# MinghanLi/STMask

Hardware: AMD Instinct MI355X
Metric: frames/sec at 360x640 R50-DCN-FPN (STMask hot path, fp32) (higher is better)
Workload: dtype f32

## Files before the change

include/stmask_hip.h:

```cpp
#ifndef STMASK_HIP_H_
#define STMASK_HIP_H_

#include <stddef.h>
#include <stdint.h>

#ifdef __cplusplus
extern "C" {
#endif

#define STM_ABI_VERSION 6

enum stm_status {
    STM_OK = 0,
    STM_EINVAL = -1,
    STM_ENULL = -2,
    STM_ELAUNCH = -3,
    STM_EWORKSPACE = -4,
    STM_EUNSUPPORTED = -5
};

typedef void* stm_stream_t;

int stm_version(void);
const char* stm_last_error_string(void);
// ... 177 lines not shown

int stm_gather_detections_f32(const int64_t* idx, const int64_t* cls, const float* score, const float* box, const int* count,
                              const float* mask_coeff, const float* track, const float* centerness, int B, int top_k, int N,
                              int mask_dim, int embed_dim, int D, float* out_box, int64_t* out_cls, float* out_score,
                              float* out_coeff, float* out_track, float* out_centerness, int* out_clip, stm_stream_t stream);
int stm_shift_rois_f32(const float* box, const int* clip, float* rois, int n, int feat_h, int feat_w, stm_stream_t stream);
int stm_shift_apply_f32(const float* loc_shift, const float* coeff_shift, float* box, float* coeff, float* score, int n,
                        int mask_dim, float score_decay, stm_stream_t stream);
int stm_match_scores_f32(const float* cos, const float* mask_iou, const float* det_box, const float* prev_box,
                         const float* det_score, const int64_t* det_cls, const int64_t* prev_cls, const int* det_clip,
                         const int* prev_offsets, int D, int Pn, const float* coeff4, float dummy_iou, int* match,
                         stm_stream_t stream);
int stm_match_scores_embed_f32(const float* det_track, const float* prev_track, int embed_dim, const float* mask_iou,
                               const float* det_box, const float* prev_box, const float* det_score, const int64_t* det_cls,
                               const int64_t* prev_cls, const int* det_clip, const int* prev_offsets, int D, int Pn,
                               const float* coeff4, float dummy_iou, int* match, stm_stream_t stream);
int stm_gather_rows2(const void* const* a_rows, const void* const* b_rows, void* const* out_rows, const int* row_bytes,
                     int n_tensors, const int* plan, int n_rows, int n_a, stm_stream_t stream);
int stm_pack_tracked_f32(const float* mask, const float* score, const int* tracked, const int* offsets, const float* box,
                         const int64_t* cls, const float* mask_coeff, int n_rows, int hw, int B, int top_k, int cols,
                         int mask_dim, int max_age, float score_thr, int* keep_ws, float* out, stm_stream_t stream);
int stm_pack_tracked_bits_f32(const uint64_t* mask_bits, int words, const float* score, const int* tracked, const int* offsets,
                              const float* box, const int64_t* cls, const float* mask_coeff, int n_rows, int B, int top_k,
                              int cols, int mask_dim, int max_age, float score_thr, int* keep_ws, float* out,
                              stm_stream_t stream);

int stm_split_planes_f16(const float* x, void* planes, int64_t n_pixels, int C, stm_stream_t stream);
int stm_conv_pack_weights_f16(const float* weight, void* packed, int Cout, int Cin, int kh, int kw, int tile_n, float wscale,
                              stm_stream_t stream);
int stm_conv2d_planar_f16(const void* x_planes, const void* packed_weight, const float* bias, const float* residual_f32,
                          const void* residual_planes, float* out_f32, void* out_planes, const stm_conv_geom* g, int relu,
                          void* workspace, size_t workspace_bytes, stm_stream_t stream);
int stm_dcn_sample_planar_f16(const float* x, const float* offset_mask, int om_ld, void* planes, int out_np,
                              long long out_plane_stride, const stm_deform_geom* g, stm_stream_t stream);

int stm_preprocess_u8_f32(const uint8_t* img, float* out, int n, int H0, int W0, int h, int w, int Hp, int Wp,
                          const double* mean, const double* stdv, int mode, stm_stream_t stream);

typedef struct stm_frame_desc {
    const uint8_t* ptr;
    int H0, W0;
    int64_t row_stride_bytes;
} stm_frame_desc;
int stm_preprocess_u8_multi_f32(const stm_frame_desc* frames, int n, float* out, int h, int w, int Hp, int Wp, const double* mean,
                                const double* stdv, int mode, stm_stream_t stream);

typedef struct stm_head_layout {
    int B, K, n_levels, n_cls, mask_dim, embed_dim, group_pad, small_ld, trk_ld;
    int lvl_start[8], lvl_hw[8];
} stm_head_layout;
int stm_head_assemble_f32(const float* const* small, const float* const* trk, const stm_head_layout* layout, float* conf,
                          float* loc, float* mask, float* track, float* centerness, stm_stream_t stream);

int stm_dcn_sample_planar_f32(const float* x, const float* offset_mask, int om_ld, void* planes, int out_np,
                              long long out_plane_stride, const stm_deform_geom* g, stm_stream_t stream);
int stm_resize_bilinear_planes_f32(const float* x, void* planes, int B, int H, int W, int C, int Ho, int Wo, int fmt,
                                   stm_stream_t stream);

int stm_bias_relu_maxpool_planes_f32(const float* x, const float* bias, void* planes, int B, int H, int W, int C, int fmt,
                                     stm_stream_t stream);

int stm_roi_align_planes_f32(const float* t2s_prev, const float* t2s, const float* corr, const float* rois, void* planes, int B,
                             int H, int W, int C1, int Cc, int n, int PH, int PW, int fmt, stm_stream_t stream);
int stm_roi_align_planes_nhwc_f32(const float* t2s_prev, const float* t2s, const float* corr, int corr_ld, const float* rois,
                                  void* planes, int B, int H, int W, int C1, int Cc, int n, int PH, int PW, int fmt,
                                  stm_stream_t stream);

int stm_stem_rows_planes_f32(const float* x, void* planes, int B, int H, int W, int Cin, int kw, int sw, int pw, int fmt,
                             stm_stream_t stream);

size_t stm_stem_packed_weight_bytes(int Cout, int fmt);
int stm_stem_pack_weights_f32(const float* weight, void* packed, int Cout, int fmt, float wscale, stm_stream_t stream);
int stm_stem_fused_f32(const float* x, const void* packed_weight, const float* bias, void* out_planes, int B, int H, int W, int Cout,
                       int fmt, int out_fmt, float out_scale, stm_stream_t stream);

int stm_planar_set_range_flag(int* device_flag);

int stm_deform_sample_planar_f32(const float* x, int x_ld, const float* offsets, int om_ld, int has_mask, void* planes, int out_np,
                                 int out_pixel_offset, long long out_plane_stride, const stm_deform_geom* g, int fmt,
                                 stm_stream_t stream);

int stm_dcn_sample_planar_fmt_f32(const float* x, const float* offset_mask, int om_ld, void* planes, int out_np,
                                  long long out_plane_stride, const stm_deform_geom* g, int fmt, stm_stream_t stream);

int stm_deform_conv_fused_planar_supported(const stm_deform_geom* g, int Cout, int has_mask, int fmt);
int stm_deform_conv_fused_planar_f32(const float* x, int x_ld, const float* offsets, int om_ld, int has_mask, const void* packed_weight,
                                     const float* bias, void* out_planes, int out_np, int out_pixel_offset, long long out_plane_stride,
                                     int Cout, int relu, float out_scale, const stm_deform_geom* g, int fmt, int out_fmt,
                                     stm_stream_t stream);

typedef struct stm_render_frame {
    const void* base;
    uint8_t* out;
    int64_t base_row_stride;
    int64_t out_row_stride;
    double mean[3], stdv[3];
    int base_fmt, base_h, base_w, base_crop_h, base_crop_w;
    int out_h, out_w;
    int inst_begin, n_inst, crop_h, crop_w;
    int reserved;
} stm_render_frame;
size_t stm_render_workspace_bytes(int n_masks);
int stm_render_overlay_u8(const stm_render_frame* frames, int n_frames, const float* masks, int n_masks, int mh, int mw,
                          const float* colors, const int* boxes, float alpha, void* workspace, size_t workspace_bytes,
                          stm_stream_t stream);

// ... 15 lines not shown
```

stmask_amd/_lib.py:

```python
import ctypes
import os
import subprocess

_HERE = os.path.dirname(os.path.abspath(__file__))
LIB_PATH = os.environ.get("STM_LIBRARY") or os.path.join(_HERE, "libstmask_hip.so")
_lib = None

c_i, c_l, c_f, c_p, c_sz = ctypes.c_int, ctypes.c_int64, ctypes.c_float, ctypes.c_void_p, ctypes.c_size_t

ABI_VERSION = 6
ABI_SYMBOLS = [
    "stm_version", "stm_last_error_string", "stm_struct_bytes", "stm_debug_reload_tunables", "stm_debug_launch_count", "stm_conv_kxr_packed_bytes", "stm_conv_pack_weights_kxr_f32", "stm_conv2d_planar_kxr_f32", "stm_conv2d_planar_dual_f32", "stm_conv2d_planar_windows_f32", "stm_conv2d_planar_windows_pool_f32", "stm_temporal_pool_fc_f32", "stm_stem_packed_weight_bytes", "stm_stem_pack_weights_f32", "stm_stem_fused_f32", "stm_chain_tail_weight_bytes", "stm_chain_tail_weight_bytes_proj", "stm_chain_pack_tail_f32", "stm_chain_pack_tail_proj_f32", "stm_bottleneck_chain_f32", "stm_bottleneck_chain_proj_f32", "stm_deform_im2col_f32", "stm_deform_conv_workspace_bytes",
    "stm_deform_conv_fwd_f32", "stm_gemm_bias_f32", "stm_gemm_workspace_bytes", "stm_gemm_bias_ws_f32", "stm_fcb_ali_offsets_f32", "stm_corr_patch_f32", "stm_corr_patch_nhwc_f32",
    "stm_roi_align_avg_f32", "stm_decode_boxes_f32", "stm_generate_candidates_f32", "stm_cc_fast_nms_f32",
    "stm_detect_cc_workspace_bytes", "stm_detect_cc_f32", "stm_detect_cc_logits_f32", "stm_fast_nms_workspace_bytes", "stm_fast_nms_f32",
    "stm_jaccard_f32", "stm_lincomb_sigmoid_crop_f32", "stm_mask_iou_workspace_bytes", "stm_mask_iou_f32",
    "stm_bias_act_f32", "stm_mask_rle_workspace_bytes", "stm_mask_resize_rle_f32",
    "stm_conv_packed_weight_bytes", "stm_conv_pack_weights_f32",
    "stm_split_bf16_planes_f32", "stm_conv2d_planar_f32", "stm_conv_packed_weight_bytes_tiled",
    "stm_conv_pack_weights_tiled_f32", "stm_preprocess_u8_f32", "stm_head_assemble_f32", "stm_conv2d_planar_ws_f32", "stm_dcn_sample_planar_f32", "stm_conv_pack_weights_fmt_f32", "stm_split_planes_fmt_f32", "stm_dcn_sample_planar_fmt_f32", "stm_planar_set_range_flag", "stm_resize_bilinear_planes_f32", "stm_bias_relu_maxpool_planes_f32", "stm_roi_align_planes_f32", "stm_roi_align_planes_nhwc_f32", "stm_deform_sample_planar_f32", "stm_stem_rows_planes_f32", "stm_mask_iou_grouped_f32", "stm_cc_fast_nms_workspace_bytes", "stm_cc_fast_nms_ws_f32",
    "stm_gather_detections_f32", "stm_shift_rois_f32", "stm_shift_apply_f32", "stm_match_scores_f32", "stm_match_scores_embed_f32", "stm_gather_rows2", "stm_pack_tracked_f32", "stm_pack_tracked_bits_f32",
    "stm_lincomb_sigmoid_crop_bits_f32", "stm_mask_iou_bits_f32", "stm_split_planes_f16", "stm_conv_pack_weights_f16", "stm_conv2d_planar_f16", "stm_dcn_sample_planar_f16",
    "stm_deform_conv_fused_planar_supported", "stm_deform_conv_fused_planar_f32", "stm_fast_nms_batched_workspace_bytes", "stm_fast_nms_batched_f32", "stm_rle_strings_host",
    "stm_preprocess_u8_multi_f32", "stm_render_workspace_bytes", "stm_render_overlay_u8",
    "stm_deform_col2im_f32", "stm_deform_col2im_coord_f32", "stm_roi_align_backward_f32", "stm_corr_backward_f32",
]


class StmError(RuntimeError):
    pass


class DeformGeom(ctypes.Structure):
    _fields_ = [(n, c_i) for n in ("B", "C", "H", "W", "kh", "kw", "sh", "sw", "ph", "pw", "dh", "dw", "dg", "Ho", "Wo")]


class ConvGeom(ctypes.Structure):
    _fields_ = ([(n, c_i) for n in ("B", "H", "W", "C", "Ho", "Wo", "Cout", "kh", "kw", "sh", "sw", "ph", "pw", "x_ld",
                                    "out_ld", "res_ld", "planes", "groups", "n_levels")] +
                [("lvl_start", c_i * 9), ("lvl_h", c_i * 8), ("lvl_w", c_i * 8),
                 ("x_plane_stride", c_l), ("out_plane_stride", c_l), ("res_plane_stride", c_l), ("x_np", c_i), ("out_np", c_i), ("res_np", c_i), ("group_cout", c_i * 8), ("fmt", c_i), ("out_scale", c_f), ("tile_n", c_i), ("out_fmt_plus1", c_i),
                 ("win_h", c_i), ("win_w", c_i), ("win_y0", c_i), ("win_x0", c_i)])


class ConvWindow(ctypes.Structure):
    _fields_ = [(n, c_i) for n in ("kh", "kw", "ph", "pw", "Ho", "Wo", "y0", "x0")]


class FrameDesc(ctypes.Structure):
    _fields_ = [("ptr", c_p), ("H0", c_i), ("W0", c_i), ("row_stride_bytes", c_l)]


class RenderFrame(ctypes.Structure):
    _fields_ = ([("base", c_p), ("out", c_p), ("base_row_stride", c_l), ("out_row_stride", c_l), ("mean", ctypes.c_double * 3),
                 ("stdv", ctypes.c_double * 3)] +
                [(n, c_i) for n in ("base_fmt", "base_h", "base_w", "base_crop_h", "base_crop_w", "out_h", "out_w", "inst_begin", "n_inst",
                                    "crop_h", "crop_w", "reserved")])


class HeadLayout(ctypes.Structure):
    _fields_ = ([(n, c_i) for n in ("B", "K", "n_levels", "n_cls", "mask_dim", "embed_dim", "group_pad", "small_ld", "trk_ld")] +
                [("lvl_start", c_i * 8), ("lvl_hw", c_i * 8)])


def build(force=False):
    cmd = ["make", "-C", os.path.join(_HERE, "csrc"), "-s", "-j4"]
    if force:
        cmd.append("-B")
    subprocess.check_call(cmd)
    return LIB_PATH


def lib():
    global _lib
    if _lib is None:
        if not os.path.exists(LIB_PATH):
            raise StmError(
                f"{LIB_PATH} is missing: build it with `python -c 'import __graft_entry__ as g; g.build()'` "
# ... 30 lines not shown
```

stmask_amd/csrc/capi.hip:

```cpp
#include <stdarg.h>
#include <stdlib.h>

#include <atomic>

#include "stm_common.h"

static thread_local char g_err[512] = "";

void stm_set_error(const char* fmt, ...)
{
    va_list ap;
    va_start(ap, fmt);
    vsnprintf(g_err, sizeof(g_err), fmt, ap);
    va_end(ap);
}

extern "C" int stm_version(void) { return STM_ABI_VERSION; }
extern "C" const char* stm_last_error_string(void) { return g_err; }
extern "C" size_t stm_struct_bytes(int which)
{
    switch (which) {
        case 0: return sizeof(stm_deform_geom);
        case 1: return sizeof(stm_conv_geom);
        case 2: return sizeof(stm_conv_window);
        case 3: return sizeof(stm_head_layout);
        case 4: return sizeof(stm_frame_desc);
        case 5: return sizeof(stm_render_frame);
        default: return 0;
    }
}

static std::atomic<int> g_env_gen{0};
int stm_env_generation() { return g_env_gen.load(std::memory_order_relaxed); }
int stm_env_int_uncached(const char* name, int dflt)
{
    const char* s = getenv(name);
    return (s && *s) ? atoi(s) : dflt;
}
extern "C" void stm_debug_reload_tunables() { g_env_gen.fetch_add(1, std::memory_order_relaxed); }

extern "C" int stm_rle_strings_host(const uint32_t* counts, int ld, const int* n_runs, int n, char* out, int out_ld, int* out_len)
{
    STM_REQUIRE(n >= 0 && ld >= 0 && out_ld >= 0, STM_EINVAL, "stm_rle_strings_host: negative size");
    if (n == 0) return STM_OK;
    STM_REQUIRE(counts && n_runs && out && out_len, STM_ENULL, "stm_rle_strings_host: NULL argument");
    int rc = STM_OK;
    for (int i = 0; i < n; ++i) {
        const uint32_t* c = counts + (size_t)i * ld;
        char* o = out + (size_t)i * out_ld;
        const int m = n_runs[i] < ld ? n_runs[i] : ld;
        int len = 0;
        for (int j = 0; j < m; ++j) {
            long long x = (long long)c[j];
            if (j > 2) x -= (long long)c[j - 2];
            bool more = true;
            while (more) {
                int ch = (int)(x & 0x1f);
                x >>= 5;
                more = (ch & 0x10) ? x != -1 : x != 0;
                if (more) ch |= 0x20;
                if (len < out_ld) o[len] = (char)(ch + 48);
                ++len;
            }
        }
        out_len[i] = len;
        if (len > out_ld) rc = STM_EINVAL;
    }
    if (rc != STM_OK) stm_set_error("stm_rle_strings_host: a string needs more than %d bytes", out_ld);
    return rc;
}
```

stmask_amd/csrc/conv_bf16x.hip:

```cpp
#include "planar_common.h"
#include <algorithm>
#include <type_traits>
#include <atomic>
#include <mutex>
#include <unordered_map>

namespace {

__device__ __forceinline__ void store_planes8(uint8_t* dst, size_t plane_b, const float (&v)[8], int fmt, int* range_flag, bool nt)
{
    unsigned q0[4], q1[4], q2[4];
    if (fmt == 0) {
#pragma unroll
        for (int e = 0; e < 4; ++e) split2(f32x2{v[2 * e], v[2 * e + 1]}, q0[e], q1[e], q2[e]);
    } else {
        f16_range_check8(v, range_flag);
#pragma unroll
        for (int e = 0; e < 4; ++e) split2_f16(f32x2{v[2 * e], v[2 * e + 1]}, q0[e], q1[e]);
    }
    const int np = fmt == 0 ? 3 : (fmt == 1 ? 2 : 1);
    if (nt) {
        __builtin_nontemporal_store(u32x4{q0[0], q0[1], q0[2], q0[3]}, reinterpret_cast<u32x4*>(dst));
        if (np > 1) __builtin_nontemporal_store(u32x4{q1[0], q1[1], q1[2], q1[3]}, reinterpret_cast<u32x4*>(dst + plane_b));
        if (np > 2) __builtin_nontemporal_store(u32x4{q2[0], q2[1], q2[2], q2[3]}, reinterpret_cast<u32x4*>(dst + 2 * plane_b));
    } else {
        *reinterpret_cast<u32x4*>(dst) = u32x4{q0[0], q0[1], q0[2], q0[3]};
        if (np > 1) *reinterpret_cast<u32x4*>(dst + plane_b) = u32x4{q1[0], q1[1], q1[2], q1[3]};
        if (np > 2) *reinterpret_cast<u32x4*>(dst + 2 * plane_b) = u32x4{q2[0], q2[1], q2[2], q2[3]};
    }
}

constexpr int STM_MAX_DEVICES = 32;
static int* g_range_flags[STM_MAX_DEVICES] = {};
static int* current_range_flag()
{
    int dev = 0;
    if (hipGetDevice(&dev) != hipSuccess || dev < 0 || dev >= STM_MAX_DEVICES) return nullptr;
    return g_range_flags[dev];
}

struct PlanarArgs {
    const uint8_t* xp;
    const uint8_t* wp;
    const float* bias;
    const float* res_f32;
    const uint8_t* res_pl;
    float* out_f32;
    uint8_t* out_pl;
    int B, H, W, C, Ho, Wo, Cout;
    int kh, kw, sh, sw, ph, pw;
    int x_ld, out_ld, res_ld;
    int x_np, out_np, res_np;
    int relu;
    int M, n_tiles, m_tiles, slabs;
    int nsub;
    unsigned plane_bytes;
    long long x_pstride, out_pstride, res_pstride;
    int groups, ntpg, cout_g;
    int group_real[8];
    int n_levels;
    int lvl_start[9], lvl_h[8], lvl_w[8];
    int pointwise;
    float inv_hw, inv_w;
    int fmt;
    int out_fmt;
    float out_scale;
    int* range_flag;
    int nt_out;
    int splitk, kslabs, ldp;
    float* partial;
    int vec_epilogue;
    const uint8_t* xp2;
    long long x2_pstride;
    unsigned plane2_bytes;
    int c1_slabs, x2_np, H2, W2, s2;
    int win_w, win_hw, win_off;
};
struct PlanarArgsCls : PlanarArgs {
    int n_cls, cls_tiles;
    unsigned long long* pool;
    int pool_ld;
    struct Cls { const uint8_t* wp; int kh, kw, ph, pw, Ho, Wo, M, slabs, win_off, tile0; float inv_hw, inv_w; } cls[9];
};

template <int NJ>
__device__ __forceinline__ float* park_base(uint8_t* smem, int wave) { return reinterpret_cast<float*>(smem) + wave * (64 * (32 * NJ + 4)); }

template <int NJ>
__device__ __forceinline__ void park16(f32x4 (&acc)[4][2 * NJ], f32x4 (&accl)[4][2 * NJ], uint8_t* smem, int wave, int lane, float ls = 1.0f)
{
    constexpr int EP_LD = 32 * NJ + 4;
    float* park = park_base<NJ>(smem, wave);
#pragma unroll
    for (int i = 0; i < 4; ++i)
#pragma unroll
        for (int j = 0; j < 2 * NJ; ++j)
#pragma unroll
            for (int r = 0; r < 4; ++r)
                park[(i * 16 + 4 * (lane >> 4) + r) * EP_LD + j * 16 + (lane & 15)] = acc[i][j][r] + accl[i][j][r] * ls;
}

template <bool SCALE_BIAS = true, int FMT = -1>
__device__ __forceinline__ void epilogue_store8(const PlanarArgs& a, int m, int co, int nvalid, float (&v)[8], bool have_pre = false,
                                                f16x8 pre0 = f16x8{}, f16x8 pre1 = f16x8{})
{
    const int fmt = FMT >= 0 ? FMT : a.fmt;
    const int ofmt = (FMT == 0 || FMT == 1) ? FMT : a.out_fmt;
    const size_t opl = (size_t)(a.out_pstride >> 1), rpl = (size_t)(a.res_pstride >> 1);
    auto pidx = [](int m_, int co_, int np) { return ((size_t)(co_ >> 5) * np + m_) * 32 + (co_ & 31); };
    int mo = m;
    if (a.win_w) {
        const int hw = a.Ho * a.Wo;
        int b = (int)((float)m * a.inv_hw);
        int rem = m - b * hw;
        if (rem < 0) { --b; rem += hw; } else if (rem >= hw) { ++b; rem -= hw; }
        int oy = (int)((float)rem * a.inv_w);
        const int t = rem - oy * a.Wo;
        if (t < 0) --oy; else if (t >= a.Wo) ++oy;
        mo = b * a.win_hw + oy * a.win_w + (rem - oy * a.Wo) + a.win_off;
    }
    if constexpr (SCALE_BIAS) {
#pragma unroll
        for (int e = 0; e < 8; ++e) v[e] = __builtin_fmaf(v[e], a.out_scale, (a.bias && e < nvalid) ? a.bias[co + e] : 0.0f);
    }
    if (a.vec_epilogue) {
        if (a.res_f32) {
            const f32x4 r0 = *reinterpret_cast<const f32x4*>(a.res_f32 + (size_t)m * a.res_ld + co);
            const f32x4 r1 = *reinterpret_cast<const f32x4*>(a.res_f32 + (size_t)m * a.res_ld + co + 4);
            v[0] += r0.x; v[1] += r0.y; v[2] += r0.z; v[3] += r0.w; v[4] += r1.x; v[5] += r1.y; v[6] += r1.z; v[7] += r1.w;
// ... 145 lines not shown
            q0[j] = *reinterpret_cast<const f32x4*>(pk);
            q1[j] = *reinterpret_cast<const f32x4*>(pk + 4);
        }
#pragma unroll
        for (int j = 0; j < 4; ++j) {
            if (k0 + j < a.splitk) {
                v[0] += q0[j].x; v[1] += q0[j].y; v[2] += q0[j].z; v[3] += q0[j].w;
                v[4] += q1[j].x; v[5] += q1[j].y; v[6] += q1[j].z; v[7] += q1[j].w;
            }
        }
    }
    epilogue_store8(a, m, grp * a.cout_g + cog, min(8, a.cout_g - cog), v);
}

__device__ __forceinline__ void pooled_epilogue(const PlanarArgs& a, unsigned long long* pool, int pool_ld, uint8_t* smem, int wave, int lane, int mw, int col)
{
    constexpr int EP_LD = 32 * 2 + 4;
    const float* park = park_base<2>(smem, wave);
    asm volatile("s_waitcnt lgkmcnt(0)" ::: "memory");
    const int hw = a.Ho * a.Wo;
    const int rows = min(64, a.M - mw);
    int b = mw / hw, r = mw - b * hw;
    const float bias = a.bias ? a.bias[col] : 0.0f;
    float sum = 0.0f;
    for (int row = 0; row < rows; ++row) {
        sum += __builtin_fmaxf(__builtin_fmaf(park[row * EP_LD + lane], a.out_scale, bias), 0.0f);
        if (++r == hw || row == rows - 1) {
            if (!(sum < 4.0e9f) && a.range_flag) *reinterpret_cast<volatile int*>(a.range_flag) = 1;
            const unsigned hi = (unsigned)sum;
            const unsigned lo = (unsigned)((sum - (float)hi) * 4294967296.0f);
            __hip_atomic_fetch_add(pool + (size_t)b * pool_ld + col, ((unsigned long long)hi << 32) | lo, __ATOMIC_RELAXED, __HIP_MEMORY_SCOPE_AGENT);
            sum = 0.0f;
            if (r == hw) { r = 0; ++b; }
        }
    }
}

template <int NPL, int MG, int NJ, int DT = 0, int ST = 2, int ABL = 0, bool DUAL = false, bool CLS = false>
__global__ __launch_bounds__(512, 1) void conv_planar_kernel(const typename std::conditional<CLS, PlanarArgsCls, PlanarArgs>::type a_in)
{
#if defined(__HIP_DEVICE_COMPILE__)
    extern __shared__ __align__(16) uint8_t smem[];
    constexpr int BM = CV_BM * MG;
    constexpr int BN = 64 * NJ;
    constexpr int WPL = BN * 64;
    constexpr int XBUF = NPL * BM * 64, WBUF = NPL * WPL, BUF = XBUF + WBUF;
    constexpr int NWAVES = 4 * MG;
    constexpr int WDMA = (BN / 16) * NPL / NWAVES;
    static_assert((BN / 16) * NPL % NWAVES == 0, "weight tile must split evenly over the waves");
    static_assert(ST == 2 || (ST == 3 && DT == 1 && NPL <= 2), "the three-buffer ring is built for the fp16 formats");

    int tiles_ = a_in.m_tiles * a_in.n_tiles * a_in.splitk;
    if constexpr (CLS) tiles_ = a_in.cls_tiles;
    const int tiles = tiles_;
    const int per_xcd = (tiles + 7) >> 3;
    int logical = (blockIdx.x & 7) * per_xcd + (blockIdx.x >> 3);
    auto regroup = [&](int j, int nt_all, int& mt_o, int& nt_o) {
        const int pg = 32 / a_in.nsub, G = pg * nt_all;
        const int gq = j / G, r = j - gq * G;
        const int nh = r >> 5, rr = r & 31;
        mt_o = gq * pg + rr / a_in.nsub;
        nt_o = nh * a_in.nsub + rr % a_in.nsub;
    };
    if constexpr (CLS) {
        const int j = blockIdx.x >> 3;
        int jm = j / a_in.n_tiles, nt_ = j - jm * a_in.n_tiles;
        if (a_in.nsub) regroup(j, a_in.n_tiles, jm, nt_);
        logical = (jm * 8 + (int)(blockIdx.x & 7)) * a_in.n_tiles + nt_;
    } else if (a_in.nsub) {
        int mt_, nt_;
        regroup(logical, a_in.n_tiles, mt_, nt_);
        logical = mt_ * a_in.n_tiles + nt_;
    }
    if (logical >= tiles) return;
    PlanarArgs a_cls;
    const PlanarArgs* ap = &a_in;
    if constexpr (CLS) {
        int c = 0;
#pragma unroll
        for (int i = 1; i < 9; ++i)
            if (i < a_in.n_cls && logical >= a_in.cls[i].tile0) c = i;
        a_cls = static_cast<const PlanarArgs&>(a_in);
        a_cls.wp = a_in.cls[c].wp;
        a_cls.kh = a_in.cls[c].kh; a_cls.kw = a_in.cls[c].kw; a_cls.ph = a_in.cls[c].ph; a_cls.pw = a_in.cls[c].pw;
        a_cls.Ho = a_in.cls[c].Ho; a_cls.Wo = a_in.cls[c].Wo; a_cls.M = a_in.cls[c].M;
        a_cls.slabs = a_in.cls[c].slabs; a_cls.kslabs = a_in.cls[c].slabs; a_cls.win_off = a_in.cls[c].win_off;
        a_cls.inv_hw = a_in.cls[c].inv_hw; a_cls.inv_w = a_in.cls[c].inv_w;
        logical -= a_in.cls[c].tile0;
        ap = &a_cls;
    }
    const PlanarArgs& a = *ap;
    const int ksp = a.splitk == 1 ? 0 : logical % a.splitk;
    const int tile = a.splitk == 1 ? logical : logical / a.splitk;
    const int mt = a.n_tiles == 1 ? tile : (a.n_tiles == 2 ? tile >> 1 : (a.n_tiles == 4 ? tile >> 2 : tile / a.n_tiles));
    const int nt = tile - mt * a.n_tiles;
    const int m0 = mt * BM;
    if (m0 >= a.M) return;
    const int s_begin = ksp * a.kslabs, s_end = min(a.slabs, s_begin + a.kslabs);

    const int tid = threadIdx.x, lane = tid & 63;
    const int wave = __builtin_amdgcn_readfirstlane(tid >> 6);
    const int wm = wave % (2 * MG), wn = wave / (2 * MG);

    const int grp = a.groups == 1 ? 0 : nt / a.ntpg;
    const int n0g = (nt - grp * a.ntpg) * BN;
    const int creal = a.group_real[grp & 7];
    int base[2], wl64[2];
    unsigned vmask[2];
    int base2[2] = {0, 0};
    const int slot = lane & 3;
#pragma unroll
    for (int i = 0; i < 2; ++i) {
        const int r = (2 * wave + i) * 16 + (lane >> 2);
        const int m = m0 + r;
        const bool ok = m < a.M;
        const int mm = ok ? m : 0;
        const int swz16 = (slot ^ swz(r)) << 4;
        if constexpr (DUAL) {
            const int hw = a.Ho * a.Wo;
            int b = (int)((float)mm * a.inv_hw);
            int rem = mm - b * hw;
            if (rem < 0) { --b; rem += hw; } else if (rem >= hw) { ++b; rem -= hw; }
            int oy = (int)((float)rem * a.inv_w);
            const int t = rem - oy * a.Wo;
            if (t < 0) --oy; else if (t >= a.Wo) ++oy;
            const int ox = rem - oy * a.Wo;
            base2[i] = ((b * a.H2 + oy * a.s2) * a.W2 + ox * a.s2) * 64 + swz16;
        }
        if (a.pointwise) {
            base[i] = mm * 64 + swz16;
            wl64[i] = 0;
            vmask[i] = ok ? 1u : 0u;
            continue;
        }
        int H = a.H, W = a.W, Ho = a.Ho, Wo = a.Wo, first = 0, local = mm;
        if (a.n_levels > 0) {
#pragma unroll
            for (int l = 0; l < 8; ++l)
                if (l < a.n_levels && mm >= a.lvl_start[l]) { first = a.lvl_start[l]; H = a.lvl_h[l]; W = a.lvl_w[l]; }
            Ho = H; Wo = W; local = mm - first;
        }
        int b, rem, oy, ox;
        if (a.n_levels > 0) {
            b = local / (Ho * Wo);
            rem = local - b * (Ho * Wo);
            oy = rem / Wo;
        } else {
            const int hw = Ho * Wo;
            b = (int)((float)local * a.inv_hw);
            rem = local - b * hw;
// ... 318 lines not shown
        }
    }
    if (a.splitk > 1) {
        constexpr int EP_LD = 32 * NJ + 4, LPR = 4 * NJ;
        const float* park = park_base<NJ>(smem, wave);
        asm volatile("s_waitcnt lgkmcnt(0)" ::: "memory");
        const int seg = lane % LPR, prow = lane / LPR;
        const int col = nt * BN + wn * (32 * NJ) + seg * 8;
#pragma unroll
        for (int pass = 0; pass < LPR; ++pass) {
            const int pr = pass * (64 / LPR) + prow;
            const int m = m0 + wm * 64 + pr;
            if (m >= a.M) continue;
            float* o = a.partial + ((size_t)ksp * a.M + m) * a.ldp + col;
            *reinterpret_cast<f32x4*>(o) = *reinterpret_cast<const f32x4*>(park + pr * EP_LD + seg * 8);
            *reinterpret_cast<f32x4*>(o + 4) = *reinterpret_cast<const f32x4*>(park + pr * EP_LD + seg * 8 + 4);
        }
    } else {
        planar_epilogue_tail<NJ, DT == 1 ? (NPL == 2 ? 1 : 2) : 0>(a, smem, wave, lane, m0, n0g, grp, wm, wn);
    }
#endif
}

constexpr int KX3_XROWS = 272, KX3_XPL = KX3_XROWS * 64, KX3_ABUF = 2 * KX3_XPL, KX3_WBUF = 2 * 128 * 64, KX3_W0 = 2 * KX3_ABUF;
constexpr int KX3_ZROW = 260;
constexpr int KX3_LDS_LOOP = KX3_W0 + 3 * KX3_WBUF;
#ifndef KX3_SCHED
#define KX3_SCHED 24
#endif
#ifndef KX3_WBUFFER
#define KX3_WBUFFER 1
#endif
#ifndef KX3_ABL
#define KX3_ABL 0
#endif
template <int ABL = 0, bool WIN = false>
__global__ __launch_bounds__(512, 1) void conv_planar_kx3_kernel(const typename std::conditional<WIN, PlanarArgsCls, PlanarArgs>::type a_in)
{
#if defined(__HIP_DEVICE_COMPILE__)
    extern __shared__ __align__(16) uint8_t smem[];
    constexpr int NJ = 2, BM = 256, BN = 128, WPL = BN * 64;
    constexpr int XROWS = WIN ? 384 : KX3_XROWS, XPL = XROWS * 64, ABUF = 2 * XPL, W0 = 2 * ABUF;
    int logical, n_tiles_ = a_in.n_tiles, cls_c = 0;
    if constexpr (WIN) {
        const int j = blockIdx.x >> 3;
        const int jm = j / n_tiles_, nt_ = j - jm * n_tiles_;
        logical = (jm * 8 + (int)(blockIdx.x & 7)) * n_tiles_ + nt_;
        if (logical >= a_in.cls_tiles) return;
#pragma unroll
        for (int i = 1; i < 9; ++i)
            if (i < a_in.n_cls && logical >= a_in.cls[i].tile0) cls_c = i;
        logical -= a_in.cls[cls_c].tile0;
    } else {
        const int tiles = a_in.m_tiles * n_tiles_;
        const int per_xcd = (tiles + 7) >> 3;
        logical = (blockIdx.x & 7) * per_xcd + (blockIdx.x >> 3);
        if (logical >= tiles) return;
    }
    const PlanarArgs& a = a_in;
    int KH = a.kh, PH = a.ph, PW = a.pw, HO = a.Ho, WO = a.Wo, MM = a.M, SLABS = a.slabs;
    const uint8_t* WP = a.wp;
    if constexpr (WIN) {
        KH = a_in.cls[cls_c].kh; PH = a_in.cls[cls_c].ph; PW = a_in.cls[cls_c].pw; HO = a_in.cls[cls_c].Ho; WO = a_in.cls[cls_c].Wo;
        MM = a_in.cls[cls_c].M; SLABS = a_in.cls[cls_c].slabs; WP = a_in.cls[cls_c].wp;
    }
    const int mt = n_tiles_ == 1 ? logical : (n_tiles_ == 2 ? logical >> 1 : (n_tiles_ == 4 ? logical >> 2 : logical / n_tiles_));
    const int nt = logical - mt * n_tiles_;
    const int m0 = mt * BM;
    const int tid = threadIdx.x, lane = tid & 63;
    const int wave = __builtin_amdgcn_readfirstlane(tid >> 6);
    const int wm = wave & 3, wn = wave >> 2;
    const int grp = a.groups == 1 ? 0 : nt / a.ntpg;
    const int n0g = (nt - grp * a.ntpg) * BN;
    const int cslabs = a.C / CV_BK;

    auto decode = [&](int m, int& first, int& b, int& oy, int& ox, int& H, int& W) -> bool {
        const bool ok = m >= 0 && m < MM;
        const int mm = ok ? m : 0;
        H = a.H; W = a.W; first = 0;
        int local = mm;
        if (a.n_levels > 0) {
#pragma unroll
            for (int l = 0; l < 8; ++l)
                if (l < a.n_levels && mm >= a.lvl_start[l]) { first = a.lvl_start[l]; H = a.lvl_h[l]; W = a.lvl_w[l]; }
            local = mm - first;
            b = local / (H * W);
            const int rem = local - b * (H * W);
            oy = rem / W;
            ox = rem - oy * W;
        } else {
            const int hw = H * W;
            b = (int)((float)local * a.inv_hw);
            int rem = local - b * hw;
            if (rem < 0) { --b; rem += hw; } else if (rem >= hw) { ++b; rem -= hw; }
            oy = (int)((float)rem * a.inv_w);
            int t = rem - oy * W;
            if (t < 0) --oy; else if (t >= W) ++oy;
            ox = rem - oy * W;
        }
        return ok;
    };

    int base[3], wlv[3];
    const int slot = lane & 3;
    const int Ws = WO + 2, wr0 = WIN ? m0 / WO : 0;
#pragma unroll
    for (int i = 0; i < 3; ++i) {
        const int q = i == 0 ? wave : (i == 1 ? wave + 8 : (WIN ? wave + 16 : 16));
        const int j = q * 16 + (lane >> 2);
        if constexpr (WIN) {
            const int qr = j / Ws, xi = j - qr * Ws;
            const int wr = wr0 + qr;
            const bool ok = wr * WO < MM;
            const int b = wr / HO, oy = wr - b * HO;
            wlv[i] = a.W * 64 + (ok ? 63 : 0);
            base[i] = ((b * a.H + oy - PH) * a.W + (xi - PW)) * 64 + ((slot ^ swz(j)) << 4);
        } else {
            int first, b, oy, ox, H, W;
            const bool ok = decode(m0 - 1 + j, first, b, oy, ox, H, W) && j < BM + 2;
            unsigned vm = 0;
            for (int ky = 0; ky < KH; ++ky)
// ... 940 lines not shown
}

extern "C" int stm_conv2d_planar_dual_f32(const void* x_planes, const void* x2_planes, int C2, int H2, int W2, int s2, long long x2_np,
                                          long long x2_plane_stride, const void* packed_weight, const float* bias, const float* residual_f32,
                                          const void* residual_planes, float* out_f32, void* out_planes, const stm_conv_geom* g, int relu,
                                          void* workspace, size_t workspace_bytes, stm_stream_t stream)
{
    STM_REQUIRE(x2_planes && g, STM_ENULL, "stm_conv2d_planar_dual_f32: x2_planes / geometry must be non-NULL");
    DualSrc d{x2_planes, C2, H2, W2, s2, x2_np, x2_plane_stride};
    return conv2d_planar_impl(x_planes, packed_weight, bias, residual_f32, residual_planes, out_f32, out_planes, g, relu, workspace,
                              workspace_bytes, stream, &d, nullptr);
}

extern "C" int stm_conv2d_planar_windows_f32(const void* x_planes, const void* const* packed_weights, const stm_conv_window* windows, int n_windows,
                                             const float* bias, float* out_f32, void* out_planes, const stm_conv_geom* g, int relu, stm_stream_t stream)
{
    const char* who = "stm_conv2d_planar_windows_f32";
    STM_REQUIRE(packed_weights && windows && g, STM_ENULL, "%s: NULL argument", who);
    STM_REQUIRE(n_windows >= 1 && n_windows <= 9, STM_EINVAL, "%s: 1 .. 9 windows", who);
    STM_REQUIRE(g->win_w > 0 && g->win_h > 0 && g->fmt == 1 && g->sh == 1 && g->sw == 1 && (g->groups <= 1) && g->n_levels <= 0 &&
                (g->tile_n == 0 || g->tile_n == 128), STM_EUNSUPPORTED, "%s: fp16x2 planes, stride 1, one group, 128-channel tiles, win_h / win_w set", who);
    for (int i = 0; i < n_windows; ++i) STM_REQUIRE(packed_weights[i], STM_ENULL, "%s: packed weight %d is NULL", who, i);
    stm_conv_geom g0 = *g;
    g0.kh = windows[0].kh; g0.kw = windows[0].kw; g0.ph = windows[0].ph; g0.pw = windows[0].pw;
    g0.Ho = windows[0].Ho; g0.Wo = windows[0].Wo; g0.win_y0 = windows[0].y0; g0.win_x0 = windows[0].x0;
    WinSet ws{packed_weights, windows, n_windows, nullptr};
    return conv2d_planar_impl(x_planes, packed_weights[0], bias, nullptr, nullptr, out_f32, out_planes, &g0, relu, nullptr, 0, stream, nullptr, &ws);
}

extern "C" int stm_conv2d_planar_windows_pool_f32(const void* x_planes, const void* const* packed_weights, const stm_conv_window* windows, int n_windows,
                                                  const float* bias, unsigned long long* pool_fix, const stm_conv_geom* g, stm_stream_t stream)
{
    const char* who = "stm_conv2d_planar_windows_pool_f32";
    STM_REQUIRE(packed_weights && windows && g && pool_fix, STM_ENULL, "%s: NULL argument", who);
    STM_REQUIRE(n_windows >= 1 && n_windows <= 9, STM_EINVAL, "%s: 1 .. 9 windows", who);
    STM_REQUIRE(g->win_w > 0 && g->win_h > 0 && g->fmt == 1 && g->sh == 1 && g->sw == 1 && (g->groups <= 1) && g->n_levels <= 0 &&
                (g->tile_n == 0 || g->tile_n == 128) && g->Cout % 128 == 0, STM_EUNSUPPORTED,
                "%s: fp16x2 planes, stride 1, one group, whole 128-channel tiles, win_h / win_w set", who);
    STM_REQUIRE((uintptr_t)pool_fix % 8 == 0, STM_EINVAL, "%s: pool_fix must be 8-byte aligned", who);
    for (int i = 0; i < n_windows; ++i) STM_REQUIRE(packed_weights[i], STM_ENULL, "%s: packed weight %d is NULL", who, i);
    stm_conv_geom g0 = *g;
    g0.kh = windows[0].kh; g0.kw = windows[0].kw; g0.ph = windows[0].ph; g0.pw = windows[0].pw;
    g0.Ho = windows[0].Ho; g0.Wo = windows[0].Wo; g0.win_y0 = windows[0].y0; g0.win_x0 = windows[0].x0;
    WinSet ws{packed_weights, windows, n_windows, pool_fix};
    return conv2d_planar_impl(x_planes, packed_weights[0], bias, nullptr, nullptr, nullptr, nullptr, &g0, 1, nullptr, 0, stream, nullptr, &ws);
}

namespace {
int conv2d_planar_impl(const void* x_planes, const void* packed_weight, const float* bias, const float* residual_f32,
                       const void* residual_planes, float* out_f32, void* out_planes, const stm_conv_geom* g,
                       int relu, void* workspace, size_t workspace_bytes, stm_stream_t stream, const DualSrc* dual, const WinSet* wset)
{
    const char* who = dual ? "stm_conv2d_planar_dual_f32" : "stm_conv2d_planar_f32";
    STM_REQUIRE(x_planes && packed_weight && (out_f32 || out_planes || (wset && wset->pool)), STM_ENULL,
                "%s: x_planes/packed_weight and at least one output must be non-NULL", who);
    STM_REQUIRE(g, STM_ENULL, "%s: geometry is NULL", who);
    const int groups = g->groups > 0 ? g->groups : 1;
    STM_REQUIRE(g->C > 0 && g->C % CV_BK == 0 && g->Cout > 0 && g->Cout % groups == 0 && g->kh > 0 && g->kw > 0 &&
                (g->planes >= 1 && g->planes <= 3), STM_EINVAL, "%s: bad channel / kernel / planes arguments", who);
    const int cout_g = g->Cout / groups;
    const int bn = g->tile_n ? g->tile_n : CV_BN;
    STM_REQUIRE(bn == 64 || bn == 128, STM_EINVAL, "%s: tile_n must be 64 or 128", who);
    STM_REQUIRE(groups == 1 || cout_g % bn == 0, STM_EINVAL, "%s: Cout per group (%d) must be a multiple of the tile width %d", who, cout_g, bn);
    int64_t M, in_pixels;
    if (g->n_levels > 0) {
        STM_REQUIRE(g->n_levels <= 8 && g->sh == 1 && g->sw == 1 && 2 * g->ph == g->kh - 1 && 2 * g->pw == g->kw - 1, STM_EINVAL,
                    "%s: multi-level launches need stride 1 and same padding (<= 8 levels)", who);
        STM_REQUIRE(g->lvl_start[0] == 0, STM_EINVAL, "%s: lvl_start[0] must be 0", who);
        for (int l = 0; l < g->n_levels; ++l) {
            const int n = g->lvl_start[l + 1] - g->lvl_start[l];
            STM_REQUIRE(g->lvl_h[l] > 0 && g->lvl_w[l] > 0 && n > 0 && n % (g->lvl_h[l] * g->lvl_w[l]) == 0, STM_EINVAL,
                        "%s: level %d: %d pixels is not a whole number of %dx%d images", who, l, n, g->lvl_h[l], g->lvl_w[l]);
        }
        M = in_pixels = g->lvl_start[g->n_levels];
    } else {
        if (!geom_ok(g, who)) return STM_EINVAL;
        M = (int64_t)g->B * g->Ho * g->Wo;
        in_pixels = (int64_t)g->B * g->H * g->W;
    }
    const int out_ld = g->out_ld ? g->out_ld : g->Cout, res_ld = g->res_ld ? g->res_ld : g->Cout;
    STM_REQUIRE(out_ld >= g->Cout && res_ld >= g->Cout, STM_EINVAL, "%s: bad leading dimensions out_ld=%d res_ld=%d", who, out_ld, res_ld);
    const bool win = g->n_levels <= 0 && g->win_w > 0;
    const int64_t out_rows = win ? (int64_t)g->B * g->win_h * g->win_w : M;
    const int64_t x_np = g->x_np ? g->x_np : in_pixels, out_np = g->out_np ? g->out_np : out_rows, res_np = g->res_np ? g->res_np : M;
    STM_REQUIRE(!win || (!residual_f32 && !residual_planes && !dual), STM_EUNSUPPORTED, "%s: window launches take no residual / second source", who);
    STM_REQUIRE(x_np >= in_pixels && out_np >= out_rows && res_np >= M, STM_EINVAL, "%s: x_np / out_np / res_np smaller than the pixel count", who);
    STM_REQUIRE((uintptr_t)x_planes % 16 == 0 && (uintptr_t)packed_weight % 16 == 0, STM_EINVAL,
                "%s: x_planes and packed_weight must be 16-byte aligned", who);
    if (dual) {
        STM_REQUIRE(groups == 1 && g->n_levels <= 0 && g->kh == 1 && g->kw == 1 && g->sh == 1 && g->sw == 1 && g->ph == 0 && g->pw == 0 &&
                    g->H == g->Ho && g->W == g->Wo && (g->fmt == 1 || g->fmt == 2), STM_EUNSUPPORTED,
                    "%s: 1x1 / stride 1 / one group / fp16 plane formats only", who);
        STM_REQUIRE(dual->C2 > 0 && dual->C2 % CV_BK == 0 && dual->C2 < g->C && dual->s2 >= 1 && dual->H2 > 0 && dual->W2 > 0 &&
                    (dual->H2 - 1) / dual->s2 + 1 == g->Ho && (dual->W2 - 1) / dual->s2 + 1 == g->Wo, STM_EINVAL,
                    "%s: second source %d channels of %dx%d at stride %d does not match the %dx%d output", who, dual->C2, dual->H2, dual->W2, dual->s2,
                    g->Ho, g->Wo);
    }
    const int64_t x_slabs = dual ? (int64_t)(g->C - dual->C2) / CV_BK : (int64_t)groups * (g->C / CV_BK);
    const int64_t plane_bytes = x_slabs * x_np * 64;
    STM_REQUIRE(plane_bytes < ((int64_t)1 << 31), STM_EUNSUPPORTED, "%s: plane larger than 2 GiB", who);
    STM_REQUIRE(M < ((int64_t)1 << 30), STM_EUNSUPPORTED, "%s: too many output pixels", who);
    const int64_t o_slabs = stm_cdiv(g->Cout, 32);
    const int64_t xps = g->x_plane_stride ? g->x_plane_stride : x_slabs * x_np * 32;
    const int64_t ops = g->out_plane_stride ? g->out_plane_stride : o_slabs * out_np * 32;
    const int64_t rps = g->res_plane_stride ? g->res_plane_stride : o_slabs * res_np * 32;
    STM_REQUIRE(xps % 8 == 0, STM_EINVAL, "%s: x_plane_stride must be a multiple of 8 elements", who);
    const int x_ld = 0;
    PlanarArgs a;
    a.xp = static_cast<const uint8_t*>(x_planes); a.wp = static_cast<const uint8_t*>(packed_weight); a.bias = bias;
    a.res_f32 = residual_f32; a.res_pl = static_cast<const uint8_t*>(residual_planes);
    a.out_f32 = out_f32; a.out_pl = static_cast<uint8_t*>(out_planes);
    a.B = g->B; a.H = g->H; a.W = g->W; a.C = g->C; a.Ho = g->Ho; a.Wo = g->Wo; a.Cout = g->Cout;
    a.kh = g->kh; a.kw = g->kw; a.sh = g->sh; a.sw = g->sw; a.ph = g->ph; a.pw = g->pw;
    a.x_ld = x_ld; a.out_ld = out_ld; a.res_ld = res_ld; a.relu = relu;
    a.x_np = (int)x_np; a.out_np = (int)out_np; a.res_np = (int)res_np;
    a.M = (int)M; a.n_tiles = stm_cdiv(g->Cout, bn); a.slabs = g->kh * g->kw * (g->C / CV_BK);
    a.nsub = 0;
    a.plane_bytes = (unsigned)plane_bytes;
    a.x_pstride = xps * 2; a.out_pstride = ops * 2; a.res_pstride = rps * 2;
    a.groups = groups; a.cout_g = cout_g; a.ntpg = stm_cdiv(cout_g, bn);
    for (int i = 0; i < 8; ++i) a.group_real[i] = (i < groups && g->group_cout[i] > 0 && g->group_cout[i] < cout_g) ? g->group_cout[i] : cout_g;
    a.n_levels = g->n_levels > 0 ? g->n_levels : 0;
    for (int l = 0; l < 8; ++l) { a.lvl_start[l] = g->lvl_start[l]; a.lvl_h[l] = g->lvl_h[l]; a.lvl_w[l] = g->lvl_w[l]; }
    a.lvl_start[8] = g->lvl_start[8];
    const ConvTunables& tn = tunables();
    a.vec_epilogue = (cout_g % 8 == 0) && (!out_f32 || out_ld % 4 == 0) && (!residual_f32 || res_ld % 4 == 0) && ((uintptr_t)out_f32 % 16 == 0) &&
                     ((uintptr_t)out_planes % 16 == 0) && ((uintptr_t)residual_f32 % 16 == 0) && ((uintptr_t)residual_planes % 16 == 0) &&
                     (ops % 8 == 0) && (rps % 8 == 0) && !tn.scalar_epilogue;
    STM_REQUIRE(g->kh * g->kw <= 32, STM_EUNSUPPORTED, "%s: more than 32 taps", who);
    a.pointwise = (g->n_levels <= 0 && !win && g->kh == 1 && g->kw == 1 && g->sh == 1 && g->sw == 1 && g->ph == 0 && g->pw == 0) ? 1 : 0;
    a.win_w = win ? g->win_w : 0; a.win_hw = win ? g->win_h * g->win_w : 0; a.win_off = win ? g->win_y0 * g->win_w + g->win_x0 : 0;
    a.inv_hw = g->n_levels > 0 ? 0.0f : 1.0f / (float)((int64_t)g->Ho * g->Wo);
    a.inv_w = g->n_levels > 0 ? 0.0f : 1.0f / (float)g->Wo;
    STM_REQUIRE(g->n_levels > 0 || M < ((int64_t)1 << 24), STM_EUNSUPPORTED, "%s: more than 2^24 output pixels in one launch", who);
    a.fmt = (g->fmt >= 0 && g->fmt <= 2) ? g->fmt : 0;
    a.out_fmt = g->out_fmt_plus1 > 0 ? g->out_fmt_plus1 - 1 : a.fmt;
    STM_REQUIRE(a.out_fmt >= 0 && a.out_fmt <= 2 && (a.out_fmt == a.fmt || (a.fmt == 2 && a.out_fmt == 1)), STM_EINVAL,
                "%s: output format %d cannot be produced by a format-%d layer", who, a.out_fmt, a.fmt);
    a.out_scale = (a.fmt >= 1 && g->out_scale > 0.0f) ? g->out_scale : 1.0f;
    a.range_flag = current_range_flag();
    a.nt_out = tn.nt_mb > 0 && M * (int64_t)g->Cout * 4 >= tn.nt_mb * 1000000;
    const int want_planes = a.fmt == 0 ? 3 : (a.fmt == 1 ? 2 : 1);
    STM_REQUIRE(g->planes == want_planes || (a.fmt == 0 && g->planes == 2), STM_EINVAL, "%s: format %d has %d planes (planes = %d)", who, a.fmt,
                want_planes, g->planes);
    a.splitk = 1; a.kslabs = a.slabs; a.partial = nullptr; a.ldp = a.n_tiles * bn;
    a.xp2 = nullptr; a.x2_pstride = 0; a.plane2_bytes = 0; a.c1_slabs = a.slabs; a.x2_np = 0; a.H2 = a.W2 = 0; a.s2 = 1;
    if (dual) {
        const int64_t in2 = (int64_t)g->B * dual->H2 * dual->W2;
        const int64_t np2 = dual->x2_np ? dual->x2_np : in2;
        const int64_t slabs2 = dual->C2 / CV_BK;
        const int64_t ps2 = dual->x2_plane_stride ? dual->x2_plane_stride : slabs2 * np2 * 32;
        STM_REQUIRE(np2 >= in2 && slabs2 * np2 * 64 < ((int64_t)1 << 31) && ps2 % 8 == 0 && (uintptr_t)dual->x2 % 16 == 0, STM_EINVAL,
                    "%s: bad second-source plane geometry", who);
        a.xp2 = static_cast<const uint8_t*>(dual->x2); a.x2_pstride = ps2 * 2; a.plane2_bytes = (unsigned)(slabs2 * np2 * 64);
        a.c1_slabs = (int)x_slabs; a.x2_np = (int)np2; a.H2 = dual->H2; a.W2 = dual->W2; a.s2 = dual->s2;
    }
    bool full = cout_g % 64 == 0;
    for (int gi = 0; gi < groups && gi < 8; ++gi) full = full && a.group_real[gi] == cout_g;
    auto plan_splitk = [&](int tiles) {
        int sk = tn.splitk;
        if (sk <= 0) {
            sk = 1;
            if (bn == 64) {
                if (tn.sk_rule == 1 || !full) {
                    if (tiles <= 256 && a.slabs >= 24) sk = (int)std::min<int64_t>(std::min<int64_t>(8, 768 / tiles), a.slabs / 10);
                } else if (tiles <= 128 && a.slabs >= 24)
                    sk = (int)std::min<int64_t>(std::min<int64_t>(8, tn.sk_target / tiles), a.slabs / (tiles <= 40 ? 10 : 16));
            } else if (tiles < 128 && a.slabs >= 24) sk = (int)std::min<int64_t>(std::min<int64_t>(8, 256 / tiles), a.slabs / 12);
        }
        if (sk < 2) return;
        const int per = stm_cdiv(a.slabs, sk);
        sk = stm_cdiv(a.slabs, per);
        if (sk < 2 || !workspace || (size_t)sk * M * a.ldp * sizeof(float) > workspace_bytes || ((uintptr_t)workspace % 16)) return;
        a.splitk = sk; a.kslabs = per; a.partial = static_cast<float*>(workspace);
    };
    auto finish_splitk = [&]() -> int {
        if (a.splitk < 2) return STM_OK;
        const int64_t total = M * groups * ((cout_g + 7) / 8);
        hipLaunchKernelGGL(planar_splitk_finish_kernel, dim3(stm_cdiv(total, 256)), dim3(256), 0, stm_hs(stream), a, bn);
        STM_CHECK_LAUNCH("planar_splitk_finish_kernel");
        return STM_OK;
    };
    if (wset) {
        STM_REQUIRE(bn == 128 && a.fmt == 1 && !dual && win, STM_EUNSUPPORTED, "%s: window sets run on the 256 x 128 ring tiles of the fp16x2 format", who);
        PlanarArgsCls ac[2];
        int t0[2] = {0, 0}, ncls[2] = {0, 0};
        for (int k = 0; k < 2; ++k) {
            static_cast<PlanarArgs&>(ac[k]) = a;
            ac[k].pool = wset->pool;
            ac[k].pool_ld = g->Cout;
        }
        for (int i = 0; i < wset->n; ++i) {
            const stm_conv_window& w = wset->win[i];
            STM_REQUIRE(w.kh > 0 && w.kw > 0 && w.kh * w.kw <= 32 && w.Ho > 0 && w.Wo > 0 && w.y0 >= 0 && w.x0 >= 0 && w.y0 + w.Ho <= g->win_h &&
                            w.x0 + w.Wo <= g->win_w, STM_EINVAL, "%s: window %d (%dx%d at %d, %d, kernel %dx%d) is not inside the %dx%d output", who, i, w.Ho,
                        w.Wo, w.y0, w.x0, w.kh, w.kw, g->win_h, g->win_w);
            STM_REQUIRE((uintptr_t)wset->packed[i] % 16 == 0, STM_EINVAL, "%s: packed weight %d is not 16-byte aligned", who, i);
            const int64_t Mc = (int64_t)g->B * w.Ho * w.Wo;
            STM_REQUIRE(Mc < ((int64_t)1 << 24), STM_EUNSUPPORTED, "%s: more than 2^24 output pixels in one window", who);
            const bool taps_inside = -w.ph >= 0 && -w.ph + (w.Ho - 1) + (w.kh - 1) <= g->H - 1 && -w.pw >= 0 && -w.pw + (w.Wo - 1) + (w.kw - 1) <= g->W - 1;
            const int k = (tn.kx3 && w.kw == 3 && w.kh <= 6 && taps_inside && (255 / w.Wo + 2) * (w.Wo + 2) <= 384) ? 1 : 0;
            PlanarArgsCls::Cls& c = ac[k].cls[ncls[k]++];
            c.wp = static_cast<const uint8_t*>(wset->packed[i]);
            c.kh = w.kh; c.kw = w.kw; c.ph = w.ph; c.pw = w.pw; c.Ho = w.Ho; c.Wo = w.Wo; c.M = (int)Mc;
            c.slabs = w.kh * w.kw * (g->C / CV_BK); c.win_off = w.y0 * g->win_w + w.x0; c.tile0 = t0[k];
            c.inv_hw = 1.0f / (float)(w.Ho * w.Wo); c.inv_w = 1.0f / (float)w.Wo;
            t0[k] += stm_cdiv(Mc, 2 * CV_BM) * a.n_tiles;
        }
        for (int k = 0; k < 2; ++k) {
            if (!ncls[k]) continue;
            for (int i = ncls[k]; i < 9; ++i) ac[k].cls[i] = ac[k].cls[0];
            ac[k].n_cls = ncls[k];
            ac[k].cls_tiles = t0[k];
            ac[k].m_tiles = 0;
            ac[k].nsub = 0;
            if (k == 0) {
                ac[0].nsub = ((tn.nsub == 2 || tn.nsub == 4) && a.n_tiles > tn.nsub && a.n_tiles % tn.nsub == 0 && g->groups == 1) ? tn.nsub : 0;
                const int pg = ac[0].nsub ? 32 / ac[0].nsub : 1;
#ifndef CLS_ABL
#define CLS_ABL 0
#endif
                const int rc0 = launch_planar<2, 2, 2, 1, 3, CLS_ABL, false, true>(ac[0], stm_cdiv(stm_cdiv(t0[0] / a.n_tiles, 8), pg) * pg * 8 * a.n_tiles, stream);
                if (rc0 != STM_OK) return rc0;
            } else {
                static std::atomic<bool> kx3w_reserved[STM_MAX_DEVICES];
                constexpr size_t lds = 2 * 2 * 384 * 64 + 3 * KX3_WBUF;
                int dev = 0;
                const bool have_dev = hipGetDevice(&dev) == hipSuccess && dev >= 0 && dev < STM_MAX_DEVICES;
                if (!have_dev || !kx3w_reserved[dev].load(std::memory_order_relaxed)) {
                    STM_REQUIRE(hipFuncSetAttribute(reinterpret_cast<const void*>(conv_planar_kx3_kernel<KX3_ABL, true>), hipFuncAttributeMaxDynamicSharedMemorySize,
                                                    (int)lds) == hipSuccess, STM_ELAUNCH, "%s: cannot reserve %zu bytes of LDS", who, lds);
                    if (have_dev) kx3w_reserved[dev].store(true, std::memory_order_relaxed);
                }
                hipLaunchKernelGGL((conv_planar_kx3_kernel<KX3_ABL, true>), dim3(stm_cdiv(t0[1] / a.n_tiles, 8) * 8 * a.n_tiles), dim3(512), lds, stm_hs(stream), ac[1]);
                STM_CHECK_LAUNCH("conv_planar_kx3_kernel<WIN>");
                g_kx3_launches.fetch_add(1, std::memory_order_relaxed);
            }
        }
        return STM_OK;
    }
    int rc;
    if (bn == 64) {
        a.m_tiles = stm_cdiv(M, CV_BM);
        plan_splitk(a.m_tiles * a.n_tiles);
        const int tiles = a.m_tiles * a.n_tiles * a.splitk;
        const bool small_grid = tiles <= tn.ring64_small;
        const bool ring = full && (tn.ring64 == 3 ? (small_grid || (a.splitk == 1 && a.slabs >= 12 && a.slabs <= 40)) : tn.ring64 == 4);
        if (dual) {
            if (a.fmt == 2) rc = ring ? launch_planar<1, 1, 1, 1, 3, 0, true>(a, tiles, stream) : launch_planar<1, 1, 1, 1, 2, 0, true>(a, tiles, stream);
            else rc = ring ? launch_planar<2, 1, 1, 1, 3, 0, true>(a, tiles, stream) : launch_planar<2, 1, 1, 1, 2, 0, true>(a, tiles, stream);
        } else if (a.fmt == 2) rc = ring ? launch_planar<1, 1, 1, 1, 3>(a, tiles, stream) : launch_planar<1, 1, 1, 1>(a, tiles, stream);
        else if (a.fmt == 1) rc = ring ? launch_planar<2, 1, 1, 1, 3>(a, tiles, stream) : launch_planar<2, 1, 1, 1>(a, tiles, stream);
        else rc = g->planes == 3 ? launch_planar<3, 1, 1>(a, tiles, stream) : launch_planar<2, 1, 1>(a, tiles, stream);
        return rc != STM_OK ? rc : finish_splitk();
    }
    const int64_t t2 = (int64_t)stm_cdiv(M, 2 * CV_BM) * a.n_tiles;
    const int mg = tn.mg ? tn.mg : (t2 >= 192 ? 2 : 1);
    a.m_tiles = stm_cdiv(M, CV_BM * mg);
    plan_splitk(a.m_tiles * a.n_tiles);
    a.nsub = ((tn.nsub == 2 || tn.nsub == 4) && a.splitk == 1 && a.n_tiles > tn.nsub && a.n_tiles % tn.nsub == 0 && g->groups == 1 &&
              a.m_tiles >= 4 * (32 / tn.nsub)) ? tn.nsub : 0;
    if (a.nsub) a.m_tiles = stm_cdiv(a.m_tiles, 32 / a.nsub) * (32 / a.nsub);
    const int tiles = a.m_tiles * a.n_tiles * a.splitk;
    const bool ring = tn.ring == 3;
#ifdef STM_ABLATE
    if (a.fmt == 1 && ring && mg == 2 && tn.abl) {
        const int abl = tn.abl;
        rc = abl == 1 ? launch_planar<2, 2, 2, 1, 3, 1>(a, tiles, stream) : abl == 2 ? launch_planar<2, 2, 2, 1, 3, 2>(a, tiles, stream)
           : abl == 3 ? launch_planar<2, 2, 2, 1, 3, 3>(a, tiles, stream) : abl == 5 ? launch_planar<2, 2, 2, 1, 3, 5>(a, tiles, stream)
           : abl == 8 ? launch_planar<2, 2, 2, 1, 3, 8>(a, tiles, stream) : abl == 16 ? launch_planar<2, 2, 2, 1, 3, 16>(a, tiles, stream)
           : abl == 32 ? launch_planar<2, 2, 2, 1, 3, 32>(a, tiles, stream) : abl == 64 ? launch_planar<2, 2, 2, 1, 3, 64>(a, tiles, stream)
                      : launch_planar<2, 2, 2, 1, 3, 7>(a, tiles, stream);
        return rc != STM_OK ? rc : finish_splitk();
    }
#endif
    if (tn.kx3 && a.fmt == 1 && ring && mg == 2 && !dual && !win && a.splitk == 1 && a.kw == 3 && a.pw == 1 && a.sh == 1 && a.sw == 1 &&
        a.slabs % 3 == 0 && a.kh <= 6 && 2 * a.ph == a.kh - 1 && full) {
        static std::atomic<bool> kx3_reserved[STM_MAX_DEVICES];
        constexpr size_t lds = 8 * 64 * (64 + 4) * sizeof(float) > (size_t)KX3_LDS_LOOP ? 8 * 64 * (64 + 4) * sizeof(float) : (size_t)KX3_LDS_LOOP;
        int dev = 0;
        const bool have_dev = hipGetDevice(&dev) == hipSuccess && dev >= 0 && dev < STM_MAX_DEVICES;
        if (!have_dev || !kx3_reserved[dev].load(std::memory_order_relaxed)) {
            STM_REQUIRE(hipFuncSetAttribute(reinterpret_cast<const void*>(conv_planar_kx3_kernel<KX3_ABL, false>), hipFuncAttributeMaxDynamicSharedMemorySize, (int)lds) ==
                            hipSuccess, STM_ELAUNCH, "%s: cannot reserve %zu bytes of LDS", who, lds);
            if (have_dev) kx3_reserved[dev].store(true, std::memory_order_relaxed);
        }
        hipLaunchKernelGGL((conv_planar_kx3_kernel<KX3_ABL, false>), dim3(8 * stm_cdiv(tiles, 8)), dim3(512), lds, stm_hs(stream), a);
        STM_CHECK_LAUNCH("conv_planar_kx3_kernel");
        g_kx3_launches.fetch_add(1, std::memory_order_relaxed);
        return STM_OK;
    }
    if (dual) {
        if (a.fmt == 2) rc = mg == 2 ? launch_planar<1, 2, 2, 1, 3, 0, true>(a, tiles, stream) : launch_planar<1, 1, 2, 1, 3, 0, true>(a, tiles, stream);
        else rc = mg == 2 ? launch_planar<2, 2, 2, 1, 3, 0, true>(a, tiles, stream) : launch_planar<2, 1, 2, 1, 3, 0, true>(a, tiles, stream);
    } else if (a.fmt == 2) {
        if (ring) rc = mg == 2 ? launch_planar<1, 2, 2, 1, 3>(a, tiles, stream) : launch_planar<1, 1, 2, 1, 3>(a, tiles, stream);
        else rc = mg == 2 ? launch_planar<1, 2, 2, 1>(a, tiles, stream) : launch_planar<1, 1, 2, 1>(a, tiles, stream);
    } else if (a.fmt == 1) {
        if (ring) rc = mg == 2 ? launch_planar<2, 2, 2, 1, 3>(a, tiles, stream) : launch_planar<2, 1, 2, 1, 3>(a, tiles, stream);
        else rc = mg == 2 ? launch_planar<2, 2, 2, 1>(a, tiles, stream) : launch_planar<2, 1, 2, 1>(a, tiles, stream);
    } else if (g->planes == 3) rc = mg == 2 ? launch_planar<3, 2, 2>(a, tiles, stream) : launch_planar<3, 1, 2>(a, tiles, stream);
    else rc = mg == 2 ? launch_planar<2, 2, 2>(a, tiles, stream) : launch_planar<2, 1, 2>(a, tiles, stream);
    return rc != STM_OK ? rc : finish_splitk();
}
}

extern "C" long long stm_debug_launch_count(int which)
{
    return which == 0 ? g_kx3_launches.load(std::memory_order_relaxed) : (which == 1 ? stm_internal_fused_dcn_launches() : -1);
}

extern "C" int stm_conv2d_planar_f32(const void* x_planes, const void* packed_weight, const float* bias, const float* residual_f32,
                                     const void* residual_planes, float* out_f32, void* out_planes, const stm_conv_geom* g,
// ... 29 lines not shown
```

stmask_amd/csrc/conv_kxr.hip:

```cpp
#include "planar_common.h"

#include <algorithm>
#include <atomic>

namespace {

constexpr int KX_CONSUMERS = 4, KX_PRODUCERS = 2, KX_THREADS = 64 * (KX_CONSUMERS + KX_PRODUCERS);
constexpr int KX_MAX_JOBS = 4;
constexpr int KX_MAX_DEVICES = 32;
constexpr int KX_LDS_MAX = 160 * 1024;

constexpr int kx_stage_bytes(int kw, int npl, int nc, int pt) { return npl * (64 * pt + 16) * 64 + kw * npl * nc * 1024; }
constexpr int kx_pt(int kw, int npl, int nc)
{
    if (nc >= 4 && npl == 2) return 2;
#ifndef KX_PT_MAX
#define KX_PT_MAX 4
#endif
    for (int pt = KX_PT_MAX; pt > 2; --pt)
        if (3 * kx_stage_bytes(kw, npl, nc, pt) <= KX_LDS_MAX) return pt;
    return 2;
}
constexpr int kx_depth(int kw, int npl, int nc)
{
    const int d = KX_LDS_MAX / kx_stage_bytes(kw, npl, nc, kx_pt(kw, npl, nc));
    return d > 4 ? 4 : d;
}

struct KxrJob {
    const uint8_t* wp;
    const float* bias;
    int bias_n;
    int x_slab0;
    int out_ch0;
    int nc;
    int tile0;
    int per_xcd;
    int lvl_tile0[9];
};

struct KxrArgs {
    const uint8_t* xp;
    float* out_f32;
    uint8_t* out_pl;
    KxrJob job[KX_MAX_JOBS];
    int n_jobs, total;
    int cslabs, kh, ph, pw;
    int x_np, out_ld, out_np;
    long long x_pstride, out_pstride;
    unsigned plane_bytes;
    int relu, out_fmt;
    float out_scale;
    int* range_flag;
    int n_lvl;
    int lvl_start[9], lvl_h[8], lvl_w[8];
};

typedef __attribute__((address_space(3))) void* lds_ptr;
typedef const __attribute__((address_space(1))) void* glb_ptr;

#define KX_MM(a_, b_, c_) __builtin_amdgcn_mfma_f32_16x16x32_f16(a_, b_, c_, 0, 0, 0)
#ifndef KX_ABL
#define KX_ABL 0
#endif

template <int KW, int NPL, int NC>
__device__ __forceinline__ void kxr_body(const KxrArgs& a, const KxrJob& jb, int tile_first, int n_seq, int tile_step, uint8_t* smem)
{
#if defined(__HIP_DEVICE_COMPILE__)
    constexpr int PT = kx_pt(KW, NPL, NC), D = kx_depth(KW, NPL, NC);
    constexpr int BM = 64 * PT, XROWS = BM + 16, NRG = XROWS / 16;
    constexpr int HALO = KW - 1;
    constexpr int XPL = XROWS * 64;
    constexpr int XBUF = NPL * XPL;
    constexpr int WT = NC * 16 * 64;
    constexpr int WBUF = KW * NPL * WT;
    constexpr int BUF = XBUF + WBUF;
    constexpr int NWD = KW * NPL * NC;
    constexpr int NXD = NRG * NPL;
    constexpr int XDW = (NXD + KX_PRODUCERS - 1) / KX_PRODUCERS, WDW = (NWD + KX_PRODUCERS - 1) / KX_PRODUCERS;
    constexpr int NPD = XDW + WDW;
    static_assert(BM + HALO <= XROWS - 1, "the always-zero row must exist");
    static_assert(D >= 2 && D * BUF <= KX_LDS_MAX && (D - 2) * NPD <= 63, "ring does not fit");

    const int tid = threadIdx.x, lane = tid & 63;
    const int wave = __builtin_amdgcn_readfirstlane(tid >> 6);
    const int S = a.cslabs * a.kh;
    struct TileGeo { int H, W, lstart, lend, m0; };
    auto tile_geo = [&](int id) {
        const int tile = (id & 7) * jb.per_xcd + (id >> 3);
        int lvl = 0;
#pragma unroll
        for (int l = 1; l < 8; ++l)
            if (l < a.n_lvl && tile >= jb.lvl_tile0[l]) lvl = l;
        TileGeo g;
        g.H = a.lvl_h[lvl]; g.W = a.lvl_w[lvl]; g.lstart = a.lvl_start[lvl]; g.lend = a.lvl_start[lvl + 1];
        g.m0 = g.lstart + (tile - jb.lvl_tile0[lvl]) * BM;
        return g;
    };

    if (wave >= KX_CONSUMERS) {
        const int pw_ = wave - KX_CONSUMERS;
        __amdgpu_buffer_rsrc_t xr[NPL];
#pragma unroll
        for (int p = 0; p < NPL; ++p)
            xr[p] = __builtin_amdgcn_make_buffer_rsrc(const_cast<uint8_t*>(a.xp) + (size_t)p * a.x_pstride, 0, (int)a.plane_bytes, 0x00020000);
        int dbase[XDW];
        unsigned dmask[XDW];
        int W = 1;
        auto setup = [&](int tile) {
            const TileGeo tg = tile_geo(tile);
            W = tg.W;
            const int HW = tg.H * tg.W;
#pragma unroll
            for (int i = 0; i < XDW; ++i) {
                const int piece = min(pw_ + KX_PRODUCERS * i, NXD - 1);
                const int rg = piece % NRG;
                const int j = rg * 16 + (lane >> 2);
                const int q = tg.m0 - a.pw + j;
                const bool okq = j < BM + HALO && q >= tg.lstart && q < tg.lend;
                const int local = okq ? q - tg.lstart : 0;
                const int y = (local % HW) / tg.W;
                unsigned vm = 0;
                for (int ky = 0; ky < a.kh; ++ky)
                    if ((unsigned)(y + ky - a.ph) < (unsigned)tg.H) vm |= 1u << ky;
                dmask[i] = okq ? vm : 0u;
                dbase[i] = (q - a.ph * tg.W) * 64 + (((lane & 3) ^ swz(j)) << 4);
            }
        };
        int cs = 0, ky = 0, buf = 0, s_in = 0, t_in = 0;
        auto issue = [&]() {
            if (s_in == 0) setup(tile_first + t_in * tile_step);
            uint8_t* xb = smem + buf * BUF;
            const int uni = (jb.x_slab0 + cs) * (a.x_np * 64) + ky * (W * 64);
#pragma unroll
            for (int i = 0; i < XDW; ++i) {
                const int piece = min(pw_ + KX_PRODUCERS * i, NXD - 1);
                const int p = piece / NRG, rg = piece - p * NRG;
                const unsigned oob = ((dmask[i] >> ky) & 1u) ^ 1u;
                const unsigned off = (unsigned)(dbase[i] + uni) | (oob << 31);
                if (!(KX_ABL & 5)) __builtin_amdgcn_raw_ptr_buffer_load_lds(xr[NPL == 2 ? (p & 1) : 0], (lds_ptr)(xb + p * XPL + rg * 1024), 16, off, 0, 0, 0);
            }
            uint8_t* wb = xb + XBUF;
// ... 280 lines not shown
        j.lvl_tile0[a.n_lvl] = t0;
        j.per_xcd = (t0 + 7) / 8;
        a.total += 8 * j.per_xcd;
    }
    static std::atomic<int> reserved[KX_MAX_DEVICES];
    int dev = 0;
    const bool have_dev = hipGetDevice(&dev) == hipSuccess && dev >= 0 && dev < KX_MAX_DEVICES;
    if (!have_dev || reserved[dev].load(std::memory_order_relaxed) < (int)lds) {
        STM_REQUIRE(hipFuncSetAttribute(reinterpret_cast<const void*>(conv_kxr_kernel<KW, NPL>), hipFuncAttributeMaxDynamicSharedMemorySize,
                                        (int)lds) == hipSuccess, STM_ELAUNCH, "stm_conv2d_planar_kxr_f32: cannot reserve %zu bytes of LDS", lds);
        if (have_dev) reserved[dev].store((int)lds, std::memory_order_relaxed);
    }
    static std::atomic<int> n_cus[KX_MAX_DEVICES];
    int cus = have_dev ? n_cus[dev].load(std::memory_order_relaxed) : 0;
    if (cus <= 0) {
        hipDeviceProp_t prop;
        cus = (have_dev && hipGetDeviceProperties(&prop, dev) == hipSuccess && prop.multiProcessorCount > 0) ? prop.multiProcessorCount : 256;
        if (have_dev) n_cus[dev].store(cus, std::memory_order_relaxed);
    }
    hipLaunchKernelGGL((conv_kxr_kernel<KW, NPL>), dim3(std::min(a.total, std::max(cus / 8 * 8, 8))), dim3(KX_THREADS), lds, stm_hs(stream), a);
    STM_CHECK_LAUNCH("conv_kxr_kernel");
    return STM_OK;
}

}

extern "C" size_t stm_conv_kxr_packed_bytes(const stm_conv_geom* g)
{
    KxrPlan pl;
    return kxr_plan(g, &pl, "stm_conv_kxr_packed_bytes") ? pl.woff[pl.n_jobs] : 0;
}

extern "C" int stm_conv_pack_weights_kxr_f32(const float* weight, void* packed, const stm_conv_geom* g, float wscale, stm_stream_t stream)
{
    const char* who = "stm_conv_pack_weights_kxr_f32";
    STM_REQUIRE(weight && packed, STM_ENULL, "%s: weight/packed must be non-NULL", who);
    KxrPlan pl;
    if (!kxr_plan(g, &pl, who)) return STM_EINVAL;
    STM_REQUIRE((uintptr_t)packed % 16 == 0, STM_EINVAL, "%s: packed buffer must be 16-byte aligned", who);
    STM_REQUIRE(wscale > 0.0f && wscale < 3.0e38f, STM_EINVAL, "%s: bad weight scale", who);
    for (int i = 0; i < pl.n_jobs; ++i) {
        const int64_t total = (int64_t)(g->C / 32) * g->kh * g->kw * pl.nc[i] * 16 * 4;
        hipLaunchKernelGGL(kxr_pack_kernel, dim3(stm_cdiv(total, 256)), dim3(256), 0, stm_hs(stream), weight, static_cast<uint8_t*>(packed) + pl.woff[i],
                           i * pl.cout_g, pl.creal[i], pl.nc[i], g->C, g->kh, g->kw, pl.npl, wscale);
        STM_CHECK_LAUNCH("kxr_pack_kernel");
    }
    return STM_OK;
}

extern "C" int stm_conv2d_planar_kxr_f32(const void* x_planes, const void* packed_weight, const float* bias, float* out_f32, void* out_planes,
                                         const stm_conv_geom* g, int relu, stm_stream_t stream)
{
    const char* who = "stm_conv2d_planar_kxr_f32";
    STM_REQUIRE(x_planes && packed_weight && (out_f32 || out_planes), STM_ENULL, "%s: x_planes/packed_weight and at least one output must be non-NULL", who);
    KxrPlan pl;
    if (!kxr_plan(g, &pl, who)) return STM_EINVAL;
    KxrArgs a;
    memset(&a, 0, sizeof(a));
    int64_t M;
    if (g->n_levels > 0) {
        STM_REQUIRE(g->n_levels <= 8 && g->lvl_start[0] == 0, STM_EINVAL, "%s: at most 8 levels, lvl_start[0] = 0", who);
        a.n_lvl = g->n_levels;
        for (int l = 0; l < g->n_levels; ++l) {
            const int n = g->lvl_start[l + 1] - g->lvl_start[l];
            STM_REQUIRE(g->lvl_h[l] > 0 && g->lvl_w[l] > 0 && n > 0 && n % (g->lvl_h[l] * g->lvl_w[l]) == 0, STM_EINVAL,
                        "%s: level %d: %d pixels is not a whole number of %dx%d images", who, l, n, g->lvl_h[l], g->lvl_w[l]);
            a.lvl_start[l] = g->lvl_start[l]; a.lvl_h[l] = g->lvl_h[l]; a.lvl_w[l] = g->lvl_w[l];
        }
        a.lvl_start[g->n_levels] = g->lvl_start[g->n_levels];
        M = g->lvl_start[g->n_levels];
    } else {
        STM_REQUIRE(g->B > 0 && g->H > 0 && g->W > 0, STM_EINVAL, "%s: bad image batch", who);
        STM_REQUIRE(g->Ho == g->H + 2 * g->ph - g->kh + 1 && g->Wo == g->W + 2 * g->pw - g->kw + 1 && g->Ho == g->H && g->Wo == g->W, STM_EUNSUPPORTED,
                    "%s: the kernel keeps the image size (padding (k - 1) / 2)", who);
        a.n_lvl = 1;
        M = (int64_t)g->B * g->H * g->W;
        a.lvl_start[0] = 0; a.lvl_start[1] = (int)M; a.lvl_h[0] = g->H; a.lvl_w[0] = g->W;
    }
    STM_REQUIRE(2 * g->ph == g->kh - 1 && 2 * g->pw == g->kw - 1, STM_EUNSUPPORTED, "%s: same padding only", who);
    STM_REQUIRE(M < ((int64_t)1 << 30), STM_EUNSUPPORTED, "%s: too many pixels", who);
    const int groups = pl.n_jobs;
    const int64_t x_np = g->x_np ? g->x_np : M, out_np = g->out_np ? g->out_np : M;
    STM_REQUIRE(x_np >= M && out_np >= M, STM_EINVAL, "%s: x_np / out_np smaller than the pixel count", who);
    const int64_t x_slabs = (int64_t)groups * (g->C / 32);
    const int64_t plane_bytes = x_slabs * x_np * 64;
    STM_REQUIRE(plane_bytes < ((int64_t)1 << 31), STM_EUNSUPPORTED, "%s: plane larger than 2 GiB", who);
    const int64_t xps = g->x_plane_stride ? g->x_plane_stride : x_slabs * x_np * 32;
    const int64_t ops = g->out_plane_stride ? g->out_plane_stride : (int64_t)stm_cdiv(g->Cout, 32) * out_np * 32;
    const int out_ld = g->out_ld ? g->out_ld : g->Cout;
    STM_REQUIRE((uintptr_t)x_planes % 16 == 0 && (uintptr_t)packed_weight % 16 == 0 && xps % 8 == 0, STM_EINVAL, "%s: 16-byte alignment required", who);
    STM_REQUIRE(!out_f32 || ((uintptr_t)out_f32 % 16 == 0 && out_ld % 4 == 0), STM_EINVAL, "%s: out_f32 must be 16-byte aligned with out_ld a multiple of 4", who);
    STM_REQUIRE(!out_planes || ((uintptr_t)out_planes % 16 == 0 && ops % 8 == 0), STM_EINVAL, "%s: out_planes must be 16-byte aligned", who);
    a.xp = static_cast<const uint8_t*>(x_planes); a.out_f32 = out_f32; a.out_pl = static_cast<uint8_t*>(out_planes);
    a.n_jobs = groups;
    int nc_max = 1;
    for (int i = 0; i < groups; ++i) {
        KxrJob& j = a.job[i];
        j.wp = static_cast<const uint8_t*>(packed_weight) + pl.woff[i];
        j.bias = bias ? bias + (size_t)i * pl.cout_g : nullptr;
        j.bias_n = pl.cout_g;
        j.x_slab0 = i * (g->C / 32);
        j.out_ch0 = i * pl.cout_g;
        j.nc = pl.nc[i];
        nc_max = std::max(nc_max, j.nc);
        STM_REQUIRE(j.out_ch0 + 16 * j.nc <= (out_f32 ? out_ld : g->Cout) || !out_f32, STM_EINVAL,
                    "%s: group %d writes channels [%d, %d) but an output row has %d", who, i, j.out_ch0, j.out_ch0 + 16 * j.nc, out_ld);
        STM_REQUIRE(!out_planes || j.out_ch0 + 16 * j.nc <= stm_cdiv(g->Cout, 32) * 32, STM_EINVAL, "%s: group %d leaves the output planes", who, i);
    }
    a.cslabs = g->C / 32; a.kh = g->kh; a.ph = g->ph; a.pw = g->pw;
    a.x_np = (int)x_np; a.out_ld = out_ld; a.out_np = (int)out_np;
    a.x_pstride = xps * 2; a.out_pstride = ops * 2;
    a.plane_bytes = (unsigned)plane_bytes;
    a.relu = relu;
    a.out_fmt = g->out_fmt_plus1 > 0 ? g->out_fmt_plus1 - 1 : g->fmt;
    STM_REQUIRE(a.out_fmt == g->fmt || (g->fmt == 2 && a.out_fmt == 1), STM_EINVAL, "%s: output format %d cannot be produced by a format-%d layer", who,
                a.out_fmt, g->fmt);
    a.out_scale = g->out_scale > 0.0f ? g->out_scale : 1.0f;
    a.range_flag = stm_internal_range_flag();
    (void)nc_max;
    if (g->fmt == 1) return g->kw == 3 ? kxr_launch<3, 2>(a, stream) : kxr_launch<5, 2>(a, stream);
    return g->kw == 3 ? kxr_launch<3, 1>(a, stream) : kxr_launch<5, 1>(a, stream);
}
```

stmask_amd/csrc/stm_common.h:

```cpp
#pragma once
#include <hip/hip_runtime.h>
#include <stdint.h>
#include <stdio.h>
#include <string.h>

#include "../../include/stmask_hip.h"

#define STM_WAVE 64

void stm_set_error(const char* fmt, ...);

#define STM_REQUIRE(cond, code, ...)      \
    do {                                  \
        if (!(cond)) {                    \
            stm_set_error(__VA_ARGS__);   \
            return (code);                \
        }                                 \
    } while (0)

#define STM_CHECK_LAUNCH(name)                                                       \
    do {                                                                             \
        hipError_t e_ = hipGetLastError();                                           \
        if (e_ != hipSuccess) {                                                      \
            stm_set_error("%s: launch failed: %s", (name), hipGetErrorString(e_));   \
            return STM_ELAUNCH;                                                      \
        }                                                                            \
    } while (0)

int stm_env_generation();
int stm_env_int_uncached(const char* name, int dflt);
#define STM_ENV_INT(name, dflt)                                                          \
    ([]() -> int {                                                                       \
        static int v_ = 0, gen_ = -1;                                                    \
        const int g_ = stm_env_generation();                                             \
        if (gen_ != g_) { v_ = stm_env_int_uncached((name), (dflt)); gen_ = g_; }        \
        return v_;                                                                       \
    }())

int* stm_internal_range_flag();
long long stm_internal_fused_dcn_launches();

static inline hipStream_t stm_hs(stm_stream_t s) { return reinterpret_cast<hipStream_t>(s); }

static inline int stm_cdiv(int64_t a, int64_t b) { return (int)((a + b - 1) / b); }


__device__ __forceinline__ int64_t stm_xcd_block(int64_t nblocks)
{
    const int64_t per_xcd = (nblocks + 7) >> 3;
    const int64_t b = (int64_t)(blockIdx.x & 7) * per_xcd + (blockIdx.x >> 3);
    return b < nblocks ? b : -1;
}
__device__ __forceinline__ int64_t stm_xcd_block_or_plain(int xcd, int64_t nblocks) { return xcd ? stm_xcd_block(nblocks) : (int64_t)blockIdx.x; }
static inline unsigned stm_xcd_grid(int64_t nblocks) { return (unsigned)(8 * ((nblocks + 7) / 8)); }

__device__ __forceinline__ void stm_bilinear_tap(int o, float scale, int in, int& i0, int& i1, float& l, float& h)
{
    float f = scale * ((float)o + 0.5f) - 0.5f;
    if (f < 0.0f) f = 0.0f;
    i0 = (int)f;
    i1 = i0 + (i0 < in - 1 ? 1 : 0);
    l = f - (float)i0;
    h = 1.0f - l;
}
__device__ __forceinline__ float stm_bilinear_blend(const float* __restrict__ m, int64_t ld, int y0, int y1, int x0, int x1, float ly, float hy,
                                                    float lx, float hx)
{
    return hy * (hx * m[y0 * ld + x0] + lx * m[y0 * ld + x1]) + ly * (hx * m[y1 * ld + x0] + lx * m[y1 * ld + x1]);
}

__device__ __forceinline__ double stm_exp_f64(double x)
{
    if (x > 709.0) return __longlong_as_double(0x7FF0000000000000LL);
    if (x < -745.0) return 0.0;
    const double LOG2E = 1.4426950408889634074;
    const double LN2_HI = 6.93147180369123816490e-01;
    const double LN2_LO = 1.90821492927058770002e-10;
    double kf = rint(x * LOG2E);
    double r = fma(-kf, LN2_HI, x);
    r = fma(-kf, LN2_LO, r);
    double p = 1.0 / 6227020800.0;
    p = fma(p, r, 1.0 / 479001600.0);
    p = fma(p, r, 1.0 / 39916800.0);
    p = fma(p, r, 1.0 / 3628800.0);
    p = fma(p, r, 1.0 / 362880.0);
    p = fma(p, r, 1.0 / 40320.0);
    p = fma(p, r, 1.0 / 5040.0);
    p = fma(p, r, 1.0 / 720.0);
    p = fma(p, r, 1.0 / 120.0);
    p = fma(p, r, 1.0 / 24.0);
    p = fma(p, r, 1.0 / 6.0);
    p = fma(p, r, 0.5);
    p = fma(p, r, 1.0);
// ... 73 lines not shown
```

stmask_amd/ops.py:

```python
import ctypes
import os

import torch

from . import _lib
from ._lib import DeformGeom, StmError, c_f, c_i, c_l, c_p, c_sz, check


def _pair(v):
    return (v, v) if isinstance(v, int) else tuple(v)


def _dev(*ts):
    for t in ts:
        if t is not None and not t.is_cuda:
            raise StmError("stmask_amd ops need tensors on the MI355X (got a CPU tensor); there is no CPU fallback")


def _f32c(t):
    if t.dtype != torch.float32:
        raise StmError(f"expected float32, got {t.dtype}")
    return t if t.is_contiguous() else t.contiguous()


# ... 650 lines not shown
    g.win_h, g.win_w = out_h, out_w
    g.out_scale = out_scale
    g.x_np, g.x_plane_stride = xp.shape[2], xp.shape[1] * xp.shape[2] * 32
    wins = (_lib.ConvWindow * n)()
    for i, wv in enumerate(windows):
        wins[i].kh, wins[i].kw, wins[i].ph, wins[i].pw, wins[i].Ho, wins[i].Wo, wins[i].y0, wins[i].x0 = wv
    ptrs = (ctypes.c_void_p * n)(*[p.data_ptr() for p in packed_list])
    check(_lib.lib().stm_conv2d_planar_windows_pool_f32(_p(xp), ptrs, wins, c_i(n), _p(bias) if bias is not None else None, _p(pool_fix),
                                                        ctypes.byref(g), _stream()), "stm_conv2d_planar_windows_pool_f32")
    return pool_fix


def temporal_pool_fc(pool_fix, n, npix, weight, bias, n_first=None, clear=True, want_pooled=False):
    _dev(pool_fix, weight)
    if pool_fix.dtype != torch.int64 or pool_fix.dim() != 2 or not pool_fix.is_contiguous() or pool_fix.shape[0] < n or n < 0:
        raise StmError(f"temporal_pool_fc: pool_fix must be contiguous int64 [>= {n}, C], got {pool_fix.dtype} {tuple(pool_fix.shape)}")
    if weight.dim() != 2 or weight.shape[1] != pool_fix.shape[1] or (bias is not None and bias.numel() != weight.shape[0]):
        raise StmError(f"temporal_pool_fc: weight {tuple(weight.shape)} / bias do not match C = {pool_fix.shape[1]}")
    C, n_out = pool_fix.shape[1], weight.shape[0]
    weight = _f32c(weight)
    dev = pool_fix.device
    nf = n_out if n_first is None else int(n_first)
    out = torch.empty(n, nf, device=dev, dtype=torch.float32)
    out2 = torch.empty(n, n_out - nf, device=dev, dtype=torch.float32) if n_first is not None else None
    pooled = torch.empty(n, C, device=dev, dtype=torch.float32) if want_pooled else None
    check(_lib.lib().stm_temporal_pool_fc_f32(_p(pool_fix), c_i(n), c_i(C), c_i(npix), _p(weight), _p(_f32c(bias)) if bias is not None else None,
                                              c_i(n_out), c_i(nf), _p(out), _p(out2) if out2 is not None else None,
                                              _p(pooled) if pooled is not None else None, c_i(1 if clear else 0), _stream()),
          "stm_temporal_pool_fc_f32")
    res = (out, out2) if n_first is not None else (out,)
    if want_pooled:
        res = res + (pooled,)
    return res if len(res) > 1 else res[0]


def conv_kxr_supported(O, C, kh, kw, stride, padding, groups, group_cout, fmt, max_tiles=4):
    (sh, sw), (ph, pw) = _pair(stride), _pair(padding)
    if fmt not in (1, 2) or (sh, sw) != (1, 1) or kw not in (3, 5) or not (1 <= kh <= 8) or 2 * ph != kh - 1 or 2 * pw != kw - 1:
        return False
    if C % 32 or groups < 1 or groups > 4 or O % groups:
        return False
    cg = O // groups
    real = [(group_cout[i] if group_cout and 0 < group_cout[i] < cg else cg) for i in range(groups)]
    npl = 2 if fmt == 1 else 1
    for r in real:
        nc = -(-r // 16)
        if nc > max_tiles or 16 * nc > cg or cg % 4:
            return False
        if 3 * (npl * (64 * 2 + 16) * 64 + kw * npl * nc * 1024) > 160 * 1024:
            return False
    return True


def conv_pack_weights_kxr(weight, geom):
    _dev(weight)
    weight = _f32c(weight)
    nbytes = _lib.lib().stm_conv_kxr_packed_bytes(ctypes.byref(geom))
    if nbytes == 0:
        raise StmError("conv_pack_weights_kxr: " + _lib.lib().stm_last_error_string().decode(errors="replace"))
    packed = torch.empty(nbytes, device=weight.device, dtype=torch.uint8)
    import math
    wmax = float(weight.abs().max())
    wscale = 2.0 ** (10 - math.floor(math.log2(wmax))) if wmax > 0 else 1.0
    check(_lib.lib().stm_conv_pack_weights_kxr_f32(_p(weight), _p(packed), ctypes.byref(geom), c_f(wscale), _stream()),
          "stm_conv_pack_weights_kxr_f32")
    return packed, 1.0 / wscale


def _pow2_wscale(weight):
    import math
    wmax = float(weight.abs().max())
    return 2.0 ** (10 - math.floor(math.log2(wmax))) if wmax > 0 else 1.0


def chain_pack_tail(w3, w1_next=None, wds=None):
    _dev(w3)
    w3 = _f32c(w3.reshape(256, 64))
    if wds is not None:
        wds = _f32c(wds.reshape(256, 64))
    ws3 = _pow2_wscale(torch.cat([w3, wds], 1) if wds is not None else w3)
    ws1 = 1.0
    if w1_next is not None:
        w1_next = _f32c(w1_next.reshape(64, 256))
        ws1 = _pow2_wscale(w1_next)
    L = _lib.lib()
    packed = torch.zeros(L.stm_chain_tail_weight_bytes_proj() if wds is not None else L.stm_chain_tail_weight_bytes(), device=w3.device, dtype=torch.uint8)
    pw1 = _p(w1_next) if w1_next is not None else None
    if wds is not None:
        check(L.stm_chain_pack_tail_proj_f32(_p(w3), _p(wds), pw1, _p(packed), c_f(ws3), c_f(ws1), _stream()), "stm_chain_pack_tail_proj_f32")
    else:
        check(L.stm_chain_pack_tail_f32(_p(w3), pw1, _p(packed), c_f(ws3), c_f(ws1), _stream()), "stm_chain_pack_tail_f32")
    return packed, 1.0 / ws3, 1.0 / ws1


def bottleneck_chain(mid1, x, w2_packed, tail_packed, b2, b3, b1_next, scales, B, H, W, y=None, z=None, want_z=True, proj=False):
    _dev(mid1)
    n = B * H * W
    xs = 2 if proj else 8
    if tuple(mid1.shape) != (2, 2, n, 32) or tuple(x.shape) != (2, xs, n, 32) or mid1.dtype != torch.float16 or x.dtype != torch.float16:
        raise StmError(f"bottleneck_chain: planes {tuple(mid1.shape)} / {tuple(x.shape)} do not match [2, 2, {n}, 32] / [2, {xs}, {n}, 32] fp16")
    if not (mid1.is_contiguous() and x.is_contiguous()):
        raise StmError("bottleneck_chain: planes must be dense")
    if y is None:
        y = torch.empty(2, 8, n, 32, device=mid1.device, dtype=torch.float16)
    if want_z and z is None:
        z = torch.empty(2, 2, n, 32, device=mid1.device, dtype=torch.float16)
    s2, s3, s1 = scales
    fn = _lib.lib().stm_bottleneck_chain_proj_f32 if proj else _lib.lib().stm_bottleneck_chain_f32
    check(fn(_p(mid1), _p(x), _p(y), _p(z) if want_z else None, _p(w2_packed), _p(tail_packed),
             _p(b2) if b2 is not None else None, _p(b3) if b3 is not None else None,
             _p(b1_next) if (want_z and b1_next is not None) else None, c_f(s2), c_f(s3), c_f(s1),
             c_i(B), c_i(H), c_i(W), _stream()), "stm_bottleneck_chain_proj_f32" if proj else "stm_bottleneck_chain_f32")
    return y, (z if want_z else None)


def plane_layout(fmt):
# ... 335 lines not shown

def preprocess_frames_multi(frames, out=None, size=(640, 360), divisor=32, mean=(123.675, 116.28, 103.53), std=(58.395, 57.12, 57.375),
                            mode=1):
    frames = list(frames)
    if not frames:
        raise StmError("preprocess_frames_multi: no frames")
    _dev(*frames)
    w, h = size
    Hp, Wp = -(-h // divisor) * divisor, -(-w // divisor) * divisor
    n, dev = len(frames), frames[0].device
    desc = (_lib.FrameDesc * n)()
    keep = []
    for i, f in enumerate(frames):
        if f.dtype != torch.uint8 or f.dim() != 3 or f.shape[-1] != 3 or f.device != dev:
            raise StmError(f"preprocess_frames_multi: frame {i}: expected uint8 [H,W,3] on {dev}, got {f.dtype} {tuple(f.shape)} on {f.device}")
        if f.stride(2) != 1 or f.stride(1) != 3 or f.stride(0) < 3 * f.shape[1]:
            f = f.contiguous()
            keep.append(f)
        desc[i].ptr, desc[i].H0, desc[i].W0, desc[i].row_stride_bytes = f.data_ptr(), f.shape[0], f.shape[1], f.stride(0)
    if out is None:
        out = torch.empty(n, 3, Hp, Wp, device=dev, dtype=torch.float32)
    elif out.dtype != torch.float32 or tuple(out.shape) != (n, 3, Hp, Wp) or not out.is_contiguous() or out.device != dev:
        raise StmError(f"preprocess_frames_multi: out must be contiguous fp32 {(n, 3, Hp, Wp)} on {dev}, got {out.dtype} {tuple(out.shape)}")
    m3, s3 = (ctypes.c_double * 3)(*mean), (ctypes.c_double * 3)(*std)
    check(_lib.lib().stm_preprocess_u8_multi_f32(desc, c_i(n), _p(out), c_i(h), c_i(w), c_i(Hp), c_i(Wp), m3, s3, c_i(mode), _stream()),
          "stm_preprocess_u8_multi_f32")
    return out


def head_assemble(small, trk, B, sizes, n_cls, mask_dim, embed_dim, group_pad):
    _dev(*small, *trk)
    K = len(small)
    L = _lib.HeadLayout()
    L.B, L.K, L.n_levels, L.n_cls, L.mask_dim, L.embed_dim, L.group_pad = B, K, len(sizes), n_cls, mask_dim, embed_dim, group_pad
    L.small_ld, L.trk_ld = small[0].shape[-1], trk[0].shape[-1]
    start = 0
    for l, (h, w) in enumerate(sizes):
        L.lvl_start[l], L.lvl_hw[l] = start, h * w
        start += B * h * w
    N = K * sum(h * w for h, w in sizes)
    for t in list(small) + list(trk):
        if t.dtype != torch.float32 or not t.is_contiguous() or t.shape[0] != start:
            raise StmError("head_assemble: inputs must be contiguous fp32 matrices over all level pixels")
    dev = small[0].device
    conf = torch.empty(B, N, n_cls, device=dev)
    loc = torch.empty(B, N, 4, device=dev)
    mask = torch.empty(B, N, mask_dim, device=dev)
    track = torch.empty(B, N, embed_dim, device=dev)
    cen = torch.empty(B, N, 1, device=dev)
    sp = (ctypes.c_void_p * 4)(*([t.data_ptr() for t in small] + [0] * (4 - K)))
    tp = (ctypes.c_void_p * 4)(*([t.data_ptr() for t in trk] + [0] * (4 - K)))
    check(_lib.lib().stm_head_assemble_f32(sp, tp, ctypes.byref(L), _p(conf), _p(loc), _p(mask), _p(track), _p(cen), _stream()),
          "stm_head_assemble_f32")
    return conf, loc, mask, track, cen


def deform_conv_fused_supported(C, O, kernel_size, has_mask, fmt, deformable_groups=1):
    kh, kw = _pair(kernel_size)
    g = DeformGeom(1, C, 8, 8, kh, kw, 1, 1, kh // 2, kw // 2, 1, 1, deformable_groups, 8, 8)
    return bool(_lib.lib().stm_deform_conv_fused_planar_supported(ctypes.byref(g), c_i(O), c_i(1 if has_mask else 0), c_i(fmt)))


def deform_conv_fused_tiles(B, Ho, Wo, O):
    wide = O % 256 == 0 and os.environ.get("STM_DCN_FUSED_WIDE", "1") != "0"
    tp, bn = (64, 256) if wide else (128, 128)
    best, bt, bper = -1.0, 1, 1 << 30
    for tw in range(4, tp + 1):
        th = tp // tw
        if th < 1:
            break
        thc, twc = min(th, Ho), min(tw, Wo)
        tiles = -(-Ho // thc) * -(-Wo // twc)
        eff = Ho * Wo / (tiles * float(tp))
        per = thc + twc
        if eff > best + 1e-9 or (eff > best - 1e-9 and per < bper):
            best, bt, bper = eff, tiles, per
    return B * bt * (O // bn)


def deform_conv_fused_planar(x_pix, B, H, W, C, om, packed, out_scale, bias, O, kernel_size=3, stride=1, padding=1, dilation=1, has_mask=True,
                             relu=False, fmt=1, out_fmt=None, out=None, out_off=0):
    _dev(x_pix, om, packed)
    if x_pix.dtype != torch.float32 or x_pix.dim() != 2 or x_pix.stride(1) != 1 or x_pix.shape[0] != B * H * W or x_pix.shape[1] != C:
        raise StmError(f"deform_conv_fused_planar: x must be fp32 [B*H*W, C] with unit channel stride, got {tuple(x_pix.shape)} {x_pix.stride()}")
    om = _f32c(om)
    kh, kw = _pair(kernel_size)
    (sh, sw), (ph, pw), (dh, dw) = _pair(stride), _pair(padding), _pair(dilation)
    Ho, Wo = conv_out_hw(H, W, kh, kw, sh, sw, ph, pw, dh, dw)
    M, K = B * Ho * Wo, kh * kw
    if om.dim() != 2 or om.shape[0] != M or om.shape[1] < (3 if has_mask else 2) * K:
        raise StmError(f"deform_conv_fused_planar: offsets {tuple(om.shape)} do not match {M} output pixels x {(3 if has_mask else 2) * K}")
    out_fmt = fmt if out_fmt is None else out_fmt
    if out is None:
        out = _empty_planes(out_fmt, O // 32, M, x_pix.device)
        out_off = 0
    elif out.dim() != 4 or out.shape[1] * 32 != O or not out.is_contiguous() or out.shape[0] < plane_layout(out_fmt)[0]:
        raise StmError(f"deform_conv_fused_planar: planes {tuple(out.shape)} do not hold {O} channels in format {out_fmt}")
    if bias is not None:
        _dev(bias)
        bias = _f32c(bias)
    g = DeformGeom(B, C, H, W, kh, kw, sh, sw, ph, pw, dh, dw, 1, Ho, Wo)
    timing = _fused_dcn_timing
    if timing is not None:
        e0, e1 = torch.cuda.Event(enable_timing=True), torch.cuda.Event(enable_timing=True)
        e0.record()
    check(_lib.lib().stm_deform_conv_fused_planar_f32(_p(x_pix), c_i(x_pix.stride(0)), _p(om), c_i(om.shape[1]), c_i(1 if has_mask else 0), _p(packed),
# ... 34 lines not shown
```

stmask_amd/pipeline.py:

```python
import os

import torch
import torch.nn.functional as F

from . import ops
from .layers import Track_TF, generate_candidate
from .layers.box_utils import center_size, sanitize_coordinates_hw

ROI_CHUNKS = (256, 128, 64)


class _StageTimer:

    def __init__(self):
        import os
        self.on = os.environ.get("STM_PIPE_TIMING", "0") == "1"
        self.acc, self.t0 = {}, None

    def tic(self):
        if self.on:
            import time
            torch.cuda.synchronize()
            self.t0 = time.perf_counter()

# ... 105 lines not shown
            torch.cuda.synchronize(dev)
            t0 = time.perf_counter()
            for s_ in streams:
                with torch.cuda.stream(s_):
                    spin(cycles)
            torch.cuda.synchronize(dev)
            return time.perf_counter() - t0

        run([main])
        base = min(run([main]) for _ in range(3))
        for c in cands:
            if len(chosen) == n:
                break
            if min(run([main] + chosen + [c]) for _ in range(2)) < 1.4 * base:
                chosen.append(c)
    for c in cands:
        if len(chosen) == n:
            break
        if c not in chosen:
            chosen.append(c)
    _SIDE_STREAMS[key] = chosen
    return chosen[:n]


def trunk_stream_count():
    return max(2, BatchedClipPipeline.PREFETCH_DEPTH)


class BatchedClipPipeline:

    def __init__(self, net, n_clips):
        self.net, self.cfg, self.B = net, net.cfg, n_clips
        self.tf = bool(self.cfg.temporal_fusion_module)
        self.range_fallback = True
        self.fell_back = False
        self._last = None
        self.t = 0
        self.prev = None
        self.prev_n = [0] * n_clips
        self.prev_feat = None
        self.has_prev = [False] * n_clips
        self.tracked = [[] for _ in range(n_clips)]
        self.timer = _StageTimer()
        self._pending = []
        self._sides = []
        self._side_next = 0
        self.prefetch_early = True
        self.use_graph = False
        self.graph_active = False
        self._graphs = []
        self._graph_next = 0
        self._graph_warm = 0
        self._graph_ws = []
        self._graph_planes = None
        self._idle_masks = {}
        self._idle_dev = None
        self.max_instances = 0

    def _shift_prev(self, P4, T2S, proto, dev):
        net, cfg, prev = self.net, self.cfg, self.prev
        clip_of_row = prev["clip"]
        P4_prev, T2S_prev = self.prev_feat
        P = cfg.correlation_patch_size
        fh, fw = P4.shape[2:]
        box_ref = prev["box"]
        rois = ops.shift_rois(box_ref, clip_of_row, fh, fw)
        ptn = getattr(net, "_planar_temporal", None)
        a_prev, a_cur = T2S_prev.permute(0, 2, 3, 1), T2S.permute(0, 2, 3, 1)
        fused = (ptn is not None and ptn.ncorr == P * P and a_prev.is_contiguous() and a_cur.is_contiguous()
                 and 2 * T2S.shape[1] + P * P == ptn.cin)
        if fused:
            n = rois.shape[0]
            corr = ops.corr_patch_nhwc(P4_prev, P4, P, scale=1.0 / P4.shape[1], leaky_slope=0.1)
            xp = ops.roi_align_planes(a_prev, a_cur, corr, rois, 7, fmt=ptn.fmt, corr_nhwc=P * P)
            self.timer.toc("tf_corr_roi")
            loc_shift, coeff_shift = ptn.forward_planes(xp, n)
        else:
            corr = ops.corr_patch(P4_prev, P4, P, 1, scale=1.0 / P4.shape[1], leaky_slope=0.1)
            corr = corr.view(P4.shape[0], P * P, P4.shape[2], P4.shape[3])
            feats = F.relu(torch.cat([corr, T2S_prev, T2S], dim=1))
            roi_feats = ops.roi_align(feats, rois, 7)
            self.timer.toc("tf_corr_roi")
            n = roi_feats.shape[0]
        if fused:
            pass
        elif ptn is not None:
            loc_shift, coeff_shift = ptn(roi_feats)
        else:
            n_pad = -(-n // ROI_CHUNKS[-1]) * ROI_CHUNKS[-1]
            if n_pad != n:
                roi_feats = torch.cat([roi_feats, roi_feats.new_zeros(n_pad - n, *roi_feats.shape[1:])], 0)
            outs, i = [], 0
            while i < n_pad:
                c = next(c for c in ROI_CHUNKS if c <= n_pad - i)
                outs.append(net.TemporalNet(roi_feats[i:i + c]))
                i += c
            loc_shift = torch.cat([o[0] for o in outs], 0)[:n]
            coeff_shift = torch.cat([o[1] for o in outs], 0)[:n]
        self.timer.toc("tf_temporalnet")
        ops.shift_apply_(loc_shift, coeff_shift, prev["box"], prev["mask_coeff"], prev["score"], 0.95)
        prev["mask"], self._prev_bits = ops.lincomb_sigmoid_crop_bits(proto, prev["mask_coeff"], prev["box"], clip_of_row)
        self.timer.toc("tf_masks")
        for b in range(self.B):
            self.tracked[b] = [v + 1 for v in self.tracked[b]]

    PREFETCH_DEPTH = int(os.environ.get("STM_PREFETCH_DEPTH", "3"))
    N_GRAPH_SLOTS = 2 * PREFETCH_DEPTH + 2
    LARGE_BATCH = 8

    @property
    def prefetch_depth(self):
        return self.PREFETCH_DEPTH if self.B <= self.LARGE_BATCH else min(self.PREFETCH_DEPTH, 2)

    @property
    def n_graph_slots(self):
        return 2 * self.prefetch_depth + 2

    def _trunk(self, frames):
        net = self.net
        if not (self.use_graph and getattr(net, "_planar", None) is not None and not self.timer.on and ops._conv_timing is None
                and ops._im2col_timing is None):
            return net.forward_single(frames)
        planes = getattr(net, "_planar_planes", None)
        if self._graphs and self._graph_planes != planes:
            self._pending = []
            torch.cuda.synchronize()
            self._graphs, self._graph_next, self.graph_active, self._graph_warm, self._graph_ws = [], 0, False, 0, []
        if self._graph_warm < 2:
            self._graph_warm += 1
            return net.forward_single(frames)
        if len(self._graphs) < self.n_graph_slots:
            reserved0 = torch.cuda.memory_reserved(frames.device)
            static_in = frames.clone(memory_format=torch.preserve_format)
            graph = torch.cuda.CUDAGraph()
            ws = {}
            self._graph_ws.append(ws)
            cur = torch.cuda.current_stream()
            cap = torch.cuda.Stream(device=frames.device)
            cap.wait_stream(cur)
            with ops.workspace_scope(ws):
                with torch.cuda.stream(cap):
                    net.forward_single(static_in)
                with torch.cuda.graph(graph, stream=cap):
                    out = net.forward_single(static_in)
            cur.wait_stream(cap)
            if not self._graphs:
                slot_bytes = max(torch.cuda.memory_reserved(frames.device) - reserved0, 0)
                free = torch.cuda.mem_get_info(frames.device)[0] + torch.cuda.memory_reserved(frames.device) - torch.cuda.memory_allocated(frames.device)
                if (self.n_graph_slots - 1) * slot_bytes > 0.9 * free:
                    import sys
                    sys.stderr.write(f"stmask_amd: {self.n_graph_slots} trunk-graph slots of {slot_bytes / 1e9:.1f} GB do not fit in {free / 1e9:.1f} GB of free HBM: "
                                     "this pipeline keeps the eager trunk\n")
                    del graph, out, static_in
                    self._graph_ws.pop()
                    self.use_graph = False
                    torch.cuda.synchronize()
                    torch.cuda.empty_cache()
                    return net.forward_single(frames)
            self._graphs.append((static_in, graph, out))
            self._graph_planes = planes
            self.graph_active = True
        static_in, graph, out = self._graphs[self._graph_next]
        self._graph_next = (self._graph_next + 1) % self.n_graph_slots
        if static_in.shape != frames.shape:
            raise ops.StmError("BatchedClipPipeline: the frame batch changed shape under a captured trunk graph")
        static_in.copy_(frames)
        graph.replay()
        return out

    def _prefetch_trunk(self, next_frames):
        if next_frames is None or self.timer.on:
            return
        nxt = list(next_frames) if isinstance(next_frames, (list, tuple)) else [next_frames]
        depth = self.prefetch_depth if (self.use_graph and self.graph_active) else 1
        main = torch.cuda.current_stream()
        for f in nxt[:depth]:
            if f is None or any(p[0] is f for p in self._pending):
                continue
            if not self._sides:
                self._sides = concurrent_side_streams(f.device, trunk_stream_count())
            side = self._sides[self._side_next]
            self._side_next = (self._side_next + 1) % len(self._sides)
            side.wait_stream(main)
            with torch.cuda.stream(side):
                out = self._trunk(f)
                ev = torch.cuda.Event()
                ev.record()
            self._pending.append((f, out, ev))

    def _take_trunk(self, frames):
        net = self.net
        dropped = False
        while self._pending and self._pending[0][0] is not frames:
            torch.cuda.current_stream().wait_event(self._pending.pop(0)[2])
            dropped = True
        if self._pending:
            _, (fpn_outs, pred), ev = self._pending.pop(0)
            torch.cuda.current_stream().wait_event(ev)
            if not self.graph_active:
                for t_ in list(pred.values()) + list(fpn_outs):
                    if torch.is_tensor(t_):
                        t_.record_stream(torch.cuda.current_stream())
                t2s_ = pred["T2S_feat"][net.correlation_selected_layer] if isinstance(pred.get("T2S_feat"), (list, tuple)) and self.tf else None
                if torch.is_tensor(t2s_):
                    t2s_.record_stream(torch.cuda.current_stream())
        else:
            fpn_outs, pred = self._trunk(frames)
        return fpn_outs, pred, dropped

    def _detect(self, pred):
        cfg, net = self.cfg, self.net
        priors = pred["priors"].squeeze(0)
        det = net.Detect_TF if self.tf else net.detect
# ... 387 lines not shown
```

stmask_amd/planar.py:

```python
import ctypes
import os

import torch
import torch.nn.functional as F

from . import _lib, ops
from ._lib import StmError, c_i, check


def _pair(v):
    return (v, v) if isinstance(v, int) else tuple(v)


FMT = 0
BACKBONE_FMT = None

TILE64_MAX_SLABS = 8
FCB_PLANAR = True
STEM_PLANAR = True
C3DS_FUSED = True
STEM_FUSED = True
CONV_KXR = True
TN_BORDER = True
TN_POOL = True
CONV_CHAIN = True
DCN_FUSED = os.environ.get("STM_DCN_FUSED", "1") != "0"
DCN_FUSED_MIN_TILES = int(os.environ.get("STM_DCN_FUSED_MIN_TILES", "200"))
DCN_FUSED_RULE = 0
FCB_FUSED = os.environ.get("STM_FCB_FUSED", "1") != "0"
TRUNK_BRANCHES = 0
BRANCH_MAX_IMAGES = 16
CHAIN_MODE = int(os.environ.get("STM_CHAIN_MODE", "3"))
CHAIN_MAX_PIXELS = (1 << 21) - 1


def set_format(fmt, backbone_fmt=None):
    global FMT, BACKBONE_FMT
    if fmt not in (0, 1, 2) or backbone_fmt not in (None, 0, 1, 2):
        raise StmError("planar format must be 0 (bf16 x 3), 1 (fp16 x 2) or 2 (fp16 x 1)")
    if backbone_fmt is not None and backbone_fmt != fmt and (backbone_fmt, fmt) != (2, 1):
        raise StmError("a backbone format different from the graph's is only built for fp16x1 under fp16x2")
    FMT, BACKBONE_FMT = fmt, backbone_fmt


def _planes_dtype(fmt):
    return ops.plane_layout(fmt)


class PlanarConv:

    SPLITK_WS_BYTES = 64 << 20

    def __init__(self, weight, bias, stride=1, padding=0, relu=False, groups=1, planes=3, algo_frac=1.0, tile_n=None,
                 group_cout=None, fmt=None, out_fmt=None):
        self.weight = weight.detach().float().contiguous()
        self.fmt = FMT if fmt is None else fmt
        self.out_fmt = self.fmt if out_fmt is None else out_fmt
        self.algo_frac = algo_frac
        self.group_cout = list(group_cout) if group_cout else None
        self.O, self.C, self.kh, self.kw = self.weight.shape
        (self.sh, self.sw), (self.ph, self.pw) = _pair(stride), _pair(padding)
        self.relu, self.groups, self.planes, self.tile_n = relu, groups, (planes if self.fmt == 0 else ops.plane_layout(self.fmt)[0]), tile_n
        self._packed = {}
        self.out_scale = 1.0
        self.role = "trunk"
        self.kxr = CONV_KXR and self.out_fmt == self.fmt and ops.conv_kxr_supported(self.O, self.C, self.kh, self.kw, (self.sh, self.sw), (self.ph, self.pw),
                                                                                     self.groups, self.group_cout, self.fmt, max_tiles=3)
        self.kxr_min_pixels = None
        self.bias = bias.detach().float().contiguous() if bias is not None else None

    def packed(self, tile_n):
        if tile_n not in self._packed:
            if self.fmt >= 1:
                ops.planar_range_flag()
                self._packed[tile_n], self.out_scale = ops.conv_pack_weights(self.weight, tile_n=tile_n, fmt=self.fmt)
            else:
                self._packed[tile_n] = ops.conv_pack_weights(self.weight, self.planes, tile_n)
        return self._packed[tile_n]

    def pick_tile(self, M):
        if self.tile_n is not None:
            return self.tile_n
        cg = self.O // self.groups
        if self.groups > 1 and cg % 128 != 0:
            return 64
        if cg <= 64 or (cg % 128 != 0 and cg % 128 <= 64 and cg < 256):
            return 64
        tiles128 = -(-M // 128) * -(-self.O // 128)
        slabs = self.C * self.kh * self.kw // 32
        if tiles128 < 400 and not (192 <= tiles128 <= 256 and slabs >= 64):
            return 64
        if slabs <= TILE64_MAX_SLABS:
            return 64
        return 128

    def __call__(self, xp, shape, out="planes", x_off=0, out_planes=None, out_f32=None, out_off=0, residual=None, x_ch_off=0,
                 out_ch_off=0, x2=None, window=None):
        NP, dt = _planes_dtype(self.fmt)
        if xp.dtype != dt or xp.dim() != 4 or xp.shape[0] < NP or xp.shape[3] != 32 or not xp.is_contiguous():
            raise StmError(f"PlanarConv: expected contiguous {dt} planes [{NP}, S, N, 32], got {xp.dtype} {tuple(xp.shape)}")
        S, N = xp.shape[1], xp.shape[2]
        g = _lib.ConvGeom()
        g.C, g.Cout, g.kh, g.kw, g.sh, g.sw, g.ph, g.pw = self.C, self.O, self.kh, self.kw, self.sh, self.sw, self.ph, self.pw
        g.planes, g.groups = self.planes, self.groups
        if self.group_cout:
            for i, c in enumerate(self.group_cout):
                g.group_cout[i] = c
        c_first = self.C - (x2[0].shape[1] * 32 if x2 is not None else 0)
        if S * 32 < x_ch_off + self.groups * c_first or x_ch_off % 32:
            raise StmError(f"PlanarConv: input has {S * 32} channels, layer reads {self.groups} x {c_first} from channel {x_ch_off}")
        if shape[0] == "levels":
            _, B, sizes = shape
            g.n_levels = len(sizes)
            start = 0
            for l, (h, w) in enumerate(sizes):
                g.lvl_start[l], g.lvl_h[l], g.lvl_w[l] = start, h, w
                start += B * h * w
            g.lvl_start[len(sizes)] = start
            M = start
            if x_off or N != start:
                raise StmError("PlanarConv: a multi-level launch covers the whole plane buffer")
        else:
            _, B, H, W = shape
            Ho, Wo = ops.conv_out_hw(H, W, self.kh, self.kw, self.sh, self.sw, self.ph, self.pw, 1, 1)
            out_rows = None
            if window is not None:
                y0, x0, Ho, Wo, g.ph, g.pw, fh, fw = window
                g.win_h, g.win_w, g.win_y0, g.win_x0 = fh, fw, y0, x0
                out_rows = B * fh * fw
                if residual is not None or x2 is not None:
                    raise StmError("PlanarConv: window launches take no residual / second source")
            g.B, g.H, g.W, g.Ho, g.Wo = B, H, W, Ho, Wo
            M = B * Ho * Wo
            if x_off + B * H * W > N:
                raise StmError("PlanarConv: input slice runs past the plane buffer")
        g.x_np, g.x_plane_stride = N, S * N * 32
        use_kxr = (self.kxr and residual is None and window is None and (shape[0] == "levels" or (Ho, Wo) == (H, W))
                   and M >= (self.kxr_min_pixels if self.kxr_min_pixels is not None else (20000 if self.groups > 1 else 30000)))
        g.tile_n = 0 if use_kxr else self.pick_tile(M)
        dev = xp.device
        NPo, dto = _planes_dtype(self.out_fmt)
        if window is not None and ((out in ("planes", "both") and out_planes is None) or (out in ("f32", "both") and out_f32 is None)):
            raise StmError("PlanarConv: a window launch writes into caller-provided full-size outputs")
        if out in ("planes", "both") and out_planes is None:
            out_planes, out_off_p = torch.empty(NPo, -(-self.O // 32), M, 32, device=dev, dtype=dto), 0
        else:
            out_off_p = out_off
        if out in ("f32", "both") and out_f32 is None:
            out_f32, out_off_f = torch.empty(M, self.O, device=dev, dtype=torch.float32), 0
        else:
            out_off_f = out_off
        if out == "planes":
            out_f32 = None
        if out == "f32":
            out_planes = None
        p_pl = p_f32 = 0
        if out_planes is not None:
            g.out_np, g.out_plane_stride = out_planes.shape[2], out_planes.shape[1] * out_planes.shape[2] * 32
            p_pl = out_planes.data_ptr() + out_off_p * 64
        if out_f32 is not None:
            g.out_ld = out_f32.shape[-1]
            p_f32 = out_f32.data_ptr() + (out_off_f * g.out_ld + out_ch_off) * 4
        r32 = rpl = 0
        if residual is not None:
            if residual.dtype == dt:
                if residual.shape[0] < NP:
                    raise StmError(f"PlanarConv: residual has {residual.shape[0]} plane(s), format {self.fmt} reads {NP}")
                g.res_np, g.res_plane_stride = residual.shape[2], residual.shape[1] * residual.shape[2] * 32
                rpl = residual.data_ptr()
            else:
                g.res_ld = residual.shape[-1]
                r32 = residual.data_ptr()
        timing = ops._conv_timing
        if timing is not None:
            e0, e1 = torch.cuda.Event(enable_timing=True), torch.cuda.Event(enable_timing=True)
            e0.record()
        x_ptr = xp.data_ptr() + ((x_ch_off // 32) * N + x_off) * 64
        if use_kxr:
            g.fmt = self.fmt
            if "kxr" not in self._packed:
                ops.planar_range_flag()
                self._packed["kxr"] = ops.conv_pack_weights_kxr(self.weight, g)
            packed, g.out_scale = self._packed["kxr"]
            rc = _lib.lib().stm_conv2d_planar_kxr_f32(ctypes.c_void_p(x_ptr), ops._p(packed), ops._p(self.bias), ctypes.c_void_p(p_f32),
                                                      ctypes.c_void_p(p_pl), ctypes.byref(g), c_i(1 if self.relu else 0), ops._stream())
            check(rc, "stm_conv2d_planar_kxr_f32")
            return self._finish(timing, e0 if timing is not None else None, M, shape, g, NP, NPo, dt, out, out_f32, out_planes, residual)
        packed = self.packed(g.tile_n)
        g.fmt, g.out_scale = self.fmt, self.out_scale
        g.out_fmt_plus1 = 0 if self.out_fmt == self.fmt else self.out_fmt + 1
        ws = ops._workspace(self.SPLITK_WS_BYTES, dev, "conv_splitk")
        if x2 is not None:
            p2, H2, W2, s2 = x2
            if p2.dtype != dt or p2.dim() != 4 or p2.shape[0] < NP or p2.shape[3] != 32 or not p2.is_contiguous() or shape[0] != "img":
                raise StmError("PlanarConv: the second source must be contiguous planes of this layer's format over one image size")
            rc = _lib.lib().stm_conv2d_planar_dual_f32(ctypes.c_void_p(x_ptr), ops._p(p2), c_i(p2.shape[1] * 32), c_i(H2), c_i(W2), c_i(s2),
                                                       ctypes.c_longlong(p2.shape[2]), ctypes.c_longlong(p2.shape[1] * p2.shape[2] * 32),
                                                       ops._p(packed), ops._p(self.bias), ctypes.c_void_p(r32), ctypes.c_void_p(rpl),
                                                       ctypes.c_void_p(p_f32), ctypes.c_void_p(p_pl), ctypes.byref(g), c_i(1 if self.relu else 0),
                                                       ops._p(ws), ctypes.c_size_t(ws.numel()), ops._stream())
            check(rc, "stm_conv2d_planar_dual_f32")
            return self._finish(timing, e0 if timing is not None else None, M, shape, g, NP, NPo, dt, out, out_f32, out_planes, residual)
        rc = _lib.lib().stm_conv2d_planar_ws_f32(ctypes.c_void_p(x_ptr), ops._p(packed),
                                                 ops._p(self.bias), ctypes.c_void_p(r32), ctypes.c_void_p(rpl),
                                                 ctypes.c_void_p(p_f32), ctypes.c_void_p(p_pl), ctypes.byref(g),
                                                 c_i(1 if self.relu else 0), ops._p(ws), ctypes.c_size_t(ws.numel()),
                                                 ops._stream())
        check(rc, "stm_conv2d_planar_f32")
        return self._finish(timing, e0 if timing is not None else None, M, shape, g, NP, NPo, dt, out, out_f32, out_planes, residual)

    def deform(self, x32, B, H, W, om, stride, padding, dilation, has_mask, out=None, out_off=0):
        packed = self.packed(128)
        return ops.deform_conv_fused_planar(x32, B, H, W, self.C, om, packed, self.out_scale, self.bias, self.O, (self.kh, self.kw), stride, padding,
                                            dilation, has_mask=has_mask, relu=self.relu, fmt=self.fmt, out_fmt=self.out_fmt, out=out, out_off=out_off)

    def _finish(self, timing, e0, M, shape, g, NP, NPo, dt, out, out_f32, out_planes, residual):
        if timing is not None:
            e1 = torch.cuda.Event(enable_timing=True)
            e1.record()
            in_px = M if shape[0] == "levels" else shape[1] * shape[2] * shape[3]
            nbytes = in_px * self.groups * self.C * 2 * NP + self.weight.numel() * 2 * NP
            if out_planes is not None:
                nbytes += M * self.O * 2 * NPo
            if out_f32 is not None:
                nbytes += M * self.O * 4
            if residual is not None:
                nbytes += M * self.O * (2 * NP if residual.dtype == dt else 4)
            timing.append((e0, e1, 2.0 * M * self.O * self.C * self.kh * self.kw * self.algo_frac,
                           (M, self.C, self.O, self.kh, self.sh, self.groups, g.tile_n),
                           {0: 6 if self.planes == 3 else 3, 1: 3, 2: 1}[self.fmt], self.role, float(nbytes)))
        if out == "both":
            return out_f32, out_planes
        return out_f32 if out == "f32" else out_planes


def _nhwc(t):
    return t.permute(0, 2, 3, 1).contiguous()


def _split(t_nhwc, fmt=None):
    return ops.split_planes(t_nhwc, FMT if fmt is None else fmt)


class PlanarGraph:
    GROUP_PAD = 64

    def __init__(self, net):
        cfg = net.cfg
        self.net = net
        self.fmt = FMT
        fpn = net.fpn
        self.n_lat = len(fpn.lat_layers)
        self.fpn_pred = [PlanarConv(m.weight, m.bias, m.stride, m.padding, relu=True) for m in fpn.pred_layers]
        self.fpn_down = [PlanarConv(m.weight, m.bias, m.stride, m.padding, relu=False) for m in fpn.downsample_layers]
        self.fpn_lat = [PlanarConv(m.weight, m.bias, 1, 0, relu=False) for m in fpn.lat_layers]
        self.proto = []
        mods = [m for m in net.proto_net.children() if not isinstance(m, (torch.nn.ReLU, torch.nn.Identity))]
        for m in mods:
            if isinstance(m, torch.nn.Conv2d):
# ... 11 lines not shown
        up = convs(head.upfeature)
        assert len(up) == 1
        self.up = PlanarConv(up[0].weight, up[0].bias, 1, up[0].padding, relu=True)
        towers = [convs(head.conf_extra), convs(head.bbox_extra), convs(head.mask_extra), convs(head.track_extra)]
        assert all(len(t) == 2 for t in towers), "extra_layers (2,2,2,2) is the only head layout on the hot path"
        w1 = torch.cat([t[0].weight for t in towers], 0)
        b1 = torch.cat([t[0].bias for t in towers], 0)
        self.tower1 = PlanarConv(w1, b1, 1, towers[0][0].padding, relu=True)
        w2 = torch.cat([t[1].weight for t in towers], 0)
        b2 = torch.cat([t[1].bias for t in towers], 0)
        self.tower2 = PlanarConv(w2, b2, 1, towers[0][1].padding, relu=True, groups=4)
        self.finals = []
        P = self.GROUP_PAD
        self.dims = (head.num_priors * head.num_classes, head.num_priors * 4, head.num_priors * head.mask_dim,
                     head.num_priors * head.embed_dim)
        for k in range(len(cfg.head_layer_params)):
            mods = [[head.centerness_layer[k], head.bbox_layer[k]], [head.mask_layer[k]]]
            if not self.fcb:
                mods = [[head.conf_layer[k]]] + mods
            ws, bs = [], []
            for grp in mods:
                w = torch.cat([m.weight for m in grp], 0)
                b = torch.cat([m.bias for m in grp], 0)
                assert w.shape[0] <= P
                ws.append(F.pad(w, (0, 0, 0, 0, 0, 0, 0, P - w.shape[0])))
                bs.append(F.pad(b, (0, P - b.shape[0])))
            m0 = mods[0][0]
            real = sum(m.weight.shape[0] for grp in mods for m in grp)
            small = PlanarConv(torch.cat(ws, 0), torch.cat(bs, 0), 1, m0.padding, relu=False, groups=len(mods),
                               algo_frac=real / (len(mods) * float(P)), tile_n=64,
                               group_cout=[sum(m.weight.shape[0] for m in grp) for grp in mods])
            tr = head.track_layer[k]
            entry = [small, PlanarConv(tr.weight, tr.bias, 1, tr.padding, relu=False)]
            if self.fcb:
                fa = head.conf_layer[k]
                entry.append(fa)
                n_c = fa.conv.weight.shape[0]
                n_cp = -(-n_c // 16) * 16
                assert n_cp <= P
                entry.append(PlanarConv(F.pad(fa.conv.weight, (0, 0, 0, 0, 0, 0, 0, n_cp - n_c)), F.pad(fa.conv.bias, (0, n_cp - n_c)), 1, fa.conv.padding,
                                        relu=False, tile_n=64, group_cout=[n_c], algo_frac=n_c / n_cp))
                ad = fa.conv_adaption
                O, Cin, akh, akw = ad.weight.shape
                if ad.deform_groups == 1 and Cin == 256 and akh * akw in (9, 15):
                    wk = ad.weight.detach().permute(0, 2, 3, 1).reshape(O, akh * akw * Cin, 1, 1)
                    entry.append(PlanarConv(wk, None, 1, 0, relu=True))
                    entry.append(PlanarConv(ad.weight, None, 1, fa.padding, relu=True)
                                 if DCN_FUSED and FCB_FUSED and self.fmt in (1, 2) and ops.deform_conv_fused_supported(Cin, O, (akh, akw), False, self.fmt) else None)
                else:
                    entry.append(None)
                    entry.append(None)
            self.finals.append(tuple(entry))
        self.head = head

    def run(self, bb_outs, planes=None):
        net, fpn = self.net, self.net.fpn
        n = self.n_lat
        toc = self.timer.toc if self.timer is not None else (lambda name: None)
        toc("backbone")
        lat, latp, x = [None] * n, [None] * n, None
        if planes is not None:
            B = planes[0][1]
            sizes = [(h, w) for (_, _, h, w) in planes]
            for i, conv in enumerate(self.fpn_lat):
                j = n - 1 - i
                h, w = sizes[j]
                res = None
                if x is not None:
                    if fpn.interpolation_mode == "bilinear":
                        res = ops.resize_bilinear_planes(x, (h, w), self.fmt)
                    else:
                        up = F.interpolate(x.permute(0, 3, 1, 2), size=(h, w), mode=fpn.interpolation_mode)
                        res = _nhwc(up).view(-1, conv.O)
                if j > 0:
                    y32, latp[j] = conv(planes[j][0], ("img", B, h, w), out="both", residual=res)
                    x = y32.view(B, h, w, conv.O)
                else:
                    latp[j] = conv(planes[j][0], ("img", B, h, w), out="planes", residual=res)
        else:
            B = bb_outs[0].shape[0]
            for i, layer in enumerate(fpn.lat_layers):
                j = n - 1 - i
                lateral = layer(bb_outs[j])
                if x is None:
                    x = lateral
                else:
                    h, w = bb_outs[j].shape[2:]
                    x = F.interpolate(x, size=(h, w), mode=fpn.interpolation_mode, align_corners=False) + lateral
                lat[j] = x
            sizes = [tuple(t.shape[2:]) for t in lat]
        toc("fpn_lateral")
        for d in self.fpn_down:
            h, w = sizes[-1]
            sizes.append(ops.conv_out_hw(h, w, d.kh, d.kw, d.sh, d.sw, d.ph, d.pw, 1, 1))
        starts = [0]
        for h, w in sizes:
            starts.append(starts[-1] + B * h * w)
        ntot, nf = starts[-1], self.fpn_pred[0].O
        dev = (latp[0] if latp[0] is not None else lat[0]).device
        NP, pdt = _planes_dtype(self.fmt)
        feat = torch.empty(NP, nf // 32, ntot, 32, device=dev, dtype=pdt)
        feat32 = torch.empty(ntot, nf, device=dev, dtype=torch.float32) if not self.head_planar else None
        fpn_outs = [None] * len(sizes)

        def pred_level(i):
            conv = self.fpn_pred[i]
# ... 49 lines not shown
                if isinstance(layer, PlanarConv):
                    nxt_is_interp = (not last) and not isinstance(self.proto[li + 1], PlanarConv)
                    if cur is not None:
                        xp, x_off = _split(cur, self.fmt), 0
                        cur = None
                    if last or nxt_is_interp:
                        y = layer(xp, ("img", B, h, w), out="f32", x_off=x_off)
                        cur = y.view(B, h, w, layer.O)
                    else:
                        xp, x_off = layer(xp, ("img", B, h, w), out="planes", x_off=x_off), 0
                else:
                    kw = layer.kwargs
                    sf = kw.get("scale_factor")
                    nxt_conv = (not last) and isinstance(self.proto[li + 1], PlanarConv)
                    if (nxt_conv and not layer.args and kw.get("mode") == "bilinear" and not kw.get("align_corners", False)
                            and isinstance(sf, (int, float)) and float(sf).is_integer() and set(kw) <= {"scale_factor", "mode", "align_corners"}):
                        h, w = h * int(sf), w * int(sf)
                        xp, x_off, cur = ops.resize_bilinear_planes(cur, (h, w), self.fmt), 0, None
                    else:
                        t = layer(cur.permute(0, 3, 1, 2))
                        h, w = t.shape[2:]
                        cur = _nhwc(t)
            return cur

        proto_side = side is not None and TRUNK_BRANCHES >= 1 and self.head_planar
        if proto_side:
            main = torch.cuda.current_stream()
            side.wait_stream(main)
            with torch.cuda.stream(side), ops.workspace_branch("proto"):
                proto = proto_net()
        else:
            proto = proto_net()
        toc("proto_net")

        keys = ("mask_coeff", "priors", "loc", "T2S_feat", "centerness", "conf", "track")
        pred = {k: [] for k in keys}
        if not self.head_planar:
            for idx, layer in zip(net.selected_layers, net.prediction_layers):
                p = layer(fpn_outs[idx])
                for k in keys:
                    pred[k].append(p[k])
            for k in keys:
                if k != "T2S_feat":
                    pred[k] = torch.cat(pred[k], 1)
            pred["proto"] = proto
            return fpn_outs, pred

        lv = ("levels", B, sizes)
        head = self.head
        if self.cor_idx is not None:
            up32, up = self.up(feat, lv, out="both")
        else:
            up32, up = None, self.up(feat, lv, out="planes")
        t1 = self.tower1(up, lv, out="planes")
        cw = self.tower2.O // 4
        P = self.GROUP_PAD
        if not self.fcb:
            t2 = self.tower2(t1, lv, out="planes")
            toc("head_towers")
            outs = [(small(t2, lv, out="f32"), trk(t2, lv, out="f32", x_ch_off=3 * cw)) for small, trk in self.finals]
        else:
            t2_32, t2 = self.tower2(t1, lv, out="both")
            toc("head_towers")
            conf_x = None
            outs = []
            for small, trk, fa, fconv, adconv, adfused in self.finals:
                buf = torch.empty(ntot, 3 * P, device=dev, dtype=torch.float32)
                small(t2, lv, out="f32", out_f32=buf, x_ch_off=cw, out_ch_off=P)
                npri = head.num_priors
                if adconv is not None and npri == 1 and FCB_PLANAR:
                    kh, kw = fa.kernel_size
                    K = kh * kw
                    bbox_pix = buf[:, P + npri:P + npri + 4]
                    if fa.use_pred_offset:
                        off = bbox_pix @ fa.conv_offset.weight.view(2 * K, 4).t()
                    NP_, pdt_ = _planes_dtype(self.fmt)
                    n_fused = 0
                    if adfused is not None:
                        while n_fused < len(sizes) and ops.deform_conv_fused_tiles(B, sizes[n_fused][0], sizes[n_fused][1], adfused.O) >= DCN_FUSED_MIN_TILES:
                            n_fused += 1
                    c0 = starts[n_fused]
                    feat_pl = torch.empty(NP_, cw // 32, ntot, 32, device=dev, dtype=pdt_)
                    cols = torch.empty(NP_, K * cw // 32, ntot - c0, 32, device=dev, dtype=pdt_) if ntot > c0 else None
                    for l, (hh, ww) in enumerate(sizes):
                        sl = slice(starts[l], starts[l + 1])
                        if fa.use_pred_offset:
                            off_l = off[sl]
                        else:
                            loc_l = bbox_pix[sl].reshape(B, hh, ww, 4).permute(0, 3, 1, 2).contiguous()
                            off_l = ops.fcb_ali_offsets(loc_l, kh, kw).permute(0, 2, 3, 1).reshape(-1, 2 * K)
                        if l < n_fused:
                            adfused.deform(t2_32[sl, 0:cw], B, hh, ww, off_l, 1, fa.padding, 1, has_mask=False, out=feat_pl, out_off=starts[l])
                        else:
                            ops.deform_sample_planar(t2_32[sl, 0:cw], B, hh, ww, cw, off_l, (kh, kw), fa.padding, cols, starts[l] - c0, self.fmt)
                    if cols is not None:
                        adconv(cols, ("img", 1, 1, ntot - c0), out_planes=feat_pl, out_off=c0)
                    fconv(feat_pl, lv, out="f32", out_f32=buf)
                    outs.append((buf, trk(t2, lv, out="f32", x_ch_off=3 * cw)))
                    continue
                if conf_x is None:
                    conf_x = [t2_32[starts[l]:starts[l + 1], 0:cw].reshape(B, hh, ww, cw).permute(0, 3, 1, 2).contiguous()
                              for l, (hh, ww) in enumerate(sizes)]
                feat_k = torch.empty(ntot, cw, device=dev, dtype=torch.float32)
                for l, (hh, ww) in enumerate(sizes):
                    sl = slice(starts[l], starts[l + 1])
                    bbox_cur = buf[sl, P + npri:P + npri + 4 * npri].reshape(B, hh, ww, 4 * npri).permute(0, 3, 1, 2).contiguous()
                    if fa.use_pred_offset:
                        offset = fa.conv_offset(bbox_cur)
                    else:
                        offset = ops.fcb_ali_offsets(bbox_cur, fa.kernel_size[0], fa.kernel_size[1])
                    y = ops.deform_conv(conf_x[l], offset, None, fa.conv_adaption.weight, None, 1, fa.padding, 1,
                                        fa.conv_adaption.deform_groups, relu=True)
                    feat_k[sl] = y.permute(0, 2, 3, 1).reshape(-1, cw)
                fconv(ops.split_planes(feat_k, self.fmt), lv, out="f32", out_f32=buf)
                outs.append((buf, trk(t2, lv, out="f32", x_ch_off=3 * cw)))
        toc("head_finals")
        P = self.GROUP_PAD
        ncls, nbox, nmask, ntrk = self.dims
        npri = head.num_priors
        t2s = [None] * len(sizes)
        if up32 is not None:
            l = self.cor_idx
            t2s[l] = up32[starts[l]:starts[l + 1]].view(B, *sizes[l], -1).permute(0, 3, 1, 2)
        for hh, ww in sizes:
            pred["priors"].append(head.make_priors(hh, ww, dev))
        pred["priors"] = torch.cat(pred["priors"], 1)
        if npri == 1:
            conf, loc, mask, track, cen = ops.head_assemble([o[0] for o in outs], [o[1] for o in outs], B, sizes,
                                                            head.num_classes, head.mask_dim, head.embed_dim, P)
            pred["conf"], pred["loc"], pred["mask_coeff"], pred["track"], pred["centerness"] = conf, loc, mask, track, cen
        else:
            conf, loc, mask, track, cen = [], [], [], [], []
            for l, (hh, ww) in enumerate(sizes):
                sl = slice(starts[l], starts[l + 1])
                per_k = [o[0][sl].view(B, hh * ww, 3 * P) for o in outs]
                cat = torch.stack(per_k, dim=2)
                conf.append(cat[..., 0:ncls].reshape(B, -1, head.num_classes))
                loc.append(cat[..., P + npri:P + npri + nbox].reshape(B, -1, 4))
                mask.append(cat[..., 2 * P:2 * P + nmask].reshape(B, -1, head.mask_dim))
                track.append(torch.stack([o[1][sl].view(B, hh * ww, ntrk) for o in outs], dim=2).reshape(B, -1, head.embed_dim))
                cen.append(torch.stack([pk[..., P:P + npri] for pk in per_k], dim=1).reshape(B, -1, 1))
            pred["conf"] = torch.cat(conf, 1)
            pred["loc"] = torch.cat(loc, 1)
            pred["mask_coeff"] = torch.cat(mask, 1)
            pred["track"] = F.normalize(torch.cat(track, 1), dim=-1)
            pred["centerness"] = torch.tanh(torch.cat(cen, 1))
        pred["T2S_feat"] = t2s
        pred["proto"] = proto
        if proto_side:
            torch.cuda.current_stream().wait_stream(side)
        toc("head_assemble")
        return fpn_outs, pred

    def _side_stream(self, dev, n_images):
        if TRUNK_BRANCHES <= 0 or n_images > BRANCH_MAX_IMAGES or self.timer is not None and self.timer.on:
            return None
        if not torch.cuda.is_current_stream_capturing():
            return None
        if getattr(self, "_side", None) is None or self._side.device != torch.device(dev):
            self._side = torch.cuda.Stream(device=dev)
        return self._side


_BORDER_CLASSES = [(ry, rx, k0y, k1y, k0x, k1x) for ry, (k0y, k1y) in enumerate(((1, 3), (0, 3), (0, 2)))
                   for rx, (k0x, k1x) in enumerate(((1, 3), (0, 3), (0, 2)))]


def border_windows(h, w):
    rows, cols = ((0, 1), (1, h - 1), (h - 1, h)), ((0, 1), (1, w - 1), (w - 1, w))
    out = []
    for ci, (ry, rx, k0y, k1y, k0x, k1x) in enumerate(_BORDER_CLASSES):
        (y0, y1), (x0, x1) = rows[ry], cols[rx]
        if y1 <= y0 or x1 <= x0:
            continue
        out.append((ci, (k1y - k0y, k1x - k0x, 1 - y0 - k0y, 1 - x0 - k0x, y1 - y0, x1 - x0, y0, x0)))
    return out


class PlanarTemporalNet:

# ... 293 lines not shown
```

Before: 1629.

## Add sparse detection head that runs box/mask towers only around confident pixels

Result: faster. 1767 (median of 6 runs) (+8.5%).

```diff
diff --git a/include/stmask_hip.h b/include/stmask_hip.h
--- a/include/stmask_hip.h
+++ b/include/stmask_hip.h
@@ -253,6 +253,20 @@
 int stm_head_assemble_f32(const float* const* small, const float* const* trk, const stm_head_layout* layout, float* conf,
                           float* loc, float* mask, float* track, float* centerness, stm_stream_t stream);
 
+void stm_conv_set_pixel_gate(const int* valid_pixels);
+int stm_head_candidates_f32(const float* const* cls_logits, int K, int ld, int n_cls, float conf_thresh, int capacity,
+                            int patch_pixels_a, int patch_pixels_b, int n_levels, int B, const int* lvl_start, const int* lvl_h,
+                            const int* lvl_w, int* flags, int* list, int* ctl, stm_stream_t stream);
+int stm_head_patch_gather(const void* src_planes, long long src_np, void* dst_planes, int side, int n_planes, int slabs,
+                          int capacity, int n_levels, int B, const int* lvl_start, const int* lvl_h, const int* lvl_w, const int* list,
+                          const int* ctl, stm_stream_t stream);
+int stm_head_patch_mask(void* planes, int side, int n_planes, int slabs, int capacity, int n_levels, int B, const int* lvl_start,
+                        const int* lvl_h, const int* lvl_w, const int* list, const int* ctl, stm_stream_t stream);
+int stm_head_assemble_sparse_f32(const float* const* cls_logits, int cls_ld, const float* const* small, const float* const* trk,
+                                 const float* const* small_dense, const float* const* trk_dense, const stm_head_layout* layout,
+                                 int row_mul, int row_add, const int* list, const int* ctl, int capacity, float* conf, float* loc,
+                                 float* mask, float* track, float* centerness, stm_stream_t stream);
+
 int stm_dcn_sample_planar_f32(const float* x, const float* offset_mask, int om_ld, void* planes, int out_np,
                               long long out_plane_stride, const stm_deform_geom* g, stm_stream_t stream);
 int stm_resize_bilinear_planes_f32(const float* x, void* planes, int B, int H, int W, int C, int Ho, int Wo, int fmt,
diff --git a/stmask_amd/_lib.py b/stmask_amd/_lib.py
--- a/stmask_amd/_lib.py
+++ b/stmask_amd/_lib.py
@@ -24,6 +24,7 @@
     "stm_deform_conv_fused_planar_supported", "stm_deform_conv_fused_planar_f32", "stm_fast_nms_batched_workspace_bytes", "stm_fast_nms_batched_f32", "stm_rle_strings_host",
     "stm_preprocess_u8_multi_f32", "stm_render_workspace_bytes", "stm_render_overlay_u8",
     "stm_deform_col2im_f32", "stm_deform_col2im_coord_f32", "stm_roi_align_backward_f32", "stm_corr_backward_f32",
+    "stm_conv_set_pixel_gate", "stm_head_candidates_f32", "stm_head_patch_gather", "stm_head_patch_mask", "stm_head_assemble_sparse_f32",
 ]
 
 
diff --git a/stmask_amd/csrc/capi.hip b/stmask_amd/csrc/capi.hip
--- a/stmask_amd/csrc/capi.hip
+++ b/stmask_amd/csrc/capi.hip
@@ -28,6 +28,15 @@
         case 5: return sizeof(stm_render_frame);
         default: return 0;
     }
+}
+
+static thread_local const int* g_pixel_gate = nullptr;
+extern "C" void stm_conv_set_pixel_gate(const int* valid_pixels) { g_pixel_gate = valid_pixels; }
+const int* stm_internal_take_pixel_gate()
+{
+    const int* g = g_pixel_gate;
+    g_pixel_gate = nullptr;
+    return g;
 }
 
 static std::atomic<int> g_env_gen{0};
diff --git a/stmask_amd/csrc/conv_bf16x.hip b/stmask_amd/csrc/conv_bf16x.hip
--- a/stmask_amd/csrc/conv_bf16x.hip
+++ b/stmask_amd/csrc/conv_bf16x.hip
@@ -75,6 +75,7 @@
     unsigned plane2_bytes;
     int c1_slabs, x2_np, H2, W2, s2;
     int win_w, win_hw, win_off;
+    const int* m_gate;
 };
 struct PlanarArgsCls : PlanarArgs {
     int n_cls, cls_tiles;
@@ -326,8 +327,10 @@
 
     int tiles_ = a_in.m_tiles * a_in.n_tiles * a_in.splitk;
     if constexpr (CLS) tiles_ = a_in.cls_tiles;
+    else if (a_in.m_gate) tiles_ = min(a_in.m_tiles, (*a_in.m_gate + BM - 1) / BM) * a_in.n_tiles;
     const int tiles = tiles_;
     const int per_xcd = (tiles + 7) >> 3;
+    if (!CLS && a_in.m_gate && (int)(blockIdx.x >> 3) >= per_xcd) return;
     int logical = (blockIdx.x & 7) * per_xcd + (blockIdx.x >> 3);
     auto regroup = [&](int j, int nt_all, int& mt_o, int& nt_o) {
         const int pg = 32 / a_in.nsub, G = pg * nt_all;
@@ -370,6 +373,7 @@
     const int nt = tile - mt * a.n_tiles;
     const int m0 = mt * BM;
     if (m0 >= a.M) return;
+    if (a.m_gate && m0 >= *a.m_gate) return;
     const int s_begin = ksp * a.kslabs, s_end = min(a.slabs, s_begin + a.kslabs);
 
     const int tid = threadIdx.x, lane = tid & 63;
@@ -794,8 +798,9 @@
             if (i < a_in.n_cls && logical >= a_in.cls[i].tile0) cls_c = i;
         logical -= a_in.cls[cls_c].tile0;
     } else {
-        const int tiles = a_in.m_tiles * n_tiles_;
+        const int tiles = (a_in.m_gate ? min(a_in.m_tiles, (*a_in.m_gate + BM - 1) / BM) : a_in.m_tiles) * n_tiles_;
         const int per_xcd = (tiles + 7) >> 3;
+        if (a_in.m_gate && (int)(blockIdx.x >> 3) >= per_xcd) return;
         logical = (blockIdx.x & 7) * per_xcd + (blockIdx.x >> 3);
         if (logical >= tiles) return;
     }
@@ -809,6 +814,7 @@
     const int mt = n_tiles_ == 1 ? logical : (n_tiles_ == 2 ? logical >> 1 : (n_tiles_ == 4 ? logical >> 2 : logical / n_tiles_));
     const int nt = logical - mt * n_tiles_;
     const int m0 = mt * BM;
+    if (a.m_gate && m0 >= *a.m_gate) return;
     const int tid = threadIdx.x, lane = tid & 63;
     const int wave = __builtin_amdgcn_readfirstlane(tid >> 6);
     const int wm = wave & 3, wn = wave >> 2;
@@ -1855,6 +1861,7 @@
                        int relu, void* workspace, size_t workspace_bytes, stm_stream_t stream, const DualSrc* dual, const WinSet* wset)
 {
     const char* who = dual ? "stm_conv2d_planar_dual_f32" : "stm_conv2d_planar_f32";
+    const int* const gate = stm_internal_take_pixel_gate();
     STM_REQUIRE(x_planes && packed_weight && (out_f32 || out_planes || (wset && wset->pool)), STM_ENULL,
                 "%s: x_planes/packed_weight and at least one output must be non-NULL", who);
     STM_REQUIRE(g, STM_ENULL, "%s: geometry is NULL", who);
@@ -1947,6 +1954,8 @@
     STM_REQUIRE(g->planes == want_planes || (a.fmt == 0 && g->planes == 2), STM_EINVAL, "%s: format %d has %d planes (planes = %d)", who, a.fmt,
                 want_planes, g->planes);
     a.splitk = 1; a.kslabs = a.slabs; a.partial = nullptr; a.ldp = a.n_tiles * bn;
+    a.m_gate = gate;
+    STM_REQUIRE(!gate || !wset, STM_EUNSUPPORTED, "%s: window sets take no pixel gate", who);
     a.xp2 = nullptr; a.x2_pstride = 0; a.plane2_bytes = 0; a.c1_slabs = a.slabs; a.x2_np = 0; a.H2 = a.W2 = 0; a.s2 = 1;
     if (dual) {
         const int64_t in2 = (int64_t)g->B * dual->H2 * dual->W2;
@@ -1961,6 +1970,7 @@
     bool full = cout_g % 64 == 0;
     for (int gi = 0; gi < groups && gi < 8; ++gi) full = full && a.group_real[gi] == cout_g;
     auto plan_splitk = [&](int tiles) {
+        if (a.m_gate) return;
         int sk = tn.splitk;
         if (sk <= 0) {
             sk = 1;
@@ -2061,7 +2071,7 @@
     const int mg = tn.mg ? tn.mg : (t2 >= 192 ? 2 : 1);
     a.m_tiles = stm_cdiv(M, CV_BM * mg);
     plan_splitk(a.m_tiles * a.n_tiles);
-    a.nsub = ((tn.nsub == 2 || tn.nsub == 4) && a.splitk == 1 && a.n_tiles > tn.nsub && a.n_tiles % tn.nsub == 0 && g->groups == 1 &&
+    a.nsub = ((tn.nsub == 2 || tn.nsub == 4) && a.splitk == 1 && !a.m_gate && a.n_tiles > tn.nsub && a.n_tiles % tn.nsub == 0 && g->groups == 1 &&
               a.m_tiles >= 4 * (32 / tn.nsub)) ? tn.nsub : 0;
     if (a.nsub) a.m_tiles = stm_cdiv(a.m_tiles, 32 / a.nsub) * (32 / a.nsub);
     const int tiles = a.m_tiles * a.n_tiles * a.splitk;
diff --git a/stmask_amd/csrc/conv_kxr.hip b/stmask_amd/csrc/conv_kxr.hip
--- a/stmask_amd/csrc/conv_kxr.hip
+++ b/stmask_amd/csrc/conv_kxr.hip
@@ -54,6 +54,8 @@
     int* range_flag;
     int n_lvl;
     int lvl_start[9], lvl_h[8], lvl_w[8];
+    const int* m_gate;
+    int M;
 };
 
 typedef __attribute__((address_space(3))) void* lds_ptr;
@@ -83,12 +85,31 @@
     static_assert(BM + HALO <= XROWS - 1, "the always-zero row must exist");
     static_assert(D >= 2 && D * BUF <= KX_LDS_MAX && (D - 2) * NPD <= 63, "ring does not fit");
 
+    auto gated_per_xcd = [&]() {
+        int per = jb.per_xcd;
+        if (a.m_gate) {
+            const int gate = *a.m_gate;
+            if (gate < a.M) per = ((gate + BM - 1) / BM + 7) >> 3;
+        }
+        return per;
+    };
+    if (a.m_gate) {
+        const int gate = *a.m_gate;
+        if (gate < a.M) {
+            const int gt = (gate + BM - 1) / BM;
+            const int per = (gt + 7) >> 3;
+            const int j0 = tile_first >> 3, st = tile_step >> 3;
+            const int jend = min(per, gt - (tile_first & 7) * per);
+            n_seq = j0 >= jend ? 0 : min(n_seq, (jend - j0 + st - 1) / st);
+        }
+        if (n_seq <= 0) return;
+    }
     const int tid = threadIdx.x, lane = tid & 63;
     const int wave = __builtin_amdgcn_readfirstlane(tid >> 6);
     const int S = a.cslabs * a.kh;
     struct TileGeo { int H, W, lstart, lend, m0; };
     auto tile_geo = [&](int id) {
-        const int tile = (id & 7) * jb.per_xcd + (id >> 3);
+        const int tile = (id & 7) * gated_per_xcd() + (id >> 3);
         int lvl = 0;
 #pragma unroll
         for (int l = 1; l < 8; ++l)
@@ -475,6 +496,7 @@
                                          const stm_conv_geom* g, int relu, stm_stream_t stream)
 {
     const char* who = "stm_conv2d_planar_kxr_f32";
+    const int* const gate = stm_internal_take_pixel_gate();
     STM_REQUIRE(x_planes && packed_weight && (out_f32 || out_planes), STM_ENULL, "%s: x_planes/packed_weight and at least one output must be non-NULL", who);
     KxrPlan pl;
     if (!kxr_plan(g, &pl, who)) return STM_EINVAL;
@@ -540,6 +562,7 @@
                 a.out_fmt, g->fmt);
     a.out_scale = g->out_scale > 0.0f ? g->out_scale : 1.0f;
     a.range_flag = stm_internal_range_flag();
+    a.m_gate = gate; a.M = (int)M;
     (void)nc_max;
     if (g->fmt == 1) return g->kw == 3 ? kxr_launch<3, 2>(a, stream) : kxr_launch<5, 2>(a, stream);
     return g->kw == 3 ? kxr_launch<3, 1>(a, stream) : kxr_launch<5, 1>(a, stream);
diff --git a/stmask_amd/csrc/head_sparse.hip b/stmask_amd/csrc/head_sparse.hip
--- /dev/null
+++ b/stmask_amd/csrc/head_sparse.hip
@@ -0,0 +1,416 @@
+#include <algorithm>
+
+#include "stm_common.h"
+
+namespace {
+
+enum { CTL_RAW = 0,
+       CTL_N = 1,
+       CTL_FILL = 2,
+       CTL_GATE_A = 3,
+       CTL_GATE_B = 4,
+       CTL_DENSE = 5,
+       CTL_OVERFLOW = 6,
+       CTL_INTS = 8 };
+
+struct Levels {
+    int n, B;
+    int start[9], h[8], w[8];
+};
+
+__device__ __forceinline__ void decode_pixel(const Levels& L, int m, int& l, int& b, int& y, int& x)
+{
+    l = 0;
+#pragma unroll
+    for (int i = 1; i < 8; ++i)
+        if (i < L.n && m >= L.start[i]) l = i;
+    const int r = m - L.start[l], hw = L.h[l] * L.w[l];
+    b = r / hw;
+    const int p = r - b * hw;
+    y = p / L.w[l];
+    x = p - y * L.w[l];
+}
+
+struct CandArgs {
+    const float* cls[4];
+    int K, ld, n_cls, n_pixels, capacity;
+    float thresh;
+    int* list;
+    int* ctl;
+    int* flags;
+    Levels L;
+};
+
+__global__ __launch_bounds__(256) void head_clear_kernel(int* ctl, int* flags, int n_pixels)
+{
+    const int i = blockIdx.x * 256 + threadIdx.x;
+    if (i < n_pixels) flags[i] = 0;
+    else if (i < n_pixels + CTL_INTS) ctl[i - n_pixels] = 0;
+}
+
+__device__ __forceinline__ void list_pixel(const CandArgs& a, int m)
+{
+    if (atomicCAS(a.flags + m, 0, 1) != 0) return;
+    const int i = atomicAdd(a.ctl + CTL_RAW, 1);
+    if (i < a.capacity) a.list[i] = m;
+}
+
+constexpr int CAND_PX = 64;
+
+__global__ __launch_bounds__(256) void head_candidates_kernel(const CandArgs a, int vec)
+{
+    extern __shared__ float slab[];
+    __shared__ unsigned kept_s[CAND_PX];
+    const int stride = a.n_cls | 1;
+    const int m0 = blockIdx.x * CAND_PX;
+    const int rows = min(CAND_PX, a.n_pixels - m0);
+    if (threadIdx.x < CAND_PX) kept_s[threadIdx.x] = 0u;
+    for (int k = 0; k < a.K; ++k) {
+        const float* src = a.cls[k] + (int64_t)m0 * a.ld;
+        float* dst = slab + k * CAND_PX * stride;
+        if (vec) {
+            const int nv = (a.n_cls + 3) >> 2;
+            for (int idx = threadIdx.x; idx < rows * nv; idx += 256) {
+                const int r = idx / nv, v = idx - r * nv;
+                const float4 q = *reinterpret_cast<const float4*>(src + (int64_t)r * a.ld + 4 * v);
+                float* d = dst + r * stride + 4 * v;
+                d[0] = q.x;
+                if (4 * v + 1 < a.n_cls) d[1] = q.y;
+                if (4 * v + 2 < a.n_cls) d[2] = q.z;
+                if (4 * v + 3 < a.n_cls) d[3] = q.w;
+            }
+        } else {
+            for (int idx = threadIdx.x; idx < rows * a.n_cls; idx += 256) {
+                const int r = idx / a.n_cls, c = idx - r * a.n_cls;
+                dst[r * stride + c] = src[(int64_t)r * a.ld + c];
+            }
+        }
+    }
+    __syncthreads();
+    const int k = threadIdx.x / CAND_PX, r = threadIdx.x - k * CAND_PX;
+    if (k < a.K && r < rows) {
+        const float* row = slab + (k * CAND_PX + r) * stride;
+        float mf = row[1];
+        for (int c = 2; c < a.n_cls; ++c) mf = row[c] > mf ? row[c] : mf;
+        const float mx = row[0] > mf ? row[0] : mf;
+        float sum = 0.0f;
+        for (int c = 0; c < a.n_cls; ++c) sum += expf(row[c] - mx);
+        const float p = expf(mf - mx) / sum;
+        if (p > a.thresh) atomicOr(&kept_s[r], 1u << k);
+    }
+    __syncthreads();
+    if (threadIdx.x >= rows) return;
+    const unsigned kept = kept_s[threadIdx.x];
+    if (!kept) return;
+    const int m = m0 + threadIdx.x;
+    list_pixel(a, m);
+    int l, b, y, x;
+    decode_pixel(a.L, m, l, b, y, x);
+    const int hw = a.L.h[l] * a.L.w[l], pix = y * a.L.w[l] + x;
+    for (int kk = 0; kk < a.K; ++kk)
+        if (kept >> kk & 1) list_pixel(a, a.L.start[l] + b * hw + (pix * a.K + kk) % hw);
+}
+
+__global__ void head_control_kernel(int* ctl, int capacity, int n_pixels, int px_a, int px_b)
+{
+    if (threadIdx.x || blockIdx.x) return;
+    const int raw = ctl[CTL_RAW];
+    const bool over = raw > capacity;
+    const int n = over ? 0 : raw;
+    const int fill = min(capacity, (n + 255) & ~255);
+    ctl[CTL_N] = n;
+    ctl[CTL_FILL] = fill;
+    ctl[CTL_GATE_A] = fill * px_a;
+    ctl[CTL_GATE_B] = fill * px_b;
+    ctl[CTL_DENSE] = over ? n_pixels : 0;
+    ctl[CTL_OVERFLOW] = over ? 1 : 0;
+}
+
+struct GatherArgs {
+    const uint8_t* src;
+    uint8_t* dst;
+    int rows;
+    int64_t src_np, dst_np;
+    int S;
+    const int* list;
+    const int* ctl;
+    Levels L;
+};
+
+__global__ __launch_bounds__(256) void head_patch_gather_kernel(const GatherArgs a)
+{
+    const int n = a.ctl[CTL_N], fill = a.ctl[CTL_FILL];
+    const int SS = a.S * a.S, half = a.S >> 1;
+    const int row_groups = (a.rows + 15) >> 4;
+    const int64_t units = (int64_t)fill * SS * row_groups;
+    const int lane = threadIdx.x & 63;
+    const int sub_row = lane >> 2, chunk = lane & 3;
+    for (int64_t u = (int64_t)blockIdx.x * 4 + (threadIdx.x >> 6); u < units; u += (int64_t)gridDim.x * 4) {
+        const int64_t pp = u / row_groups;
+        const int rg = (int)(u - pp * row_groups);
+        const int i = (int)(pp / SS), q = (int)(pp - (int64_t)i * SS);
+        const int row = rg * 16 + sub_row;
+        if (row >= a.rows) continue;
+        uint4 v = make_uint4(0u, 0u, 0u, 0u);
+        if (i < n) {
+            int l, b, y, x;
+            decode_pixel(a.L, a.list[i], l, b, y, x);
+            const int dy = q / a.S - half, dx = q - (q / a.S) * a.S - half;
+            const int yy = y + dy, xx = x + dx;
+            if ((unsigned)yy < (unsigned)a.L.h[l] && (unsigned)xx < (unsigned)a.L.w[l]) {
+                const int64_t sp = (int64_t)a.L.start[l] + ((int64_t)b * a.L.h[l] + yy) * a.L.w[l] + xx;
+                v = *reinterpret_cast<const uint4*>(a.src + ((int64_t)row * a.src_np + sp) * 64 + chunk * 16);
+            }
+        }
+        *reinterpret_cast<uint4*>(a.dst + ((int64_t)row * a.dst_np + pp) * 64 + chunk * 16) = v;
+    }
+}
+
+__global__ __launch_bounds__(256) void head_patch_mask_kernel(uint8_t* planes, int rows, int64_t np, int S, const int* list, const int* ctl, const Levels L)
+{
+    const int n = ctl[CTL_N];
+    const int SS = S * S, half = S >> 1;
+    for (int i = blockIdx.x; i < n; i += gridDim.x) {
+        int l, b, y, x;
+        decode_pixel(L, list[i], l, b, y, x);
+        if (y - half >= 0 && y + half < L.h[l] && x - half >= 0 && x + half < L.w[l]) continue;
+        const int work = SS * rows * 4;
+        for (int t = threadIdx.x; t < work; t += 256) {
+            const int chunk = t & 3, r = (t >> 2) % rows, q = (t >> 2) / rows;
+            const int yy = y + q / S - half, xx = x + q % S - half;
+            if ((unsigned)yy < (unsigned)L.h[l] && (unsigned)xx < (unsigned)L.w[l]) continue;
+            *reinterpret_cast<uint4*>(planes + ((int64_t)r * np + (int64_t)i * SS + q) * 64 + chunk * 16) = make_uint4(0u, 0u, 0u, 0u);
+        }
+    }
+}
+
+struct AsmArgs {
+    const float* cls[4];
+    const float* small[4];
+    const float* trk[4];
+    float *conf, *loc, *mask, *track, *cen;
+    int B, K, n_levels, n_cls, mask_dim, embed, gpad, cls_ld, small_ld, trk_ld, N;
+    int lvl_start[9], lvl_hw[8], lvl_off[8];
+    int vec4;
+    int row_mul, row_add;
+    const int* list;
+    const int* ctl;
+    int capacity;
+};
+
+__device__ __forceinline__ void assemble_rest(const AsmArgs& a, const float* sm, const float* tk, int64_t o, int64_t cen_idx, int sub)
+{
+    if (sub < 4) a.loc[o * 4 + sub] = sm[1 + sub];
+    for (int c = sub; c < a.mask_dim; c += 16) a.mask[o * a.mask_dim + c] = sm[a.gpad + c];
+    if (sub == 0) a.cen[cen_idx] = tanhf(sm[0]);
+    float ss = 0.0f;
+    if (a.vec4) {
+        typedef float f4 __attribute__((ext_vector_type(4)));
+        f4 v[4];
+        const int nv = a.embed >> 2;
+#pragma unroll
+        for (int q = 0; q < 4; ++q) {
+            const int c4 = sub + 16 * q;
+            if (c4 < nv) {
+                v[q] = *reinterpret_cast<const f4*>(tk + 4 * c4);
+                ss = fmaf(v[q].x, v[q].x, ss); ss = fmaf(v[q].y, v[q].y, ss); ss = fmaf(v[q].z, v[q].z, ss); ss = fmaf(v[q].w, v[q].w, ss);
+            }
+        }
+#pragma unroll
+        for (int d = 8; d >= 1; d >>= 1) ss += __shfl_xor(ss, d);
+        const float inv = 1.0f / fmaxf(sqrtf(ss), 1e-12f);
+#pragma unroll
+        for (int q = 0; q < 4; ++q) {
+            const int c4 = sub + 16 * q;
+            if (c4 < nv) *reinterpret_cast<f4*>(a.track + o * a.embed + 4 * c4) = v[q] * inv;
+        }
+    } else {
+        for (int c = sub; c < a.embed; c += 16) { const float v = tk[c]; ss = fmaf(v, v, ss); }
+#pragma unroll
+        for (int d = 8; d >= 1; d >>= 1) ss += __shfl_xor(ss, d);
+        const float inv = 1.0f / fmaxf(sqrtf(ss), 1e-12f);
+        for (int c = sub; c < a.embed; c += 16) a.track[o * a.embed + c] = tk[c] * inv;
+    }
+}
+
+template <int MODE>
+__global__ __launch_bounds__(256) void head_assemble_rows_kernel(const AsmArgs a)
+{
+    if (MODE == 1 && a.ctl[CTL_OVERFLOW] == 0) return;
+    const int sub = threadIdx.x & 15;
+    const int64_t row = (int64_t)stm_xcd_block(((int64_t)a.B * a.N + 15) >> 4) * 16 + (threadIdx.x >> 4);
+    if (row < 0 || row >= (int64_t)a.B * a.N) return;
+    const int b = (int)(row / a.N), n = (int)(row - (int64_t)b * a.N);
+    int l = 0;
+#pragma unroll
+    for (int i = 1; i < 8; ++i)
+        if (i < a.n_levels && n >= a.lvl_off[i]) l = i;
+    const int r = n - a.lvl_off[l];
+    const int p = r / a.K, k = r - p * a.K;
+    const int hw = a.lvl_hw[l];
+    const int64_t src = (int64_t)a.lvl_start[l] + (int64_t)b * hw + p;
+    const int64_t o = (int64_t)b * a.N + n;
+    if (MODE == 0) {
+        const float* cl = a.cls[k] + src * a.cls_ld;
+        for (int c = sub; c < a.n_cls; c += 16) a.conf[o * a.n_cls + c] = cl[c];
+    } else {
+        assemble_rest(a, a.small[k] + src * a.small_ld, a.trk[k] + src * a.trk_ld, o, (int64_t)b * a.N + a.lvl_off[l] + (int64_t)k * hw + p, sub);
+    }
+}
+
+__global__ __launch_bounds__(256) void head_assemble_listed_kernel(const AsmArgs a)
+{
+    const int n_pos = a.ctl[CTL_N];
+    const int sub = threadIdx.x & 15;
+    const int64_t units = (int64_t)n_pos * a.K;
+    for (int64_t u = (int64_t)blockIdx.x * 16 + (threadIdx.x >> 4); u < units; u += (int64_t)gridDim.x * 16) {
+        const int i = (int)(u / a.K), k = (int)(u - (int64_t)i * a.K);
+        const int m = a.list[i];
+        int l = 0;
+#pragma unroll
+        for (int j = 1; j < 8; ++j)
+            if (j < a.n_levels && m >= a.lvl_start[j]) l = j;
+        const int hw = a.lvl_hw[l];
+        const int rr = m - a.lvl_start[l];
+        const int b = rr / hw, p = rr - b * hw;
+        const int nn = a.lvl_off[l] + p * a.K + k;
+        const int64_t o = (int64_t)b * a.N + nn;
+        const int64_t src = (int64_t)i * a.row_mul + a.row_add;
+        assemble_rest(a, a.small[k] + src * a.small_ld, a.trk[k] + src * a.trk_ld, o, (int64_t)b * a.N + a.lvl_off[l] + (int64_t)k * hw + p, sub);
+    }
+}
+
+bool fill_levels(Levels& L, int n_levels, int B, const int* lvl_start, const int* lvl_h, const int* lvl_w)
+{
+    if (n_levels <= 0 || n_levels > 8 || B <= 0 || !lvl_start || !lvl_h || !lvl_w || lvl_start[0] != 0) return false;
+    L.n = n_levels; L.B = B;
+    for (int l = 0; l < 8; ++l) {
+        L.start[l] = l < n_levels ? lvl_start[l] : 0;
+        L.h[l] = l < n_levels ? lvl_h[l] : 1;
+        L.w[l] = l < n_levels ? lvl_w[l] : 1;
+        if (l < n_levels && (lvl_h[l] <= 0 || lvl_w[l] <= 0 || lvl_start[l + 1] - lvl_start[l] != B * lvl_h[l] * lvl_w[l])) return false;
+    }
+    L.start[8] = 0;
+    L.start[n_levels] = lvl_start[n_levels];
+    return true;
+}
+
+}
+
+extern "C" int stm_head_candidates_f32(const float* const* cls_logits, int K, int ld, int n_cls, float conf_thresh, int capacity,
+                                       int patch_pixels_a, int patch_pixels_b, int n_levels, int B, const int* lvl_start, const int* lvl_h,
+                                       const int* lvl_w, int* flags, int* list, int* ctl, stm_stream_t stream)
+{
+    const char* who = "stm_head_candidates_f32";
+    STM_REQUIRE(cls_logits && list && ctl && flags, STM_ENULL, "%s: NULL argument", who);
+    CandArgs a;
+    STM_REQUIRE(fill_levels(a.L, n_levels, B, lvl_start, lvl_h, lvl_w), STM_EINVAL, "%s: bad level table", who);
+    const int n_pixels = a.L.start[n_levels];
+    STM_REQUIRE(K > 0 && K <= 4 && n_cls >= 2 && ld >= n_cls && n_pixels > 0 && capacity > 0 && patch_pixels_a > 0 && patch_pixels_b > 0 &&
+                    (int64_t)capacity * std::max(patch_pixels_a, patch_pixels_b) < ((int64_t)1 << 30), STM_EINVAL, "%s: bad sizes", who);
+    for (int k = 0; k < 4; ++k) {
+        a.cls[k] = k < K ? cls_logits[k] : nullptr;
+        STM_REQUIRE(k >= K || a.cls[k], STM_ENULL, "%s: input %d is NULL", who, k);
+    }
+    a.K = K; a.ld = ld; a.n_cls = n_cls; a.n_pixels = n_pixels; a.capacity = capacity; a.thresh = conf_thresh; a.list = list; a.ctl = ctl;
+    a.flags = flags;
+    hipLaunchKernelGGL(head_clear_kernel, dim3(stm_cdiv(n_pixels + CTL_INTS, 256)), dim3(256), 0, stm_hs(stream), ctl, flags, n_pixels);
+    STM_CHECK_LAUNCH("head_clear_kernel");
+    int vec = ld % 4 == 0 && 4 * ((n_cls + 3) / 4) <= ld;
+    for (int k = 0; k < K; ++k) vec = vec && ((uintptr_t)a.cls[k] % 16) == 0;
+    const size_t lds = (size_t)K * CAND_PX * (n_cls | 1) * sizeof(float);
+    STM_REQUIRE(lds <= 48 * 1024, STM_EUNSUPPORTED, "%s: %d classes x %d shapes do not fit the staging buffer", who, n_cls, K);
+    hipLaunchKernelGGL(head_candidates_kernel, dim3(stm_cdiv(n_pixels, CAND_PX)), dim3(256), lds, stm_hs(stream), a, vec);
+    STM_CHECK_LAUNCH("head_candidates_kernel");
+    hipLaunchKernelGGL(head_control_kernel, dim3(1), dim3(64), 0, stm_hs(stream), ctl, capacity, n_pixels, patch_pixels_a, patch_pixels_b);
+    STM_CHECK_LAUNCH("head_control_kernel");
+    return STM_OK;
+}
+
+extern "C" int stm_head_patch_gather(const void* src_planes, long long src_np, void* dst_planes, int side, int n_planes, int slabs,
+                                     int capacity, int n_levels, int B, const int* lvl_start, const int* lvl_h, const int* lvl_w, const int* list,
+                                     const int* ctl, stm_stream_t stream)
+{
+    const char* who = "stm_head_patch_gather";
+    STM_REQUIRE(src_planes && dst_planes && list && ctl, STM_ENULL, "%s: NULL argument", who);
+    STM_REQUIRE(n_planes > 0 && slabs > 0 && capacity > 0 && side > 0 && (side & 1) && src_np > 0 &&
+                    (uintptr_t)src_planes % 16 == 0 && (uintptr_t)dst_planes % 16 == 0, STM_EINVAL, "%s: bad sizes or alignment", who);
+    GatherArgs a;
+    STM_REQUIRE(fill_levels(a.L, n_levels, B, lvl_start, lvl_h, lvl_w), STM_EINVAL, "%s: bad level table", who);
+    STM_REQUIRE(src_np >= a.L.start[n_levels], STM_EINVAL, "%s: the source planes hold fewer pixels than the levels", who);
+    a.src = static_cast<const uint8_t*>(src_planes); a.dst = static_cast<uint8_t*>(dst_planes);
+    a.rows = n_planes * slabs; a.src_np = src_np; a.dst_np = (int64_t)capacity * side * side; a.S = side;
+    a.list = list; a.ctl = ctl;
+    const int64_t units = (int64_t)capacity * side * side * ((a.rows + 15) / 16);
+    const unsigned grid = (unsigned)std::min<int64_t>((units + 3) / 4, 16384);
+    hipLaunchKernelGGL(head_patch_gather_kernel, dim3(grid), dim3(256), 0, stm_hs(stream), a);
+    STM_CHECK_LAUNCH("head_patch_gather_kernel");
+    return STM_OK;
+}
+
+extern "C" int stm_head_patch_mask(void* planes, int side, int n_planes, int slabs, int capacity, int n_levels, int B, const int* lvl_start,
+                                   const int* lvl_h, const int* lvl_w, const int* list, const int* ctl, stm_stream_t stream)
+{
+    const char* who = "stm_head_patch_mask";
+    STM_REQUIRE(planes && list && ctl, STM_ENULL, "%s: NULL argument", who);
+    STM_REQUIRE(n_planes > 0 && slabs > 0 && capacity > 0 && side > 0 && (side & 1) && (uintptr_t)planes % 16 == 0, STM_EINVAL, "%s: bad sizes or alignment", who);
+    Levels L;
+    STM_REQUIRE(fill_levels(L, n_levels, B, lvl_start, lvl_h, lvl_w), STM_EINVAL, "%s: bad level table", who);
+    hipLaunchKernelGGL(head_patch_mask_kernel, dim3(std::min(capacity, 2048)), dim3(256), 0, stm_hs(stream), static_cast<uint8_t*>(planes), n_planes * slabs,
+                       (int64_t)capacity * side * side, side, list, ctl, L);
+    STM_CHECK_LAUNCH("head_patch_mask_kernel");
+    return STM_OK;
+}
+
+extern "C" int stm_head_assemble_sparse_f32(const float* const* cls_logits, int cls_ld, const float* const* small, const float* const* trk,
+                                            const float* const* small_dense, const float* const* trk_dense, const stm_head_layout* L,
+                                            int row_mul, int row_add, const int* list, const int* ctl, int capacity, float* conf, float* loc,
+                                            float* mask, float* track, float* centerness, stm_stream_t stream)
+{
+    const char* who = "stm_head_assemble_sparse_f32";
+    STM_REQUIRE(cls_logits && small && trk && small_dense && trk_dense && L && list && ctl && conf && loc && mask && track && centerness, STM_ENULL,
+                "%s: NULL argument", who);
+    STM_REQUIRE(L->B > 0 && L->K > 0 && L->K <= 4 && L->n_levels > 0 && L->n_levels <= 8 && L->n_cls > 0 && cls_ld >= L->n_cls && L->mask_dim > 0 &&
+                    L->mask_dim <= L->group_pad && L->embed_dim > 0 && L->group_pad >= 5 && L->small_ld >= L->group_pad + L->mask_dim &&
+                    L->trk_ld >= L->embed_dim && capacity > 0 && row_mul > 0 && row_add >= 0 && row_add < row_mul, STM_EINVAL, "%s: bad layout", who);
+    AsmArgs a;
+    a.conf = conf; a.loc = loc; a.mask = mask; a.track = track; a.cen = centerness;
+    a.B = L->B; a.K = L->K; a.n_levels = L->n_levels; a.n_cls = L->n_cls; a.mask_dim = L->mask_dim; a.embed = L->embed_dim;
+    a.gpad = L->group_pad; a.cls_ld = cls_ld; a.small_ld = L->small_ld; a.trk_ld = L->trk_ld;
+    a.row_mul = row_mul; a.row_add = row_add; a.list = list; a.ctl = ctl; a.capacity = capacity;
+    int off = 0, start = 0;
+    for (int l = 0; l < 8; ++l) {
+        a.lvl_start[l] = l < L->n_levels ? L->lvl_start[l] : 0;
+        a.lvl_hw[l] = l < L->n_levels ? L->lvl_hw[l] : 1;
+        a.lvl_off[l] = off;
+        if (l < L->n_levels) {
+            STM_REQUIRE(L->lvl_hw[l] > 0 && L->lvl_start[l] == start, STM_EINVAL, "%s: level %d: bad pixel range", who, l);
+            off += L->lvl_hw[l] * L->K;
+            start += L->B * L->lvl_hw[l];
+        }
+    }
+    a.lvl_start[8] = 0;
+    a.N = off;
+    const int64_t rows = (int64_t)a.B * a.N;
+    const bool al = a.embed % 4 == 0 && a.embed <= 256 && a.trk_ld % 4 == 0 && ((uintptr_t)track % 16) == 0;
+    auto set = [&](const float* const* sm, const float* const* tk) -> bool {
+        a.vec4 = al;
+        for (int k = 0; k < 4; ++k) {
+            a.cls[k] = k < a.K ? cls_logits[k] : nullptr;
+            a.small[k] = k < a.K ? sm[k] : nullptr;
+            a.trk[k] = k < a.K ? tk[k] : nullptr;
+            if (k < a.K && !(a.cls[k] && a.small[k] && a.trk[k])) return false;
+            if (k < a.K) a.vec4 = a.vec4 && ((uintptr_t)a.trk[k] % 16) == 0;
+        }
+        return true;
+    };
+    STM_REQUIRE(set(small, trk), STM_ENULL, "%s: an input matrix is NULL", who);
+    hipLaunchKernelGGL(head_assemble_rows_kernel<0>, dim3(stm_xcd_grid(stm_cdiv(rows, 16))), dim3(256), 0, stm_hs(stream), a);
+    STM_CHECK_LAUNCH("head_assemble_rows_kernel<0>");
+    hipLaunchKernelGGL(head_assemble_listed_kernel, dim3((unsigned)std::min<int64_t>(stm_cdiv((int64_t)capacity * a.K, 16), 4096)), dim3(256), 0, stm_hs(stream), a);
+    STM_CHECK_LAUNCH("head_assemble_listed_kernel");
+    STM_REQUIRE(set(small_dense, trk_dense), STM_ENULL, "%s: a dense input matrix is NULL", who);
+    hipLaunchKernelGGL(head_assemble_rows_kernel<1>, dim3(stm_xcd_grid(stm_cdiv(rows, 16))), dim3(256), 0, stm_hs(stream), a);
+    STM_CHECK_LAUNCH("head_assemble_rows_kernel<1>");
+    return STM_OK;
+}
diff --git a/stmask_amd/csrc/stm_common.h b/stmask_amd/csrc/stm_common.h
--- a/stmask_amd/csrc/stm_common.h
+++ b/stmask_amd/csrc/stm_common.h
@@ -39,6 +39,8 @@
 
 int* stm_internal_range_flag();
 long long stm_internal_fused_dcn_launches();
+
+const int* stm_internal_take_pixel_gate();
 
 static inline hipStream_t stm_hs(stm_stream_t s) { return reinterpret_cast<hipStream_t>(s); }
 
diff --git a/stmask_amd/ops.py b/stmask_amd/ops.py
--- a/stmask_amd/ops.py
+++ b/stmask_amd/ops.py
@@ -726,16 +726,15 @@
     return True
 
 
-def conv_pack_weights_kxr(weight, geom):
+def conv_pack_weights_kxr(weight, geom, wscale=None):
     _dev(weight)
     weight = _f32c(weight)
     nbytes = _lib.lib().stm_conv_kxr_packed_bytes(ctypes.byref(geom))
     if nbytes == 0:
         raise StmError("conv_pack_weights_kxr: " + _lib.lib().stm_last_error_string().decode(errors="replace"))
     packed = torch.empty(nbytes, device=weight.device, dtype=torch.uint8)
-    import math
-    wmax = float(weight.abs().max())
-    wscale = 2.0 ** (10 - math.floor(math.log2(wmax))) if wmax > 0 else 1.0
+    if wscale is None:
+        wscale = _pow2_wscale(weight)
     check(_lib.lib().stm_conv_pack_weights_kxr_f32(_p(weight), _p(packed), ctypes.byref(geom), c_f(wscale), _stream()),
           "stm_conv_pack_weights_kxr_f32")
     return packed, 1.0 / wscale
@@ -1177,6 +1176,96 @@
     tp = (ctypes.c_void_p * 4)(*([t.data_ptr() for t in trk] + [0] * (4 - K)))
     check(_lib.lib().stm_head_assemble_f32(sp, tp, ctypes.byref(L), _p(conf), _p(loc), _p(mask), _p(track), _p(cen), _stream()),
           "stm_head_assemble_f32")
+    return conf, loc, mask, track, cen
+
+
+HEAD_CTL_RAW, HEAD_CTL_N, HEAD_CTL_FILL, HEAD_CTL_GATE_A, HEAD_CTL_GATE_B, HEAD_CTL_DENSE, HEAD_CTL_OVERFLOW, HEAD_CTL_INTS = 0, 1, 2, 3, 4, 5, 6, 8
+
+
+def conv_set_pixel_gate(ctl, index):
+    _lib.lib().stm_conv_set_pixel_gate(ctypes.c_void_p(ctl.data_ptr() + 4 * index))
+
+
+def _level_arrays(B, sizes):
+    n = len(sizes)
+    st, hh, ww = (ctypes.c_int * 9)(), (ctypes.c_int * 8)(), (ctypes.c_int * 8)()
+    start = 0
+    for l, (h, w) in enumerate(sizes):
+        st[l], hh[l], ww[l] = start, h, w
+        start += B * h * w
+    st[n] = start
+    return n, st, hh, ww, start
+
+
+def _ptr4(ts):
+    return (ctypes.c_void_p * 4)(*([t.data_ptr() for t in ts] + [0] * (4 - len(ts))))
+
+
+def head_candidates(cls_logits, n_cls, conf_thresh, capacity, patch_pixels_a, patch_pixels_b, B, sizes):
+    _dev(*cls_logits)
+    n_px, ld = cls_logits[0].shape
+    n, st, hh, ww, total = _level_arrays(B, sizes)
+    for t in cls_logits:
+        if t.dtype != torch.float32 or not t.is_contiguous() or tuple(t.shape) != (n_px, ld) or n_px != total:
+            raise StmError("head_candidates: inputs must be contiguous fp32 matrices over all level pixels")
+    dev = cls_logits[0].device
+    lst = torch.empty(capacity, dtype=torch.int32, device=dev)
+    ctl = torch.empty(HEAD_CTL_INTS, dtype=torch.int32, device=dev)
+    flags = torch.empty(n_px, dtype=torch.int32, device=dev)
+    check(_lib.lib().stm_head_candidates_f32(_ptr4(cls_logits), c_i(len(cls_logits)), c_i(ld), c_i(n_cls), c_f(conf_thresh), c_i(capacity),
+                                             c_i(patch_pixels_a), c_i(patch_pixels_b), c_i(n), c_i(B), st, hh, ww, _p(flags), _p(lst), _p(ctl), _stream()),
+          "stm_head_candidates_f32")
+    return lst, ctl
+
+
+def head_patch_gather(src, dst, side, capacity, B, sizes, lst, ctl):
+    _dev(src, dst)
+    if (src.dim() != 4 or dst.dim() != 4 or src.shape[3] != 32 or src.element_size() != 2 or dst.dtype != src.dtype or not src.is_contiguous()
+            or not dst.is_contiguous() or tuple(dst.shape) != (src.shape[0], src.shape[1], capacity * side * side, 32)):
+        raise StmError(f"head_patch_gather: planes {tuple(src.shape)} -> {tuple(dst.shape)} do not fit capacity {capacity}, side {side}")
+    n, st, hh, ww, _ = _level_arrays(B, sizes)
+    check(_lib.lib().stm_head_patch_gather(_p(src), ctypes.c_longlong(src.shape[2]), _p(dst), c_i(side), c_i(src.shape[0]), c_i(src.shape[1]),
+                                           c_i(capacity), c_i(n), c_i(B), st, hh, ww, _p(lst), _p(ctl), _stream()), "stm_head_patch_gather")
+    return dst
+
+
+def head_patch_mask(planes, side, capacity, B, sizes, lst, ctl):
+    _dev(planes)
+    if planes.dim() != 4 or planes.shape[3] != 32 or planes.element_size() != 2 or not planes.is_contiguous() or planes.shape[2] != capacity * side * side:
+        raise StmError(f"head_patch_mask: planes {tuple(planes.shape)} do not fit capacity {capacity}, side {side}")
+    n, st, hh, ww, _ = _level_arrays(B, sizes)
+    check(_lib.lib().stm_head_patch_mask(_p(planes), c_i(side), c_i(planes.shape[0]), c_i(planes.shape[1]), c_i(capacity), c_i(n), c_i(B), st, hh, ww,
+                                         _p(lst), _p(ctl), _stream()), "stm_head_patch_mask")
+    return planes
+
+
+def head_assemble_sparse(cls_logits, small, trk, small_dense, trk_dense, B, sizes, n_cls, mask_dim, embed_dim, group_pad, row_mul, row_add, lst, ctl,
+                         capacity):
+    _dev(*cls_logits, *small, *trk, *small_dense, *trk_dense)
+    K = len(cls_logits)
+    L = _lib.HeadLayout()
+    L.B, L.K, L.n_levels, L.n_cls, L.mask_dim, L.embed_dim, L.group_pad = B, K, len(sizes), n_cls, mask_dim, embed_dim, group_pad
+    L.small_ld, L.trk_ld = small[0].shape[-1], trk[0].shape[-1]
+    start = 0
+    for l, (h, w) in enumerate(sizes):
+        L.lvl_start[l], L.lvl_hw[l] = start, h * w
+        start += B * h * w
+    N = K * sum(h * w for h, w in sizes)
+    for t in list(cls_logits) + list(small_dense) + list(trk_dense):
+        if t.dtype != torch.float32 or not t.is_contiguous() or t.shape[0] != start:
+            raise StmError("head_assemble_sparse: dense inputs must be contiguous fp32 matrices over all level pixels")
+    for t, d in zip(list(small) + list(trk), list(small_dense) + list(trk_dense)):
+        if t.dtype != torch.float32 or not t.is_contiguous() or t.shape[0] < capacity * row_mul or t.shape[-1] != d.shape[-1]:
+            raise StmError("head_assemble_sparse: patch inputs must be contiguous fp32 matrices of capacity * row_mul rows, as wide as the dense ones")
+    dev = cls_logits[0].device
+    conf = torch.empty(B, N, n_cls, device=dev)
+    loc = torch.empty(B, N, 4, device=dev)
+    mask = torch.empty(B, N, mask_dim, device=dev)
+    track = torch.empty(B, N, embed_dim, device=dev)
+    cen = torch.empty(B, N, 1, device=dev)
+    check(_lib.lib().stm_head_assemble_sparse_f32(_ptr4(cls_logits), c_i(cls_logits[0].shape[-1]), _ptr4(small), _ptr4(trk), _ptr4(small_dense), _ptr4(trk_dense),
+                                                  ctypes.byref(L), c_i(row_mul), c_i(row_add), _p(lst), _p(ctl), c_i(capacity), _p(conf), _p(loc), _p(mask),
+                                                  _p(track), _p(cen), _stream()), "stm_head_assemble_sparse_f32")
     return conf, loc, mask, track, cen
 
 
diff --git a/stmask_amd/pipeline.py b/stmask_amd/pipeline.py
--- a/stmask_amd/pipeline.py
+++ b/stmask_amd/pipeline.py
@@ -181,10 +181,22 @@
         self._graph_next = 0
         self._graph_warm = 0
         self._graph_ws = []
+        self._graph_sparse = None
+        self._sparse_now = None
         self._graph_planes = None
         self._idle_masks = {}
         self._idle_dev = None
         self.max_instances = 0
+        self.sparse_head = os.environ.get("STM_SPARSE_HEAD", "1") != "0"
+        self.sparse_min_clips = int(os.environ.get("STM_SPARSE_MIN_CLIPS", "4"))
+        self.sparse_capacity = None
+
+    def _sparse_setting(self, pg):
+        if not (self.sparse_head and self.B >= self.sparse_min_clips and self.tf and pg is not None and pg.sparse_supported()):
+            return None
+        if not getattr(self.net.Detect_TF, "use_cross_class_nms", True):
+            return None
+        return (float(self.cfg.eval_conf_thresh), self.sparse_capacity)
 
     def _shift_prev(self, P4, T2S, proto, dev):
         net, cfg, prev = self.net, self.cfg, self.prev
@@ -246,12 +258,23 @@
         return 2 * self.prefetch_depth + 2
 
     def _trunk(self, frames):
+        pg = getattr(self.net, "_planar", None)
+        if pg is None or not hasattr(pg, "sparse"):
+            return self._trunk_run(frames)
+        self._sparse_now = self._sparse_setting(pg)
+        before, pg.sparse = pg.sparse, self._sparse_now
+        try:
+            return self._trunk_run(frames)
+        finally:
+            pg.sparse = before
+
+    def _trunk_run(self, frames):
         net = self.net
         if not (self.use_graph and getattr(net, "_planar", None) is not None and not self.timer.on and ops._conv_timing is None
                 and ops._im2col_timing is None):
             return net.forward_single(frames)
         planes = getattr(net, "_planar_planes", None)
-        if self._graphs and self._graph_planes != planes:
+        if self._graphs and (self._graph_planes != planes or self._graph_sparse != self._sparse_now):
             self._pending = []
             torch.cuda.synchronize()
             self._graphs, self._graph_next, self.graph_active, self._graph_warm, self._graph_ws = [], 0, False, 0, []
@@ -288,6 +311,7 @@
                     return net.forward_single(frames)
             self._graphs.append((static_in, graph, out))
             self._graph_planes = planes
+            self._graph_sparse = self._sparse_now
             self.graph_active = True
         static_in, graph, out = self._graphs[self._graph_next]
         self._graph_next = (self._graph_next + 1) % self.n_graph_slots
diff --git a/stmask_amd/planar.py b/stmask_amd/planar.py
--- a/stmask_amd/planar.py
+++ b/stmask_amd/planar.py
@@ -63,6 +63,7 @@
         self.relu, self.groups, self.planes, self.tile_n = relu, groups, (planes if self.fmt == 0 else ops.plane_layout(self.fmt)[0]), tile_n
         self._packed = {}
         self.out_scale = 1.0
+        self.wscale = None
         self.role = "trunk"
         self.kxr = CONV_KXR and self.out_fmt == self.fmt and ops.conv_kxr_supported(self.O, self.C, self.kh, self.kw, (self.sh, self.sw), (self.ph, self.pw),
                                                                                      self.groups, self.group_cout, self.fmt, max_tiles=3)
@@ -73,10 +74,13 @@
         if tile_n not in self._packed:
             if self.fmt >= 1:
                 ops.planar_range_flag()
-                self._packed[tile_n], self.out_scale = ops.conv_pack_weights(self.weight, tile_n=tile_n, fmt=self.fmt)
+                self._packed[tile_n], self.out_scale = ops.conv_pack_weights(self.weight, tile_n=tile_n, fmt=self.fmt, wscale=self.wscale)
             else:
                 self._packed[tile_n] = ops.conv_pack_weights(self.weight, self.planes, tile_n)
         return self._packed[tile_n]
+
+    def kxr_rule_pixels(self):
+        return 20000 if self.groups > 1 else 30000
 
     def pick_tile(self, M):
         if self.tile_n is not None:
@@ -95,7 +99,7 @@
         return 128
 
     def __call__(self, xp, shape, out="planes", x_off=0, out_planes=None, out_f32=None, out_off=0, residual=None, x_ch_off=0,
-                 out_ch_off=0, x2=None, window=None):
+                 out_ch_off=0, x2=None, window=None, gate=None, kxr=None, splitk=True):
         NP, dt = _planes_dtype(self.fmt)
         if xp.dtype != dt or xp.dim() != 4 or xp.shape[0] < NP or xp.shape[3] != 32 or not xp.is_contiguous():
             raise StmError(f"PlanarConv: expected contiguous {dt} planes [{NP}, S, N, 32], got {xp.dtype} {tuple(xp.shape)}")
@@ -136,7 +140,7 @@
                 raise StmError("PlanarConv: input slice runs past the plane buffer")
         g.x_np, g.x_plane_stride = N, S * N * 32
         use_kxr = (self.kxr and residual is None and window is None and (shape[0] == "levels" or (Ho, Wo) == (H, W))
-                   and M >= (self.kxr_min_pixels if self.kxr_min_pixels is not None else (20000 if self.groups > 1 else 30000)))
+                   and (kxr if kxr is not None else M >= (self.kxr_min_pixels if self.kxr_min_pixels is not None else self.kxr_rule_pixels())))
         g.tile_n = 0 if use_kxr else self.pick_tile(M)
         dev = xp.device
         NPo, dto = _planes_dtype(self.out_fmt)
@@ -180,8 +184,10 @@
             g.fmt = self.fmt
             if "kxr" not in self._packed:
                 ops.planar_range_flag()
-                self._packed["kxr"] = ops.conv_pack_weights_kxr(self.weight, g)
+                self._packed["kxr"] = ops.conv_pack_weights_kxr(self.weight, g, wscale=self.wscale)
             packed, g.out_scale = self._packed["kxr"]
+            if gate is not None:
+                ops.conv_set_pixel_gate(*gate)
             rc = _lib.lib().stm_conv2d_planar_kxr_f32(ctypes.c_void_p(x_ptr), ops._p(packed), ops._p(self.bias), ctypes.c_void_p(p_f32),
                                                       ctypes.c_void_p(p_pl), ctypes.byref(g), c_i(1 if self.relu else 0), ops._stream())
             check(rc, "stm_conv2d_planar_kxr_f32")
@@ -189,7 +195,11 @@
         packed = self.packed(g.tile_n)
         g.fmt, g.out_scale = self.fmt, self.out_scale
         g.out_fmt_plus1 = 0 if self.out_fmt == self.fmt else self.out_fmt + 1
-        ws = ops._workspace(self.SPLITK_WS_BYTES, dev, "conv_splitk")
+        ws = ops._workspace(self.SPLITK_WS_BYTES, dev, "conv_splitk") if splitk and gate is None else None
+        if gate is not None:
+            if x2 is not None:
+                raise StmError("PlanarConv: gated launches take no second source")
+            ops.conv_set_pixel_gate(*gate)
         if x2 is not None:
             p2, H2, W2, s2 = x2
             if p2.dtype != dt or p2.dim() != 4 or p2.shape[0] < NP or p2.shape[3] != 32 or not p2.is_contiguous() or shape[0] != "img":
@@ -204,7 +214,7 @@
         rc = _lib.lib().stm_conv2d_planar_ws_f32(ctypes.c_void_p(x_ptr), ops._p(packed),
                                                  ops._p(self.bias), ctypes.c_void_p(r32), ctypes.c_void_p(rpl),
                                                  ctypes.c_void_p(p_f32), ctypes.c_void_p(p_pl), ctypes.byref(g),
-                                                 c_i(1 if self.relu else 0), ops._p(ws), ctypes.c_size_t(ws.numel()),
+                                                 c_i(1 if self.relu else 0), ops._p(ws), ctypes.c_size_t(ws.numel() if ws is not None else 0),
                                                  ops._stream())
         check(rc, "stm_conv2d_planar_f32")
         return self._finish(timing, e0 if timing is not None else None, M, shape, g, NP, NPo, dt, out, out_f32, out_planes, residual)
@@ -322,6 +332,78 @@
                     entry.append(None)
             self.finals.append(tuple(entry))
         self.head = head
+        self.sparse = None
+        self._sparse_layers = None
+
+    SPARSE_SIDES = (9, 7, 5)
+
+    def sparse_supported(self):
+        return self.head_planar and not self.fcb and self.head.num_priors == 1
+
+    def sparse_capacity(self, B, sizes):
+        s0, s1, s2 = self.SPARSE_SIDES
+        per_frame = max(1, 2 * sum(h * w for h, w in sizes) // (s1 * s1 + s2 * s2))
+        return -(-per_frame * B // 256) * 256
+
+    def _build_sparse(self):
+        if self._sparse_layers is not None:
+            return self._sparse_layers
+        P = self.GROUP_PAD
+        cw = self.tower2.O // 4
+
+        def cut(layer, rows, **kw):
+            c = PlanarConv(layer.weight[rows], layer.bias[rows], 1, (layer.ph, layer.pw), relu=layer.relu, fmt=layer.fmt, **kw)
+            c.wscale = ops._pow2_wscale(layer.weight) if layer.fmt >= 1 else None
+            return c
+
+        t1c, t1r = cut(self.tower1, slice(0, cw)), cut(self.tower1, slice(cw, 4 * cw))
+        t2c, t2r = cut(self.tower2, slice(0, cw)), cut(self.tower2, slice(cw, 4 * cw), groups=3)
+        cls, small = [], []
+        for sm, _ in self.finals:
+            gc = sm.group_cout
+            cls.append(cut(sm, slice(0, P), tile_n=64, group_cout=gc[:1], algo_frac=gc[0] / float(P)))
+            small.append(cut(sm, slice(P, 3 * P), groups=2, tile_n=64, group_cout=gc[1:], algo_frac=sum(gc[1:]) / (2.0 * P)))
+        self._sparse_layers = (t1c, t1r, t2c, t2r, cls, small)
+        return self._sparse_layers
+
+    def _sparse_head(self, up, B, sizes, ntot, dev, toc):
+        head = self.head
+        thresh, cap = self.sparse
+        if cap is None:
+            cap = self.sparse_capacity(B, sizes)
+        t1c, t1r, t2c, t2r, cls_l, small_l = self._build_sparse()
+        trk_l = [trk for _, trk in self.finals]
+        lv = ("levels", B, sizes)
+        cw, P = self.tower2.O // 4, self.GROUP_PAD
+        S0, S1, S2 = self.SPARSE_SIDES
+        NP, pdt = _planes_dtype(self.fmt)
+        kx = ntot >= self.finals[0][0].kxr_rule_pixels()
+        x = t1c(up, lv, out="planes", splitk=False)
+        x = t2c(x, lv, out="planes", splitk=False)
+        cls = [c(x, lv, out="f32", splitk=False, kxr=kx) for c in cls_l]
+        toc("head_towers")
+        lst, ctl = ops.head_candidates(cls, head.num_classes, thresh, cap, S1 * S1, S2 * S2, B, sizes)
+        patch = ops.head_patch_gather(up, torch.empty(NP, cw // 32, cap * S0 * S0, 32, device=dev, dtype=pdt), S0, cap, B, sizes, lst, ctl)
+        x1 = torch.empty(NP, 3 * cw // 32, cap * S1 * S1, 32, device=dev, dtype=pdt)
+        t1r(patch, ("img", cap, S0, S0), out="planes", out_planes=x1, window=(0, 0, S1, S1, 0, 0, S1, S1), gate=(ctl, ops.HEAD_CTL_GATE_A))
+        ops.head_patch_mask(x1, S1, cap, B, sizes, lst, ctl)
+        gb = (ctl, ops.HEAD_CTL_GATE_B)
+        xq = torch.empty(NP, 3 * cw // 32, cap * S2 * S2, 32, device=dev, dtype=pdt)
+        t2r(x1, ("img", cap, S1, S1), out="planes", out_planes=xq, window=(0, 0, S2, S2, 0, 0, S2, S2), gate=gb)
+        ops.head_patch_mask(xq, S2, cap, B, sizes, lst, ctl)
+        ql = ("levels", cap, [(S2, S2)])
+        small = [c(xq, ql, out="f32", gate=gb, kxr=kx) for c in small_l]
+        trk = [c(xq, ql, out="f32", x_ch_off=2 * cw, gate=gb) for c in trk_l]
+        gd = (ctl, ops.HEAD_CTL_DENSE)
+        x = t1r(up, lv, out="planes", gate=gd)
+        x = t2r(x, lv, out="planes", gate=gd)
+        small_d = [c(x, lv, out="f32", gate=gd, kxr=kx) for c in small_l]
+        trk_d = [c(x, lv, out="f32", x_ch_off=2 * cw, gate=gd) for c in trk_l]
+        toc("head_finals")
+        out = ops.head_assemble_sparse(cls, small, trk, small_d, trk_d, B, sizes, head.num_classes, head.mask_dim, head.embed_dim, P,
+                                       S2 * S2, (S2 * S2) // 2, lst, ctl, cap)
+        self.sparse_ctl, self.sparse_list = ctl, lst
+        return out
 
     def run(self, bb_outs, planes=None):
         net, fpn = self.net, self.net.fpn
@@ -477,10 +559,15 @@
             up32, up = self.up(feat, lv, out="both")
         else:
             up32, up = None, self.up(feat, lv, out="planes")
-        t1 = self.tower1(up, lv, out="planes")
+        sparse_out = None
+        if self.sparse is not None and self.sparse_supported():
+            sparse_out = self._sparse_head(up, B, sizes, ntot, dev, toc)
+        t1 = self.tower1(up, lv, out="planes") if sparse_out is None else None
         cw = self.tower2.O // 4
         P = self.GROUP_PAD
-        if not self.fcb:
+        if sparse_out is not None:
+            outs = None
+        elif not self.fcb:
             t2 = self.tower2(t1, lv, out="planes")
             toc("head_towers")
             outs = [(small(t2, lv, out="f32"), trk(t2, lv, out="f32", x_ch_off=3 * cw)) for small, trk in self.finals]
@@ -550,7 +637,9 @@
         for hh, ww in sizes:
             pred["priors"].append(head.make_priors(hh, ww, dev))
         pred["priors"] = torch.cat(pred["priors"], 1)
-        if npri == 1:
+        if sparse_out is not None:
+            pred["conf"], pred["loc"], pred["mask_coeff"], pred["track"], pred["centerness"] = sparse_out
+        elif npri == 1:
             conf, loc, mask, track, cen = ops.head_assemble([o[0] for o in outs], [o[1] for o in outs], B, sizes,
                                                             head.num_classes, head.mask_dim, head.embed_dim, P)
             pred["conf"], pred["loc"], pred["mask_coeff"], pred["track"], pred["centerness"] = conf, loc, mask, track, cen
```
